# HKUDS/LLMRec

Hardware: AMD Instinct MI355X
Metric: bpr_train_edges_per_sec (higher is better)
Workload: dtype f32

## Files before the change

include/llmrec_hip.h:

```cpp
#ifndef LLMREC_HIP_H
#define LLMREC_HIP_H

#include <stdint.h>

#ifdef __cplusplus
extern "C" {
#endif

#define LLMREC_ABI_VERSION 8

enum {
    LLMREC_OK = 0,
    LLMREC_EINVAL = -1,
    LLMREC_EHIP = -2,
    LLMREC_EWORKSPACE = -3,
    LLMREC_EUNSUPPORTED = -4
};

typedef void* llmrec_stream_t;

int llmrec_abi_version(void);
const char* llmrec_status_string(int status);
const char* llmrec_last_error(void);

// ... 70 lines not shown
    const float* row_scale; const float* col_scale;
    const float* X; int64_t ldx; float* Y; int64_t ldy; int32_t d; int32_t slice_width;
    const llmrec_spmm_plan_t* plan; float* partials;
    const llmrec_spmm_epilogue_t* epilogue;
} llmrec_spmm_problem_t;
int llmrec_spmm_multi_f32(int32_t n, const llmrec_spmm_problem_t* problems, llmrec_stream_t stream);

int llmrec_linear_fwd_f32(int64_t M, int32_t N, int32_t K, const float* X, int64_t ldx,
                          const float* W, int64_t ldw, const float* bias,
                          float* Y, int64_t ldy, llmrec_stream_t stream);
#define LLMREC_LINEAR_MAX_PROBLEMS 8
typedef struct {
    const float* X; int64_t ldx; int64_t M; int32_t K;
    const float* W; int64_t ldw; const float* bias;
    float* Y; int64_t ldy;
    const float* bias_scale;
} llmrec_linear_problem_t;
int llmrec_linear_fwd_grouped_f32(int32_t n_problems, const llmrec_linear_problem_t* problems_host, int32_t N,
                                  llmrec_stream_t stream);
typedef struct { const float* dY; int64_t lddy; const float* X; int64_t ldx; int64_t M;
                 const float* db_row_weight;
                 const int32_t* row_list; const int32_t* n_rows; int64_t rows_expected;
} llmrec_wgrad_problem_t;
int llmrec_linear_wgrad_grouped_f32(int32_t n_problems, const llmrec_wgrad_problem_t* problems_host, int32_t N, int32_t K,
                                    float* dW, int64_t lddw, float* db, int32_t accumulate,
                                    void* workspace, int64_t workspace_bytes, llmrec_stream_t stream);
int llmrec_linear_wgrad_grouped_bf16x3(int32_t n_problems, const llmrec_wgrad_problem_t* problems_host, int32_t N, int32_t K,
                                       float* dW, int64_t lddw, float* db, int32_t accumulate,
                                       void* workspace, int64_t workspace_bytes, llmrec_stream_t stream);
#define LLMREC_WGRAD_MAX_TARGETS 4
typedef struct { int32_t n_problems; const llmrec_wgrad_problem_t* problems; int32_t K; float* dW; int64_t lddw; float* db; int32_t accumulate;
                 int32_t block_budget;
} llmrec_wgrad_target_t;
int64_t llmrec_linear_wgrad_multi_workspace_bytes(int32_t n_targets, const llmrec_wgrad_target_t* targets_host, int32_t N);
int llmrec_linear_wgrad_multi_bf16x3(int32_t n_targets, const llmrec_wgrad_target_t* targets_host, int32_t N,
                                     void* workspace, int64_t workspace_bytes, llmrec_stream_t stream);
typedef struct { float* W; float* m_W; float* v_W; float* b; float* m_b; float* v_b; float g_scale; } llmrec_wgrad_update_t;
int llmrec_linear_wgrad_multi_adamw_bf16x3(int32_t n_targets, const llmrec_wgrad_target_t* targets_host, int32_t N,
                                           void* workspace, int64_t workspace_bytes, const llmrec_wgrad_update_t* updates_host,
                                           const float* state3, float lr, float beta1, float beta2, float eps, float weight_decay,
                                           llmrec_stream_t stream);
int llmrec_linear_fwd_grouped_bf16x3(int32_t n_problems, const llmrec_linear_problem_t* problems_host, int32_t N,
                                     llmrec_stream_t stream);
int64_t llmrec_linear_wgrad_workspace_bytes(int64_t M, int32_t N, int32_t K);
int llmrec_linear_wgrad_f32(int64_t M, int32_t N, int32_t K, const float* dY, int64_t lddy,
                            const float* X, int64_t ldx, float* dW, int64_t lddw, float* db,
                            int32_t accumulate, void* workspace, int64_t workspace_bytes,
                            llmrec_stream_t stream);

int llmrec_softmax_rows_fwd_f32(int64_t rows, int32_t d, const float* Z, int64_t ldz,
                                float* Y, int64_t ldy, llmrec_stream_t stream);
int llmrec_softmax_rows_bwd_f32(int64_t rows, int32_t d, const float* Y, int64_t ldy,
                                const float* dY, int64_t lddy, float* dZ, int64_t lddz,
                                llmrec_stream_t stream);
int llmrec_softmax_rows_bwd_scaled_f32(int64_t rows, int32_t d, float alpha, const float* Y, int64_t ldy, const float* dY, int64_t lddy,
                                       float* dZ, int64_t lddz, llmrec_stream_t stream);
int llmrec_softmax_rows_bwd_listed_f32(int64_t n, const int64_t* ids, int32_t d, float alpha, const float* Y, int64_t ldy,
                                       const float* dY, int64_t lddy, const float* post_scale, float* dZ, int64_t lddz,
                                       llmrec_stream_t stream);

#define LLMREC_MAX_TERMS 12
int llmrec_fuse_fwd_f32(int64_t rows, int32_t d, float mean_scale,
                        int32_t n_mean, const float* const* mean_terms_host, const int64_t* mean_ld_host,
                        int32_t n_norm, const float* const* norm_terms_host, const int64_t* norm_ld_host,
                        const float* rates_host, float* out, int64_t ldo, llmrec_stream_t stream);
int llmrec_fuse_bwd_f32(int64_t rows, int32_t d, const float* dOut, int64_t lddo,
                        int32_t n_norm, const float* const* norm_terms_host, const int64_t* norm_ld_host,
                        const float* rates_host, float* const* d_terms_host, const int64_t* d_ld_host,
                        int32_t accumulate, int32_t n_reg_terms, float reg_two_coef, llmrec_stream_t stream);
int llmrec_fuse_bwd_src_f32(int64_t rows, int32_t d, const float* dOut, int64_t lddo,
                            int32_t n_norm, const float* const* norm_terms_host, const int64_t* norm_ld_host,
                            const float* rates_host, float* const* d_terms_host, const int64_t* d_ld_host,
                            const float* const* src_terms_host, const int64_t* src_ld_host,
                            int32_t n_reg_terms, float reg_two_coef, llmrec_stream_t stream);
typedef struct {
    int64_t rows; float mean_scale;
    int32_t n_mean; const float* const* mean_terms; const int64_t* mean_ld;
    int32_t n_norm; const float* const* norm_terms; const int64_t* norm_ld; const float* rates;
    float* out; int64_t ldo;
} llmrec_fuse_fwd_problem_t;
int llmrec_fuse_fwd_multi_f32(int32_t n_problems, const llmrec_fuse_fwd_problem_t* problems_host, int32_t d, llmrec_stream_t stream);
int llmrec_fuse_fwd_multi_sumsq_f32(int32_t n_problems, const llmrec_fuse_fwd_problem_t* problems_host, int32_t d, int32_t n_sumsq_terms,
                                    float* sumsq_partial, int32_t partial_capacity, int32_t* n_partial_host, llmrec_stream_t stream);
typedef struct {
    int64_t rows; const float* dOut; int64_t lddo;
    int32_t n_norm; const float* const* norm_terms; const int64_t* norm_ld; const float* rates;
    float* const* d_terms; const int64_t* d_ld;
    const float* const* src_terms; const int64_t* src_ld;
    int32_t n_reg_terms; float reg_two_coef;
    const uint8_t* row_flags;
    const int32_t* row_stamp;
} llmrec_fuse_bwd_problem_t;
int llmrec_fuse_bwd_src_multi_f32(int32_t n_problems, const llmrec_fuse_bwd_problem_t* problems_host, int32_t d, llmrec_stream_t stream);


#define LLMREC_BPR_MAX_B 4096
#define LLMREC_BPR_MAX_PROBLEMS 8
#define LLMREC_BPR_SAVED_FLOATS(B) (6 * (B) + 8)
int llmrec_bpr_prune_fwd_f32(const float* Eu, int64_t ldu, const float* Ei, int64_t ldi, int32_t d,
                             const int64_t* users, const int64_t* pos, const int64_t* neg,
                             int32_t B_max, const int32_t* n_valid_dev,
                             double remember_rate, float decay, float batch_size_flag,
                             float* out2, float* saved, llmrec_stream_t stream);
int llmrec_bpr_prune_fwd_sharded_f32(const float* Eu, int64_t ldu, const float* Ei, int64_t ldi, int32_t d,
                                     const int64_t* users, const int64_t* pos, const int64_t* neg,
                                     int32_t B_local, double remember_rate, float decay, float batch_size_flag,
                                     const float* global_m, int32_t global_B, int32_t my_offset, int32_t scores_only,
                                     float* out2, float* saved, llmrec_stream_t stream);
typedef struct {
    const float* Eu; int64_t ldu; const float* Ei; int64_t ldi;
    float* dEu; int64_t lddu; float* dEi; int64_t lddi;
    float g_mf, g_emb;
} llmrec_bpr_problem_t;
int llmrec_bpr_multi_fwd_f32(int32_t n_problems, const llmrec_bpr_problem_t* problems_host, int32_t d,
                             const int64_t* users, const int64_t* pos, const int64_t* neg,
                             int32_t B_max, const int32_t* n_valid_dev, double remember_rate, float decay,
                             float batch_size_flag, float* out, float* saved, llmrec_stream_t stream);
#define LLMREC_BPR_GATHER_FLOATS(P, B) ((P) * (B) + 4 * (P) + 1)
int llmrec_bpr_multi_fwd_sharded_f32(int32_t n_problems, const llmrec_bpr_problem_t* problems_host, int32_t d,
                                     const int64_t* users, const int64_t* pos, const int64_t* neg,
                                     int32_t B_max, const int32_t* n_valid_dev, double remember_rate, float decay,
                                     float batch_size_flag, int32_t phase, float* gather_block,
                                     const float* gathered, int32_t n_ranks, int64_t rank_stride, int32_t my_rank,
                                     float* out, float* saved, llmrec_stream_t stream);
#define LLMREC_BPR_PLAN_WORDS(B) (5 * (B))
int llmrec_bpr_scatter_plan(const int64_t* users, const int64_t* pos, const int64_t* neg, int32_t B_max, const int32_t* n_valid_dev,
                            uint64_t* plan, llmrec_stream_t stream);
int llmrec_bpr_multi_bwd_f32(int32_t n_problems, const llmrec_bpr_problem_t* problems_host, int32_t d,
                             const int64_t* users, const int64_t* pos, const int64_t* neg,
                             int32_t B_max, const int32_t* n_valid_dev, float decay, float batch_size_flag,
                             const float* saved, const uint64_t* plan, llmrec_stream_t stream);
#define LLMREC_ROW_STAMP(counter) ((uint8_t)((uint32_t)(counter) % 255u + 1u))
int llmrec_bpr_multi_scores_f32(int32_t n_problems, const llmrec_bpr_problem_t* problems_host, int32_t d,
                                const int64_t* users, const int64_t* pos, const int64_t* neg,
                                int32_t B_max, const int32_t* n_valid_dev, float* saved,
                                int32_t* row_stamp , llmrec_stream_t stream);
int llmrec_bpr_multi_select_bwd_f32(int32_t n_problems, const llmrec_bpr_problem_t* problems_host, int32_t d,
                                    const int64_t* users, const int64_t* pos, const int64_t* neg,
                                    int32_t B_max, const int32_t* n_valid_dev, double remember_rate, float decay,
                                    float batch_size_flag, float* saved,
                                    uint8_t* user_row_flags, uint8_t* item_row_flags,
                                    const int32_t* row_stamp,
                                    const uint64_t* plan,
                                    llmrec_stream_t stream);
int llmrec_bpr_multi_losses_f32(int32_t n_problems, int32_t B_max, const int32_t* n_valid_dev, double remember_rate, float decay,
                                float batch_size_flag, float* out, float* saved, llmrec_stream_t stream);
int llmrec_bpr_multi_scores_step_f32(int32_t n_problems, const llmrec_bpr_problem_t* problems_host, int32_t d,
                                     const int64_t* users, const int64_t* pos, const int64_t* neg,
                                     int32_t B_max, const int32_t* n_valid_dev, float* saved, int32_t* row_stamp,
                                     float* adamw_state3, float lr, float beta1, float beta2, llmrec_stream_t stream);
int llmrec_bpr_multi_losses_assemble_f32(int32_t n_problems, int32_t B_max, const int32_t* n_valid_dev, double remember_rate, float decay,
                                         float batch_size_flag, float* out, float* saved, const float* w_mf_host,
                                         const float* sumsq_partial, int32_t n_partial, float feat_reg_coef,
                                         float* scal4, double* running_sums3, llmrec_stream_t stream);
int llmrec_bpr_multi_zero_rows_f32(int32_t n_problems, const llmrec_bpr_problem_t* problems_host, int32_t d,
                                   const int64_t* users, const int64_t* pos, const int64_t* neg,
                                   int32_t B_max, const int32_t* n_valid_dev, llmrec_stream_t stream);
int llmrec_bpr_prune_bwd_f32(const float* Eu, int64_t ldu, const float* Ei, int64_t ldi, int32_t d,
                             const int64_t* users, const int64_t* pos, const int64_t* neg,
                             int32_t B_max, const int32_t* n_valid_dev,
                             float decay, float batch_size_flag,
                             const float* saved, const float* grads2,
                             float* dEu, int64_t lddu, float* dEi, int64_t lddi, const uint64_t* plan, llmrec_stream_t stream);

int llmrec_bpr_prune_bwd_rows_f32(const float* Eu, int64_t ldu, const float* Ei, int64_t ldi, int32_t d,
                                  const int64_t* users, const int64_t* pos, const int64_t* neg,
                                  int32_t B_max, const int32_t* n_valid_dev,
                                  float decay, float batch_size_flag,
                                  const float* saved, const float* grads2, float* rows3, llmrec_stream_t stream);

int64_t llmrec_scatter_rows_workspace_bytes(int64_t n);
int llmrec_scatter_rows_f32(int64_t n, const int64_t* ids, const float* rows, int64_t ldr, int32_t d, float alpha,
                            float* dst, int64_t ldd, void* workspace, int64_t workspace_bytes, llmrec_stream_t stream);

int64_t llmrec_sumsq_workspace_bytes(int64_t rows, int32_t d);
int llmrec_sumsq_f32(int64_t rows, int32_t d, const float* X, int64_t ldx, float coef, int32_t accumulate,
                     float* out, void* workspace, int64_t workspace_bytes, llmrec_stream_t stream);
int llmrec_axpy_f32(int64_t rows, int32_t d, float alpha, const float* alpha_dev, const float* X, int64_t ldx,
                    float* Y, int64_t ldy, int32_t accumulate, llmrec_stream_t stream);

#define LLMREC_COLSUM_MAX_GROUPS 8
int64_t llmrec_weighted_colsum_workspace_bytes(int32_t n_columns);
int llmrec_weighted_colsum_f32(int64_t rows, int32_t n_groups, int32_t group_width, const float* X, int64_t ldx, const float* w,
                               float* const* group_out_host, int32_t accumulate,
                               void* workspace, int64_t workspace_bytes, llmrec_stream_t stream);

#define LLMREC_ZERO_MAX_TENSORS 8
typedef struct { float* p; int64_t n; } llmrec_zero_tensor_t;
int llmrec_zero_multi_f32(int32_t n_tensors, const llmrec_zero_tensor_t* tensors_host, llmrec_stream_t stream);
int llmrec_zero_rows_f32(int64_t n, const int64_t* ids, int32_t d, float* dst, int64_t ldd, llmrec_stream_t stream);

int llmrec_loss_assemble_f32(int32_t mode, int32_t n_problems, const float* bpr_out, const float* w_mf_host,
                             float* scal4, float* tail, float inv_world, double* running_sums3, llmrec_stream_t stream);

int llmrec_gather_mean_f32(int64_t n, const int64_t* idx, int32_t d, float scale, int32_t n_terms,
                           const float* const* terms, const int64_t* term_ld, float* out, int64_t ldo, llmrec_stream_t stream);
int llmrec_scale_rows_f32(int64_t rows, int32_t d, const float* s, const float* X, int64_t ldx, float* Y, int64_t ldy,
                          llmrec_stream_t stream);

int llmrec_adamw_advance(float* state3, float lr, float beta1, float beta2, llmrec_stream_t stream);
int llmrec_adamw_f32(int64_t n, float* p, const float* g, float* m, float* v, const float* state3,
                     float lr, float beta1, float beta2, float eps, float weight_decay, llmrec_stream_t stream);

#define LLMREC_ADAMW_MAX_TENSORS 16
#define LLMREC_ADAMW_CHUNK 1024
typedef struct { float* p; const float* g; float* m; float* v; int64_t n;
                 float g_scale;
                 float* g_out;
} llmrec_adamw_tensor_t;
int llmrec_adamw_multi_f32(int32_t n_tensors, const llmrec_adamw_tensor_t* tensors_host, const float* state3,
                           float lr, float beta1, float beta2, float eps, float weight_decay, llmrec_stream_t stream);
#define LLMREC_ZERO_ROWS_MAX_JOBS 24
typedef struct { const int64_t* ids; float* dst; int64_t ldd; int32_t d; } llmrec_zero_rows_job_t;
int llmrec_adamw_multi_zero_rows_f32(int32_t n_tensors, const llmrec_adamw_tensor_t* tensors_host, const float* state3,
                                     float lr, float beta1, float beta2, float eps, float weight_decay,
                                     int32_t n_jobs, const llmrec_zero_rows_job_t* jobs_host, int32_t B_cap, const int32_t* n_valid_dev,
                                     llmrec_stream_t stream);

int llmrec_step_rows_group_f32(int32_t n_fuse_problems, const llmrec_fuse_bwd_problem_t* fuse_host, int32_t d,
                               int32_t n_tensors, const llmrec_adamw_tensor_t* tensors_host, const float* state3,
                               float lr, float beta1, float beta2, float eps, float weight_decay,
                               int64_t sm_rows, int32_t sm_d, float sm_alpha, const float* sm_Y, int64_t sm_ldy, const float* sm_dY, int64_t sm_lddy,
                               float* sm_dZ, int64_t sm_lddz, llmrec_stream_t stream);

#define LLMREC_TOPK_MAX 64
int llmrec_score_topk_f32(int32_t n_query, const int64_t* query_users,
                          const float* Eu, int64_t ldu, const float* Ei, int64_t ldi,
                          int64_t n_items, int32_t d,
                          const int32_t* train_rowptr, const int32_t* train_colidx,
                          int32_t K, int32_t* out_idx , float* out_score ,
                          llmrec_stream_t stream);
int llmrec_topk_set_part_items(int32_t items);
int64_t llmrec_score_topk_workspace_bytes(int32_t n_query, int64_t n_items, int32_t d);
int llmrec_score_topk_ws_f32(int32_t n_query, const int64_t* query_users,
                             const float* Eu, int64_t ldu, const float* Ei, int64_t ldi,
                             int64_t n_items, int32_t d,
                             const int32_t* train_rowptr, const int32_t* train_colidx,
                             int32_t K, int32_t* out_idx , float* out_score ,
                             void* workspace, int64_t workspace_bytes, llmrec_stream_t stream);
#define LLMREC_TOPK_PREFILTER_MAX_K 56
#define LLMREC_TOPK_MODE_EXACT_SWEEP 0
#define LLMREC_TOPK_MODE_PREFILTER 1
int llmrec_score_topk_mode_f32(int32_t n_query, const int64_t* query_users,
                               const float* Eu, int64_t ldu, const float* Ei, int64_t ldi,
                               int64_t n_items, int32_t d,
                               const int32_t* train_rowptr, const int32_t* train_colidx,
                               int32_t K, int32_t* out_idx, float* out_score,
                               void* workspace, int64_t workspace_bytes, int32_t mode, llmrec_stream_t stream);
int64_t llmrec_score_topk_stats_offset(int32_t n_query, int64_t n_items);
#define LLMREC_TOPK_WIDE_MAX 1024
int64_t llmrec_score_topk_wide_workspace_bytes(int32_t n_query, int64_t n_items, int32_t d, int32_t K, int64_t train_nnz);
int llmrec_score_topk_wide_f32(int32_t n_query, const int64_t* query_users,
                               const float* Eu, int64_t ldu, const float* Ei, int64_t ldi,
                               int64_t n_items, int32_t d,
                               const int32_t* train_rowptr, const int32_t* train_colidx,
                               int32_t K, int32_t* out_idx, float* out_score,
                               void* workspace, int64_t workspace_bytes, int32_t mode, int64_t train_nnz, llmrec_stream_t stream);
int llmrec_scores_f32(int32_t n_query, const int64_t* query_users,
                      const float* Eu, int64_t ldu, const float* Ei, int64_t ldi,
                      int64_t n_items, int32_t d, float* S, int64_t lds, llmrec_stream_t stream);
int llmrec_topk_hits(int32_t n_query, const int64_t* query_users, int32_t K, const int32_t* topk_idx,
                     const int32_t* test_rowptr, const int32_t* test_colidx, uint8_t* hits,
                     llmrec_stream_t stream);
int llmrec_topk_metrics(int32_t n_query, const int64_t* query_users, int32_t K, const uint8_t* hits, const int32_t* topk_idx,
                        const int32_t* test_rowptr, int32_t n_ks, const int32_t* ks_host, double* out, llmrec_stream_t stream);
int64_t llmrec_topk_eval_sums_workspace_bytes(int32_t n_query, int32_t n_ks);
int llmrec_topk_eval_sums(int32_t n_query, const int64_t* query_users, int32_t K, const int32_t* topk_idx, const int32_t* test_rowptr,
                          const int32_t* test_colidx, int32_t n_ks, const int32_t* ks_host, void* workspace, int64_t workspace_bytes,
                          double* out, llmrec_stream_t stream);
int64_t llmrec_score_auc_workspace_bytes(int32_t n_query, int64_t n_items, int32_t d);
int llmrec_score_auc_f32(int32_t n_query, const int64_t* query_users,
                         const float* Eu, int64_t ldu, const float* Ei, int64_t ldi,
                         int64_t n_items, int32_t d,
                         const int32_t* train_rowptr, const int32_t* train_colidx,
                         const int32_t* held_rowptr, const int32_t* held_colidx,
                         double* auc_out, int64_t* counts_out, double* sum_out,
                         void* workspace, int64_t workspace_bytes, llmrec_stream_t stream);

int llmrec_sample_bpr(uint64_t seed, uint64_t step, int64_t n_exist_users, const int64_t* exist_users,
                      int64_t n_items, const int32_t* train_rowptr, const int32_t* train_colidx,
                      int32_t B, int64_t* users, int64_t* pos, int64_t* neg, llmrec_stream_t stream);
int llmrec_sample_batch(uint64_t seed, uint64_t* step_dev, int64_t n_exist_users, const int64_t* exist_users,
                        int64_t n_items, const int32_t* train_rowptr, const int32_t* train_colidx,
                        int32_t B_global, int32_t slice_begin, int32_t B, int32_t n_aug,
                        const int64_t* aug_pos, const int64_t* aug_neg,
                        int64_t* users, int64_t* pos, int64_t* neg, int32_t* n_valid_dev, llmrec_stream_t stream);

int llmrec_timestamp(uint64_t* slot, llmrec_stream_t stream);
int64_t llmrec_timestamp_rate_hz(void);

#ifdef __cplusplus
}
#endif
#endif
```

llmrec_amd/csrc/bpr.hip:

```cpp
#include "common.h"

namespace llmrec {

constexpr int BPR_THREADS = 1024;

__device__ __forceinline__ float logsigmoid_f(float x) {
    return fminf(x, 0.f) - log1pf(expf(-fabsf(x)));
}

struct BprTables {
    const float* Eu[LLMREC_BPR_MAX_PROBLEMS];
    const float* Ei[LLMREC_BPR_MAX_PROBLEMS];
    int64_t ldu[LLMREC_BPR_MAX_PROBLEMS];
    int64_t ldi[LLMREC_BPR_MAX_PROBLEMS];
    float* dEu[LLMREC_BPR_MAX_PROBLEMS];
    float* dEi[LLMREC_BPR_MAX_PROBLEMS];
    int64_t lddu[LLMREC_BPR_MAX_PROBLEMS];
    int64_t lddi[LLMREC_BPR_MAX_PROBLEMS];
    float g_mf[LLMREC_BPR_MAX_PROBLEMS];
    float g_emb[LLMREC_BPR_MAX_PROBLEMS];
};

__device__ __forceinline__ int bpr_batch(const int32_t* n_valid_dev, int B_max) {
    int B = n_valid_dev ? n_valid_dev[0] : B_max;
    return B > B_max ? B_max : (B < 0 ? 0 : B);
}

struct StepBegin {
    int32_t* row_stamp;
    float* adamw_state;
    float lr, b1, b2;
};

__global__ __launch_bounds__(256) void bpr_scores_kernel(BprTables t, int d, const int64_t* __restrict__ users,
                                                         const int64_t* __restrict__ pos, const int64_t* __restrict__ neg,
                                                         int B_max, const int32_t* __restrict__ n_valid_dev,
                                                         float* __restrict__ saved_all, int saved_stride, StepBegin sb) {
    const int B = bpr_batch(n_valid_dev, B_max);
    const int prob = blockIdx.y;
    const int gl = threadIdx.x & 15;
    const int b = blockIdx.x * 16 + (threadIdx.x >> 4);
    if (blockIdx.x == 0 && blockIdx.y == 0 && threadIdx.x == 0) {
        if (sb.row_stamp) sb.row_stamp[0] = (int32_t)((uint32_t)sb.row_stamp[0] + 1u);
        if (sb.adamw_state) {
            const int tt = __float_as_int(sb.adamw_state[0]) + 1;
            sb.adamw_state[0] = __int_as_float(tt);
            const double bc1 = 1.0 - pow((double)sb.b1, (double)tt);
            const double bc2 = 1.0 - pow((double)sb.b2, (double)tt);
            sb.adamw_state[1] = (float)((double)sb.lr / bc1);
            sb.adamw_state[2] = (float)sqrt(bc2);
        }
    }
    if (b >= B) return;
    float* sc = saved_all + (int64_t)prob * saved_stride + B_max + 4;
    const float* u = t.Eu[prob] + users[b] * t.ldu[prob];
    const float* p = t.Ei[prob] + pos[b] * t.ldi[prob];
    const float* q = t.Ei[prob] + neg[b] * t.ldi[prob];
    float dp = 0.f, dn = 0.f, nu = 0.f, np_ = 0.f, nq = 0.f;
    for (int c = gl; c < d; c += 16) {
        const float uu = u[c], pp = p[c], qq = q[c];
        dp = fmaf(uu, pp, dp); dn = fmaf(uu, qq, dn);
        nu = fmaf(uu, uu, nu); np_ = fmaf(pp, pp, np_); nq = fmaf(qq, qq, nq);
    }
    dp = group_sum<16>(dp); dn = group_sum<16>(dn);
    nu = group_sum<16>(nu); np_ = group_sum<16>(np_); nq = group_sum<16>(nq);
    if (gl == 0) {
        const float x = (dp - dn) + 1e-8f;
        sc[b] = logsigmoid_f(x);
        sc[B_max + b] = 1.0f / (1.0f + expf(x));
        sc[2 * B_max + b] = nu; sc[3 * B_max + b] = np_; sc[4 * B_max + b] = nq;
    }
}

__device__ __forceinline__ float block_tree_sum(float v, float* red) {
    red[threadIdx.x] = v;
    __syncthreads();
    for (int off = BPR_THREADS / 2; off > 0; off >>= 1) {
        if ((int)threadIdx.x < off) red[threadIdx.x] += red[threadIdx.x + off];
        __syncthreads();
    }
    const float r = red[0];
    __syncthreads();
    return r;
// ... 26 lines not shown
    extern __shared__ __attribute__((aligned(16))) char smem[];
    float* m_s = reinterpret_cast<float*>(smem);
    const int B = bpr_batch(n_valid_dev, B_max);
    const int prob = blockIdx.y;
    float* saved = saved_all + (int64_t)prob * saved_stride;
    float* sc = saved + B_max + 4;
    int Bg, slots;
    if (ga.g) {
        slots = ga.n_ranks * ga.cap;
        Bg = gather_batch(ga);
        for (int r = 0; r < ga.n_ranks; ++r) {
            const int nv = gather_valid(ga, r);
            const float* src = ga.g + r * ga.stride + (int64_t)prob * ga.cap;
            for (int j = threadIdx.x; j < ga.cap; j += 256) m_s[r * ga.cap + j] = j < nv ? src[j] : __builtin_inff();
        }
    } else {
        slots = Bg = B;
        for (int j = threadIdx.x; j < B; j += 256) m_s[j] = sc[j];
    }
    __syncthreads();
    const int k = (int)(remember_rate * (double)Bg);
    const int gl = threadIdx.x & 15;
    const int b = blockIdx.x * 16 + (threadIdx.x >> 4);
    if (b >= B_max) return;
    if (b >= B) { if (gl == 0) { saved[b] = 0.f; sc[B_max + b] = 0.f; } return; }
    const float mb = sc[b];
    bool keep = true;
    if (k < Bg) {
        int rank = 0;
        const int me = ga.my_offset + b;
        for (int j = gl; j < slots; j += 16) {
            const float mj = m_s[j];
            rank += (mj < mb) || (mj == mb && j < me);
        }
        rank = (int)group_sum<16>((float)rank);
        keep = rank < k;
    }
    if (gl == 0) {
        saved[b] = keep ? (-1.0f / (float)k) * sc[B_max + b] : 0.f;
        sc[B_max + b] = keep ? mb : 0.f;
    }
}

__device__ __forceinline__ void bpr_reduce_problem(int prob, int B_max, const int32_t* __restrict__ n_valid_dev,
                                                   double remember_rate, float decay, float bsz,
                                                   float* __restrict__ out_all, float* __restrict__ saved_all,
                                                   int saved_stride, const BprGather& ga, float* red) {
    const int B = bpr_batch(n_valid_dev, B_max);
    float* saved = saved_all + (int64_t)prob * saved_stride;
    const float* sc = saved + B_max + 4;
    const int Bg = ga.g ? gather_batch(ga) : B;
    const int k = (int)(remember_rate * (double)Bg);
    float part = 0.f, su = 0.f, sp = 0.f, sq = 0.f;
    for (int b = threadIdx.x; b < B; b += BPR_THREADS) {
        part += sc[B_max + b];
        su += sc[2 * B_max + b]; sp += sc[3 * B_max + b]; sq += sc[4 * B_max + b];
    }
    const float kept = block_tree_sum(part, red);
    float Su = block_tree_sum(su, red), Sp = block_tree_sum(sp, red), Sq = block_tree_sum(sq, red);
    if (threadIdx.x == 0) {
        if (ga.g && ga.has_tail) {
            Su = Sp = Sq = 0.f;
            for (int r = 0; r < ga.n_ranks; ++r) {
                const float* nb = ga.g + r * ga.stride + (int64_t)ga.n_prob * ga.cap + 4 * prob;
                Su += nb[0]; Sp += nb[1]; Sq += nb[2];
            }
        }
        out_all[prob * 2 + 0] = -(kept / (float)k);
        const float reg = 1.0f / (2.0f * Su + 1e-8f) + 1.0f / (2.0f * Sp + 1e-8f) + 1.0f / (2.0f * Sq + 1e-8f);
        out_all[prob * 2 + 1] = decay * (reg / bsz);
        saved[B_max + 0] = Su; saved[B_max + 1] = Sp; saved[B_max + 2] = Sq; saved[B_max + 3] = (float)k;
    }
}

__global__ __launch_bounds__(BPR_THREADS) void bpr_reduce_kernel(int B_max, const int32_t* __restrict__ n_valid_dev,
                                                                 double remember_rate, float decay, float bsz,
                                                                 float* __restrict__ out_all, float* __restrict__ saved_all,
                                                                 int saved_stride, BprGather ga) {
    __shared__ float red[BPR_THREADS];
    bpr_reduce_problem(blockIdx.x, B_max, n_valid_dev, remember_rate, decay, bsz, out_all, saved_all, saved_stride, ga, red);
}

struct LossW { float w[LLMREC_BPR_MAX_PROBLEMS]; };
constexpr int LA_GROUP = BPR_THREADS / LLMREC_BPR_MAX_PROBLEMS;
__global__ __launch_bounds__(BPR_THREADS) void bpr_losses_assemble_kernel(int n_prob, int B_max, const int32_t* __restrict__ n_valid_dev,
                                                                          double remember_rate, float decay, float bsz,
                                                                          float* __restrict__ out_all, float* __restrict__ saved_all, int saved_stride,
                                                                          LossW w, const float* __restrict__ partial, int n_partial, float reg_coef,
                                                                          float* __restrict__ scal, double* __restrict__ running) {
    __shared__ float red[LLMREC_BPR_MAX_PROBLEMS][BPR_THREADS];
    __shared__ float outs[LLMREC_BPR_MAX_PROBLEMS][2];
    const int B = bpr_batch(n_valid_dev, B_max);
    const int prob = threadIdx.x / LA_GROUP, t = threadIdx.x % LA_GROUP;
    const bool live = prob < n_prob;
    float* saved = saved_all + (int64_t)(live ? prob : 0) * saved_stride;
    const float* sc = saved + B_max + 4;
    float tot[4] = {0.f, 0.f, 0.f, 0.f};
#pragma unroll
    for (int col = 0; col < 4; ++col) {
        const float* src = sc + (int64_t)(col + 1) * B_max;
        if (live) {
            for (int v = t; v < BPR_THREADS; v += LA_GROUP) {
                float s_ = 0.f;
                for (int b = v; b < B; b += BPR_THREADS) s_ += src[b];
                red[prob][v] = s_;
            }
        }
        __syncthreads();
        for (int off = BPR_THREADS / 2; off > 0; off >>= 1) {
            if (live) for (int i = t; i < off; i += LA_GROUP) red[prob][i] += red[prob][i + off];
            __syncthreads();
        }
        tot[col] = red[live ? prob : 0][0];
        __syncthreads();
    }
    if (live && t == 0) {
        const int k = (int)(remember_rate * (double)B);
        const float mf = -(tot[0] / (float)k);
        const float reg = 1.0f / (2.0f * tot[1] + 1e-8f) + 1.0f / (2.0f * tot[2] + 1e-8f) + 1.0f / (2.0f * tot[3] + 1e-8f);
        const float emb = decay * (reg / bsz);
        out_all[prob * 2 + 0] = mf; out_all[prob * 2 + 1] = emb;
        outs[prob][0] = mf; outs[prob][1] = emb;
        saved[B_max + 0] = tot[1]; saved[B_max + 1] = tot[2]; saved[B_max + 2] = tot[3]; saved[B_max + 3] = (float)k;
    }
    float feat = scal[0];
    if (partial) {
        float s_ = 0.f;
        for (int i = threadIdx.x; i < n_partial; i += BPR_THREADS) s_ += partial[i];
        feat = reg_coef * block_tree_sum(s_, red[0]);
    }
    __syncthreads();
    if (threadIdx.x != 0) return;
    float s = 0.f;
    for (int p = 0; p < n_prob; ++p) s += outs[p][0] * w.w[p];
    scal[0] = feat;
    scal[2] = outs[0][0]; scal[3] = outs[0][1];
    scal[1] = s + outs[0][1] + feat;
    if (running) { running[0] += (double)scal[1]; running[1] += (double)scal[2]; running[2] += (double)scal[3]; }
}

__global__ __launch_bounds__(256) void bpr_pack_kernel(int n_prob, int B_max, const int32_t* __restrict__ n_valid_dev,
                                                       const float* __restrict__ saved_all, int saved_stride, float* __restrict__ block) {
    const int B = bpr_batch(n_valid_dev, B_max);
    const int total = n_prob * B_max + 4 * n_prob + 1;
    for (int i = blockIdx.x * 256 + threadIdx.x; i < total; i += gridDim.x * 256) {
        float v;
        if (i < n_prob * B_max) {
            const int p = i / B_max, b = i - p * B_max;
            v = b < B ? saved_all[(int64_t)p * saved_stride + B_max + 4 + b] : __builtin_inff();
        } else if (i < n_prob * B_max + 4 * n_prob) {
            const int j = i - n_prob * B_max;
            v = saved_all[(int64_t)(j >> 2) * saved_stride + B_max + (j & 3)];
        } else {
            v = (float)B;
        }
        block[i] = v;
    }
}

constexpr uint32_t PLAN_NO_ID = 0xffffffffu;
__global__ __launch_bounds__(256) void bpr_plan_kernel(const int64_t* __restrict__ users, const int64_t* __restrict__ pos,
                                                       const int64_t* __restrict__ neg, int B_max,
                                                       const int32_t* __restrict__ n_valid_dev, uint64_t* __restrict__ plan) {
    extern __shared__ __attribute__((aligned(16))) char smem[];
    uint64_t* k = reinterpret_cast<uint64_t*>(smem);
    const int B = bpr_batch(n_valid_dev, B_max);
    const int nbu = (B_max + 15) / 16;
    const bool items = (int)blockIdx.x >= nbu;
    const int n = items ? 2 * B_max : B_max;
    for (int i = threadIdx.x; i < n; i += 256) {
        const int b = (items && i >= B_max) ? i - B_max : i;
        uint64_t id = PLAN_NO_ID;
        if (b < B) id = (uint64_t)(items ? (i >= B_max ? neg[b] : pos[b]) : users[b]);
        k[i] = (id << 32) | (uint64_t)(uint32_t)i;
    }
    __syncthreads();
    const int gl = threadIdx.x & 15;
    const int i = ((int)blockIdx.x - (items ? nbu : 0)) * 16 + (threadIdx.x >> 4);
    if (i >= n) return;
    const uint64_t me = k[i];
    const uint32_t id = (uint32_t)(me >> 32);
    int below = 0, lower_id = 0, same_id = 0;
    for (int j = gl; j < n; j += 16) {
        const uint64_t kj = k[j];
        const uint32_t idj = (uint32_t)(kj >> 32);
        below += kj < me; lower_id += idj < id; same_id += idj == id;
    }
    below = (int)group_sum<16>((float)below); lower_id = (int)group_sum<16>((float)lower_id); same_id = (int)group_sum<16>((float)same_id);
    if (gl == 0) {
        const int base = items ? B_max : 0;
        plan[base + below] = me;
        int32_t* runlen = reinterpret_cast<int32_t*>(plan + 3 * (int64_t)B_max);
        runlen[base + below] = (below == lower_id && id != PLAN_NO_ID) ? same_id : 0;
    }
}

constexpr int RUN_MAX_SHARE = LLMREC_BPR_MAX_PROBLEMS;
struct RunShare {
    const float* Eu[RUN_MAX_SHARE]; const float* Ei[RUN_MAX_SHARE]; const float* saved[RUN_MAX_SHARE];
    int64_t ldu[RUN_MAX_SHARE], ldi[RUN_MAX_SHARE];
    float g_mf[RUN_MAX_SHARE], cu[RUN_MAX_SHARE], cp[RUN_MAX_SHARE], cq[RUN_MAX_SHARE];
    int n, any_reg;
};
struct RunRec { const float* a; const float* b; const float* self; float ds, cr; };

template <int NV, bool VEC> struct RunAcc;
template <int NV> struct RunAcc<NV, true> {
    float4 v[NV];
    __device__ __forceinline__ void load(const float* row, int c0, int d, int gl) {
#pragma unroll
        for (int i = 0; i < NV; ++i) { const int c = c0 + 4 * (gl + 16 * i); v[i] = c < d ? *reinterpret_cast<const float4*>(row + c) : float4{0.f, 0.f, 0.f, 0.f}; }
    }
    __device__ __forceinline__ void store(float* row, int c0, int d, int gl) const {
#pragma unroll
        for (int i = 0; i < NV; ++i) { const int c = c0 + 4 * (gl + 16 * i); if (c < d) *reinterpret_cast<float4*>(row + c) = v[i]; }
    }
};
template <int NV> struct RunAcc<NV, false> {
    float v[4 * NV];
    __device__ __forceinline__ void load(const float* row, int c0, int d, int gl) {
#pragma unroll
        for (int i = 0; i < 4 * NV; ++i) { const int c = c0 + gl + 16 * i; v[i] = c < d ? row[c] : 0.f; }
    }
    __device__ __forceinline__ void store(float* row, int c0, int d, int gl) const {
#pragma unroll
        for (int i = 0; i < 4 * NV; ++i) { const int c = c0 + gl + 16 * i; if (c < d) row[c] = v[i]; }
    }
};
template <int NV, bool VEC, bool ITEM, bool REG>
__device__ __forceinline__ void run_add(RunAcc<NV, VEC>& acc, const RunAcc<NV, VEC>& a, const RunAcc<NV, VEC>& b, const RunAcc<NV, VEC>& self,
                                        float ds, float cr) {
    if constexpr (VEC) {
#pragma unroll
        for (int i = 0; i < NV; ++i) {
            const float4 x = a.v[i], y = ITEM ? float4{0.f, 0.f, 0.f, 0.f} : b.v[i], z = REG ? self.v[i] : float4{0.f, 0.f, 0.f, 0.f};
            acc.v[i].x += fmaf(ds, ITEM ? x.x : x.x - y.x, cr * z.x); acc.v[i].y += fmaf(ds, ITEM ? x.y : x.y - y.y, cr * z.y);
            acc.v[i].z += fmaf(ds, ITEM ? x.z : x.z - y.z, cr * z.z); acc.v[i].w += fmaf(ds, ITEM ? x.w : x.w - y.w, cr * z.w);
        }
    } else {
#pragma unroll
        for (int i = 0; i < 4 * NV; ++i)
            acc.v[i] += fmaf(ds, ITEM ? a.v[i] : a.v[i] - b.v[i], cr * (REG ? self.v[i] : 0.f));
    }
}

template <int NV, bool VEC, bool ITEM, bool REG>
__device__ __forceinline__ void run_stream(RunAcc<NV, VEC>& acc, const RunRec* __restrict__ recs, int n, int c0, int d, int gl) {
    int i = 0;
    for (; i + 4 <= n; i += 4) {
        RunAcc<NV, VEC> a[4], b[4], z[4];
        float ds[4], cr[4];
#pragma unroll
        for (int u = 0; u < 4; ++u) {
            const RunRec r = recs[i + u];
            ds[u] = r.ds; cr[u] = r.cr;
            a[u].load(r.a, c0, d, gl);
            if (!ITEM) b[u].load(r.b, c0, d, gl);
            if (REG) z[u].load(r.self, c0, d, gl);
        }
#pragma unroll
        for (int u = 0; u < 4; ++u) run_add<NV, VEC, ITEM, REG>(acc, a[u], b[u], z[u], ds[u], cr[u]);
    }
    for (; i < n; ++i) {
        const RunRec r = recs[i];
        RunAcc<NV, VEC> a, b, z;
        a.load(r.a, c0, d, gl);
        if (!ITEM) b.load(r.b, c0, d, gl);
        if (REG) z.load(r.self, c0, d, gl);
        run_add<NV, VEC, ITEM, REG>(acc, a, b, z, r.ds, r.cr);
    }
}

template <bool VEC, int NV>
__global__ __launch_bounds__(256) void bpr_bwd_runs_kernel(BprTables t, int n_prob, int d, const int64_t* __restrict__ users,
                                                           const int64_t* __restrict__ pos, const int64_t* __restrict__ neg,
                                                           int B_max, float decay, float bsz, const float* __restrict__ saved_all,
                                                           int saved_stride, const uint64_t* __restrict__ plan,
// ... 143 lines not shown
    const int B = bpr_batch(n_valid_dev, B_max);
    const int prob = blockIdx.y;
    const int gl = threadIdx.x & 15;
    const int b = blockIdx.x * 16 + (threadIdx.x >> 4);
    if (b >= B) return;
    float* du = t.dEu[prob] + users[b] * t.lddu[prob];
    float* dpp = t.dEi[prob] + pos[b] * t.lddi[prob];
    float* dqq = t.dEi[prob] + neg[b] * t.lddi[prob];
    for (int c = gl; c < d; c += 16) { du[c] = 0.f; dpp[c] = 0.f; dqq[c] = 0.f; }
}

__global__ __launch_bounds__(256) void bpr_bwd_rows_kernel(const float* __restrict__ Eu, int64_t ldu,
                                                           const float* __restrict__ Ei, int64_t ldi, int d,
                                                           const int64_t* __restrict__ users, const int64_t* __restrict__ pos,
                                                           const int64_t* __restrict__ neg, int B_max,
                                                           const int32_t* __restrict__ n_valid_dev, float decay, float bsz,
                                                           const float* __restrict__ saved, const float* __restrict__ grads2,
                                                           float* __restrict__ rows3) {
    int B = n_valid_dev ? n_valid_dev[0] : B_max;
    if (B > B_max) B = B_max;
    const float g_mf = grads2[0], g_emb = grads2[1];
    const float Su = saved[B_max], Sp = saved[B_max + 1], Sq = saved[B_max + 2];
    const float base = -4.0f * decay / bsz * g_emb;
    const float du_ = 2.0f * Su + 1e-8f, dp_ = 2.0f * Sp + 1e-8f, dq_ = 2.0f * Sq + 1e-8f;
    const float cu = base / (du_ * du_), cp = base / (dp_ * dp_), cq = base / (dq_ * dq_);
    const int gl = threadIdx.x & 15;
    const int groups = gridDim.x * (blockDim.x >> 4);
    const int64_t plane = (int64_t)B_max * d;
    for (int b = blockIdx.x * (blockDim.x >> 4) + (threadIdx.x >> 4); b < B_max; b += groups) {
        float* ru = rows3 + (int64_t)b * d;
        if (b >= B) {
            for (int c = gl; c < d; c += 16) { ru[c] = 0.f; ru[plane + c] = 0.f; ru[2 * plane + c] = 0.f; }
            continue;
        }
        const float ds = g_mf * saved[b];
        const float* u = Eu + users[b] * ldu;
        const float* p = Ei + pos[b] * ldi;
        const float* q = Ei + neg[b] * ldi;
        for (int c = gl; c < d; c += 16) {
            const float uu = u[c], pp = p[c], qq = q[c];
            ru[c] = fmaf(ds, pp - qq, cu * uu);
            ru[plane + c] = fmaf(ds, uu, cp * pp);
            ru[2 * plane + c] = fmaf(-ds, uu, cq * qq);
        }
    }
}

struct Philox {
    uint32_t key[2];
    __device__ Philox(uint64_t seed) { key[0] = (uint32_t)seed; key[1] = (uint32_t)(seed >> 32); }
    __device__ void operator()(uint32_t c0, uint32_t c1, uint32_t c2, uint32_t c3, uint32_t out[4]) const {
        uint32_t k0 = key[0], k1 = key[1];
#pragma unroll
        for (int r = 0; r < 10; ++r) {
            const uint64_t p0 = (uint64_t)0xD2511F53u * c0, p1 = (uint64_t)0xCD9E8D57u * c2;
            const uint32_t n0 = (uint32_t)(p1 >> 32) ^ c1 ^ k0, n1 = (uint32_t)p1;
            const uint32_t n2 = (uint32_t)(p0 >> 32) ^ c3 ^ k1, n3 = (uint32_t)p0;
            c0 = n0; c1 = n1; c2 = n2; c3 = n3;
            k0 += 0x9E3779B9u; k1 += 0xBB67AE85u;
        }
        out[0] = c0; out[1] = c1; out[2] = c2; out[3] = c3;
    }
};

__device__ __forceinline__ uint32_t bounded(uint32_t r, uint32_t n) { return (uint32_t)(((uint64_t)r * n) >> 32); }

__device__ uint64_t keyed_perm(uint64_t x, uint64_t n, int half_bits, const Philox& ph, uint32_t step_lo, uint32_t step_hi) {
    const uint64_t mask = (1ull << half_bits) - 1;
    do {
        uint64_t L = x >> half_bits, R = x & mask;
#pragma unroll
        for (int r = 0; r < 4; ++r) {
            uint32_t o[4];
            ph((uint32_t)R, (uint32_t)(R >> 32) ^ (0xA5A50000u + r), step_lo, step_hi, o);
            const uint64_t f = (((uint64_t)o[1] << 32) | o[0]) & mask;
            const uint64_t nL = R, nR = L ^ f;
            L = nL; R = nR;
        }
        x = (L << half_bits) | R;
    } while (x >= n);
    return x;
}

__device__ __forceinline__ void sample_one(const Philox& ph, uint32_t slo, uint32_t shi, int b, int B, int half_bits,
                                           int64_t n_exist, const int64_t* __restrict__ exist_users, int64_t n_items,
                                           const int32_t* __restrict__ rowptr, const int32_t* __restrict__ colidx,
                                           int64_t& u_out, int64_t& p_out, int64_t& q_out) {
    uint64_t slot;
    if ((int64_t)B <= n_exist) {
        slot = keyed_perm((uint64_t)b, (uint64_t)n_exist, half_bits, ph, slo, shi);
    } else {
        uint32_t o[4];
        ph((uint32_t)b, 0x55AA0001u, slo, shi, o);
        slot = ((((uint64_t)o[1] << 32) | o[0]) % (uint64_t)n_exist);
    }
    const int64_t u = exist_users[slot];
    const int32_t s = rowptr[u], e = rowptr[u + 1];
    uint32_t o[4];
    ph((uint32_t)b, 0x55AA0002u, slo, shi, o);
    const int64_t p = colidx[s + (int32_t)bounded(o[0], (uint32_t)(e - s))];
    int64_t q = 0;
    uint32_t ctr = 0;
    int have = 4;
    for (int tries = 0; tries < 4096; ++tries) {
        if (have == 4) { ph((uint32_t)b, 0x55AA0003u + ctr, slo, shi, o); ++ctr; have = 0; }
        const uint32_t r = o[have++];
        q = n_items <= 0xffffffffll ? (int64_t)bounded(r, (uint32_t)n_items) : (int64_t)(r % (uint64_t)n_items);
        int32_t lo = s, hi = e;
        while (lo < hi) {
            const int32_t mid = (lo + hi) >> 1;
            if (colidx[mid] < q) lo = mid + 1; else hi = mid;
        }
        if (!(lo < e && colidx[lo] == q)) break;
    }
    u_out = u; p_out = p; q_out = q;
}

__global__ void sample_bpr_kernel(uint64_t seed, uint64_t step, int64_t n_exist, const int64_t* __restrict__ exist_users,
                                  int64_t n_items, const int32_t* __restrict__ rowptr, const int32_t* __restrict__ colidx,
                                  int B, int half_bits, int64_t* __restrict__ users, int64_t* __restrict__ pos,
                                  int64_t* __restrict__ neg) {
    const int b = blockIdx.x * blockDim.x + threadIdx.x;
    if (b >= B) return;
    const Philox ph(seed);
    sample_one(ph, (uint32_t)step, (uint32_t)(step >> 32), b, B, half_bits, n_exist, exist_users, n_items, rowptr, colidx,
               users[b], pos[b], neg[b]);
}

constexpr int SAMPLE_THREADS = 1024;
__global__ __launch_bounds__(SAMPLE_THREADS) void sample_batch_kernel(
    uint64_t seed, unsigned long long* __restrict__ step_dev, int64_t n_exist, const int64_t* __restrict__ exist_users,
    int64_t n_items, const int32_t* __restrict__ rowptr, const int32_t* __restrict__ colidx,
    int B_global, int half_bits_users, int slice_begin, int B, int n_aug, int half_bits_batch,
    const int64_t* __restrict__ aug_pos, const int64_t* __restrict__ aug_neg,
    int64_t* __restrict__ users, int64_t* __restrict__ pos, int64_t* __restrict__ neg, int32_t* __restrict__ n_valid_dev) {
    __shared__ int wave_tot[SAMPLE_THREADS / 64];
    __shared__ int base_s;
    const unsigned long long step = *step_dev;
    const uint32_t slo = (uint32_t)step, shi = (uint32_t)(step >> 32);
    const Philox ph(seed);
    for (int b = threadIdx.x; b < B; b += SAMPLE_THREADS)
        sample_one(ph, slo, shi, slice_begin + b, B_global, half_bits_users, n_exist, exist_users, n_items, rowptr, colidx,
                   users[b], pos[b], neg[b]);
    if (threadIdx.x == 0) base_s = 0;
    __syncthreads();
    const Philox pa(seed ^ 0x9E3779B97F4A7C15ull);
    const int lane = threadIdx.x & 63, wv = threadIdx.x >> 6;
    for (int a0 = 0; a0 < n_aug; a0 += SAMPLE_THREADS) {
        const int a = a0 + threadIdx.x;
        int64_t u = 0, ap = 0, an = 0;
        bool ok = false;
        if (a < n_aug) {
            const uint64_t slot = keyed_perm((uint64_t)a, (uint64_t)B, half_bits_batch, pa, slo, shi);
            u = users[slot];
            ap = aug_pos[u]; an = aug_neg[u];
            ok = ap >= 0 && an >= 0 && ap < n_items && an < n_items;
        }
        const unsigned long long bal = __ballot(ok);
        const int before = __popcll(bal & ((1ull << lane) - 1ull));
        if (lane == 0) wave_tot[wv] = __popcll(bal);
        __syncthreads();
        int wave_base = 0, chunk_tot = 0;
        for (int k = 0; k < SAMPLE_THREADS / 64; ++k) { const int t = wave_tot[k]; if (k < wv) wave_base += t; chunk_tot += t; }
        const int base = base_s;
        if (a < n_aug && ok) {
            const int o = B + base + wave_base + before;
            users[o] = u; pos[o] = ap; neg[o] = an;
        }
        __syncthreads();
        if (threadIdx.x == 0) base_s = base + chunk_tot;
        __syncthreads();
    }
    const int kept = base_s;
    for (int o = B + kept + threadIdx.x; o < B + n_aug; o += SAMPLE_THREADS) { users[o] = 0; pos[o] = 0; neg[o] = 0; }
    if (threadIdx.x == 0) { n_valid_dev[0] = B + kept; *step_dev = step + 1ull; }
}

}

using namespace llmrec;

extern "C" {

static int launch_bpr_fwd(const BprTables& t, int n_prob, int d, const int64_t* users, const int64_t* pos, const int64_t* neg,
                          int B_max, const int32_t* n_valid_dev, double remember_rate, float decay, float bsz,
                          float* out, float* saved, const BprGather& ga, bool do_scores, bool do_select, float* pack_out,
                          hipStream_t stream, StepBegin step_begin = StepBegin{}) {
    const int stride = LLMREC_BPR_SAVED_FLOATS(B_max);
    const BprGather none = {};
    if (do_scores && B_max > 0) {
        dim3 grid((unsigned)ceil_div(B_max, 16), (unsigned)n_prob);
        bpr_scores_kernel<<<grid, 256, 0, stream>>>(t, d, users, pos, neg, B_max, n_valid_dev, saved, stride, step_begin);
        LLMREC_LAUNCH_CHECK();
    }
    if (pack_out) {
        bpr_reduce_kernel<<<n_prob, BPR_THREADS, 0, stream>>>(B_max, n_valid_dev, remember_rate, decay, bsz, out, saved, stride, none);
        LLMREC_LAUNCH_CHECK();
        bpr_pack_kernel<<<ceil_div(n_prob * B_max + 4 * n_prob + 1, 256), 256, 0, stream>>>(n_prob, B_max, n_valid_dev, saved, stride, pack_out);
        LLMREC_LAUNCH_CHECK();
    }
    if (do_select) {
        const size_t shmem = sizeof(float) * (size_t)(ga.g ? ga.n_ranks * ga.cap : (B_max > 0 ? B_max : 1));
        dim3 grid((unsigned)ceil_div(B_max > 0 ? B_max : 1, 16), (unsigned)n_prob);
        bpr_rank_kernel<<<grid, 256, shmem, stream>>>(B_max, n_valid_dev, remember_rate, saved, stride, ga);
        LLMREC_LAUNCH_CHECK();
        bpr_reduce_kernel<<<n_prob, BPR_THREADS, 0, stream>>>(B_max, n_valid_dev, remember_rate, decay, bsz, out, saved, stride, ga);
        LLMREC_LAUNCH_CHECK();
    }
    return LLMREC_OK;
}

int llmrec_bpr_prune_fwd_f32(const float* Eu, int64_t ldu, const float* Ei, int64_t ldi, int32_t d,
                             const int64_t* users, const int64_t* pos, const int64_t* neg,
                             int32_t B_max, const int32_t* n_valid_dev,
                             double remember_rate, float decay, float batch_size_flag,
                             float* out2, float* saved, llmrec_stream_t stream_) {
    LLMREC_CHECK_ARG(B_max >= 0 && d > 0 && out2 && saved, "bpr_fwd: bad argument");
    if (B_max > LLMREC_BPR_MAX_B) { set_error("bpr_fwd: B_max %d > %d", B_max, LLMREC_BPR_MAX_B); return LLMREC_EUNSUPPORTED; }
    LLMREC_CHECK_ARG(B_max == 0 || (Eu && Ei && users && pos && neg && ldu >= d && ldi >= d), "bpr_fwd: null pointer or ld < d");
    BprTables t = {};
    t.Eu[0] = Eu; t.Ei[0] = Ei; t.ldu[0] = ldu; t.ldi[0] = ldi;
    return launch_bpr_fwd(t, 1, d, users, pos, neg, B_max, n_valid_dev, remember_rate, decay, batch_size_flag, out2, saved,
                          BprGather{}, true, true, nullptr, (hipStream_t)stream_);
}

int llmrec_bpr_prune_fwd_sharded_f32(const float* Eu, int64_t ldu, const float* Ei, int64_t ldi, int32_t d,
                                     const int64_t* users, const int64_t* pos, const int64_t* neg,
                                     int32_t B_local, double remember_rate, float decay, float batch_size_flag,
                                     const float* global_m, int32_t global_B, int32_t my_offset, int32_t scores_only,
                                     float* out2, float* saved, llmrec_stream_t stream_) {
    LLMREC_CHECK_ARG(B_local >= 0 && d > 0 && out2 && saved, "bpr_fwd_sharded: bad argument");
    if (B_local > LLMREC_BPR_MAX_B || global_B > 3 * LLMREC_BPR_MAX_B) { set_error("bpr_fwd_sharded: batch too large"); return LLMREC_EUNSUPPORTED; }
    LLMREC_CHECK_ARG(B_local == 0 || (Eu && Ei && users && pos && neg && ldu >= d && ldi >= d), "bpr_fwd_sharded: null pointer or ld < d");
    LLMREC_CHECK_ARG(scores_only || (global_m && global_B >= B_local && my_offset >= 0 && my_offset + B_local <= global_B),
                     "bpr_fwd_sharded: pass 2 needs the gathered scores and a valid offset");
    BprTables t = {};
    t.Eu[0] = Eu; t.Ei[0] = Ei; t.ldu[0] = ldu; t.ldi[0] = ldi;
    BprGather ga = {};
    if (!scores_only) { ga.g = global_m; ga.n_ranks = 1; ga.stride = 0; ga.cap = global_B; ga.n_prob = 1; ga.my_offset = my_offset; ga.has_tail = 0; }
    return launch_bpr_fwd(t, 1, d, users, pos, neg, B_local, nullptr, remember_rate, decay, batch_size_flag, out2, saved,
                          ga, scores_only != 0, scores_only == 0, nullptr, (hipStream_t)stream_);
}

static int fill_tables(BprTables& t, int n, const llmrec_bpr_problem_t* p, int d, bool need_grads) {
    for (int i = 0; i < n; ++i) {
        if (!p[i].Eu || !p[i].Ei || p[i].ldu < d || p[i].ldi < d) return 1;
        if (need_grads && (!p[i].dEu || !p[i].dEi || p[i].lddu < d || p[i].lddi < d)) return 1;
        t.Eu[i] = p[i].Eu; t.Ei[i] = p[i].Ei; t.ldu[i] = p[i].ldu; t.ldi[i] = p[i].ldi;
        t.dEu[i] = p[i].dEu; t.dEi[i] = p[i].dEi; t.lddu[i] = p[i].lddu; t.lddi[i] = p[i].lddi;
        t.g_mf[i] = p[i].g_mf; t.g_emb[i] = p[i].g_emb;
    }
    return 0;
}

int llmrec_bpr_multi_fwd_f32(int32_t n_problems, const llmrec_bpr_problem_t* problems_host, int32_t d,
                             const int64_t* users, const int64_t* pos, const int64_t* neg,
                             int32_t B_max, const int32_t* n_valid_dev, double remember_rate, float decay,
                             float batch_size_flag, float* out, float* saved, llmrec_stream_t stream_) {
    LLMREC_CHECK_ARG(n_problems >= 1 && n_problems <= LLMREC_BPR_MAX_PROBLEMS && problems_host && d > 0 && out && saved,
                     "bpr_multi_fwd: bad argument");
    if (B_max > LLMREC_BPR_MAX_B) { set_error("bpr_multi_fwd: B_max %d > %d", B_max, LLMREC_BPR_MAX_B); return LLMREC_EUNSUPPORTED; }
    LLMREC_CHECK_ARG(B_max == 0 || (users && pos && neg), "bpr_multi_fwd: null index pointer");
    BprTables t = {};
    LLMREC_CHECK_ARG(!fill_tables(t, n_problems, problems_host, d, false), "bpr_multi_fwd: bad problem table");
    return launch_bpr_fwd(t, n_problems, d, users, pos, neg, B_max, n_valid_dev, remember_rate, decay, batch_size_flag, out, saved,
                          BprGather{}, true, true, nullptr, (hipStream_t)stream_);
}

int llmrec_bpr_multi_fwd_sharded_f32(int32_t n_problems, const llmrec_bpr_problem_t* problems_host, int32_t d,
                                     const int64_t* users, const int64_t* pos, const int64_t* neg,
                                     int32_t B_max, const int32_t* n_valid_dev, double remember_rate, float decay,
                                     float batch_size_flag, int32_t phase, float* gather_block,
                                     const float* gathered, int32_t n_ranks, int64_t rank_stride, int32_t my_rank,
                                     float* out, float* saved, llmrec_stream_t stream_) {
    LLMREC_CHECK_ARG(n_problems >= 1 && n_problems <= LLMREC_BPR_MAX_PROBLEMS && problems_host && d > 0 && out && saved,
                     "bpr_multi_fwd_sharded: bad argument");
    LLMREC_CHECK_ARG(phase == 1 || phase == 2, "bpr_multi_fwd_sharded: phase is 1 (scores + gather block) or 2 (selection)");
    if (B_max > LLMREC_BPR_MAX_B) { set_error("bpr_multi_fwd_sharded: B_max %d > %d", B_max, LLMREC_BPR_MAX_B); return LLMREC_EUNSUPPORTED; }
    LLMREC_CHECK_ARG(B_max == 0 || (users && pos && neg), "bpr_multi_fwd_sharded: null index pointer");
    BprTables t = {};
    LLMREC_CHECK_ARG(!fill_tables(t, n_problems, problems_host, d, false), "bpr_multi_fwd_sharded: bad problem table");
    if (phase == 1) {
        LLMREC_CHECK_ARG(gather_block, "bpr_multi_fwd_sharded: phase 1 needs the gather block");
        return launch_bpr_fwd(t, n_problems, d, users, pos, neg, B_max, n_valid_dev, remember_rate, decay, batch_size_flag, out, saved,
                              BprGather{}, true, false, gather_block, (hipStream_t)stream_);
    }
    LLMREC_CHECK_ARG(gathered && n_ranks >= 1 && my_rank >= 0 && my_rank < n_ranks &&
                     rank_stride >= LLMREC_BPR_GATHER_FLOATS(n_problems, B_max), "bpr_multi_fwd_sharded: bad gathered layout");
    if ((int64_t)n_ranks * B_max > 4 * LLMREC_BPR_MAX_B) {
        set_error("bpr_multi_fwd_sharded: global batch capacity %lld > %d", (long long)n_ranks * B_max, 4 * LLMREC_BPR_MAX_B);
        return LLMREC_EUNSUPPORTED;
    }
    BprGather ga = {};
    ga.g = gathered; ga.n_ranks = n_ranks; ga.stride = rank_stride; ga.cap = B_max; ga.n_prob = n_problems;
    ga.my_offset = my_rank * B_max; ga.has_tail = 1;
    return launch_bpr_fwd(t, n_problems, d, users, pos, neg, B_max, n_valid_dev, remember_rate, decay, batch_size_flag, out, saved,
                          ga, false, true, nullptr, (hipStream_t)stream_);
}

int llmrec_bpr_scatter_plan(const int64_t* users, const int64_t* pos, const int64_t* neg, int32_t B_max, const int32_t* n_valid_dev,
                            uint64_t* plan, llmrec_stream_t stream_) {
    LLMREC_CHECK_ARG(B_max >= 0, "bpr_scatter_plan: bad argument");
    if (B_max > LLMREC_BPR_MAX_B) { set_error("bpr_scatter_plan: B_max %d > %d", B_max, LLMREC_BPR_MAX_B); return LLMREC_EUNSUPPORTED; }
    if (B_max == 0) return LLMREC_OK;
    LLMREC_CHECK_ARG(users && pos && neg && plan, "bpr_scatter_plan: null pointer");
    const unsigned blocks = (unsigned)(ceil_div(B_max, 16) + ceil_div(2 * (int64_t)B_max, 16));
    bpr_plan_kernel<<<blocks, 256, sizeof(uint64_t) * 2 * (size_t)B_max, (hipStream_t)stream_>>>(users, pos, neg, B_max, n_valid_dev, plan);
    LLMREC_LAUNCH_CHECK();
    return LLMREC_OK;
}

static int launch_bwd_runs(const BprTables& t, int n_prob, int d, const int64_t* users, const int64_t* pos, const int64_t* neg, int B_max,
                           float decay, float bsz, const float* saved, const uint64_t* plan, const float* grads2_dev, hipStream_t stream) {
    dim3 grid((unsigned)(ceil_div(B_max, 16) + ceil_div(2 * (int64_t)B_max, 16)), (unsigned)n_prob);
    bool vec = d % 4 == 0;
    for (int i = 0; i < n_prob && vec; ++i)
        vec = t.ldu[i] % 4 == 0 && t.ldi[i] % 4 == 0 && t.lddu[i] % 4 == 0 && t.lddi[i] % 4 == 0 &&
              ((uintptr_t)t.Eu[i] | (uintptr_t)t.Ei[i] | (uintptr_t)t.dEu[i] | (uintptr_t)t.dEi[i]) % 16 == 0;
    const int stride = LLMREC_BPR_SAVED_FLOATS(B_max);
#define RUNS_LAUNCH(V, N) bpr_bwd_runs_kernel<V, N><<<grid, 256, 0, stream>>>(t, n_prob, d, users, pos, neg, B_max, decay, bsz, saved, stride, plan, grads2_dev)
    if (vec) { if (d <= 64) RUNS_LAUNCH(true, 1); else RUNS_LAUNCH(true, 2); }
    else { if (d <= 64) RUNS_LAUNCH(false, 1); else RUNS_LAUNCH(false, 2); }
#undef RUNS_LAUNCH
    LLMREC_LAUNCH_CHECK();
    return LLMREC_OK;
}

int llmrec_bpr_multi_bwd_f32(int32_t n_problems, const llmrec_bpr_problem_t* problems_host, int32_t d,
                             const int64_t* users, const int64_t* pos, const int64_t* neg,
                             int32_t B_max, const int32_t* n_valid_dev, float decay, float batch_size_flag,
                             const float* saved, const uint64_t* plan, llmrec_stream_t stream_) {
    (void)n_valid_dev;
    LLMREC_CHECK_ARG(n_problems >= 1 && n_problems <= LLMREC_BPR_MAX_PROBLEMS && problems_host && d > 0 && saved,
                     "bpr_multi_bwd: bad argument");
    if (B_max == 0) return LLMREC_OK;
    LLMREC_CHECK_ARG(users && pos && neg && plan, "bpr_multi_bwd: null index pointer or no scatter plan (llmrec_bpr_scatter_plan)");
    BprTables t = {};
    LLMREC_CHECK_ARG(!fill_tables(t, n_problems, problems_host, d, true), "bpr_multi_bwd: bad problem table");
    return launch_bwd_runs(t, n_problems, d, users, pos, neg, B_max, decay, batch_size_flag, saved, plan, nullptr, (hipStream_t)stream_);
}

int llmrec_bpr_multi_scores_f32(int32_t n_problems, const llmrec_bpr_problem_t* problems_host, int32_t d,
                                const int64_t* users, const int64_t* pos, const int64_t* neg,
                                int32_t B_max, const int32_t* n_valid_dev, float* saved, int32_t* row_stamp, llmrec_stream_t stream_) {
    LLMREC_CHECK_ARG(n_problems >= 1 && n_problems <= LLMREC_BPR_MAX_PROBLEMS && problems_host && d > 0 && saved, "bpr_multi_scores: bad argument");
    if (B_max > LLMREC_BPR_MAX_B) { set_error("bpr_multi_scores: B_max %d > %d", B_max, LLMREC_BPR_MAX_B); return LLMREC_EUNSUPPORTED; }
    LLMREC_CHECK_ARG(B_max == 0 || (users && pos && neg), "bpr_multi_scores: null index pointer");
    BprTables t = {};
    LLMREC_CHECK_ARG(!fill_tables(t, n_problems, problems_host, d, false), "bpr_multi_scores: bad problem table");
    StepBegin sb = {};
    sb.row_stamp = row_stamp;
    return launch_bpr_fwd(t, n_problems, d, users, pos, neg, B_max, n_valid_dev, 0.0, 0.f, 1.f, nullptr, saved, BprGather{}, true, false,
                          nullptr, (hipStream_t)stream_, sb);
}

int llmrec_bpr_multi_scores_step_f32(int32_t n_problems, const llmrec_bpr_problem_t* problems_host, int32_t d,
                                     const int64_t* users, const int64_t* pos, const int64_t* neg,
                                     int32_t B_max, const int32_t* n_valid_dev, float* saved, int32_t* row_stamp,
                                     float* adamw_state3, float lr, float beta1, float beta2, llmrec_stream_t stream_) {
    LLMREC_CHECK_ARG(n_problems >= 1 && n_problems <= LLMREC_BPR_MAX_PROBLEMS && problems_host && d > 0 && saved, "bpr_multi_scores_step: bad argument");
    if (B_max > LLMREC_BPR_MAX_B) { set_error("bpr_multi_scores_step: B_max %d > %d", B_max, LLMREC_BPR_MAX_B); return LLMREC_EUNSUPPORTED; }
    LLMREC_CHECK_ARG(B_max > 0 && users && pos && neg, "bpr_multi_scores_step: empty batch capacity or null index pointer (the launch carries the step's counters)");
    BprTables t = {};
    LLMREC_CHECK_ARG(!fill_tables(t, n_problems, problems_host, d, false), "bpr_multi_scores_step: bad problem table");
    StepBegin sb = {};
    sb.row_stamp = row_stamp; sb.adamw_state = adamw_state3; sb.lr = lr; sb.b1 = beta1; sb.b2 = beta2;
    return launch_bpr_fwd(t, n_problems, d, users, pos, neg, B_max, n_valid_dev, 0.0, 0.f, 1.f, nullptr, saved, BprGather{}, true, false,
                          nullptr, (hipStream_t)stream_, sb);
}

int llmrec_bpr_multi_select_bwd_f32(int32_t n_problems, const llmrec_bpr_problem_t* problems_host, int32_t d,
                                    const int64_t* users, const int64_t* pos, const int64_t* neg,
                                    int32_t B_max, const int32_t* n_valid_dev, double remember_rate, float decay,
                                    float batch_size_flag, float* saved, uint8_t* user_row_flags, uint8_t* item_row_flags,
                                    const int32_t* row_stamp, const uint64_t* plan, llmrec_stream_t stream_) {
    LLMREC_CHECK_ARG(n_problems >= 1 && n_problems <= LLMREC_BPR_MAX_PROBLEMS && problems_host && d > 0 && saved, "bpr_multi_select_bwd: bad argument");
    if (B_max > LLMREC_BPR_MAX_B) { set_error("bpr_multi_select_bwd: B_max %d > %d", B_max, LLMREC_BPR_MAX_B); return LLMREC_EUNSUPPORTED; }
    if (B_max == 0) return LLMREC_OK;
    LLMREC_CHECK_ARG(users && pos && neg && plan, "bpr_multi_select_bwd: null index pointer or no scatter plan (llmrec_bpr_scatter_plan)");
    BprTables t = {};
    LLMREC_CHECK_ARG(!fill_tables(t, n_problems, problems_host, d, true), "bpr_multi_select_bwd: bad problem table");
    dim3 grid((unsigned)ceil_div(B_max, 16) + 1u, (unsigned)n_problems);
    const size_t shmem = sizeof(float) * (size_t)(B_max > 3 * BPR_THREADS ? B_max : 3 * BPR_THREADS);
    bpr_select_kernel<<<grid, 256, shmem, (hipStream_t)stream_>>>(users, pos, neg, B_max, n_valid_dev, remember_rate, saved,
                                                                 LLMREC_BPR_SAVED_FLOATS(B_max), user_row_flags, item_row_flags, row_stamp);
    LLMREC_LAUNCH_CHECK();
    return launch_bwd_runs(t, n_problems, d, users, pos, neg, B_max, decay, batch_size_flag, saved, plan, nullptr, (hipStream_t)stream_);
}

int llmrec_bpr_multi_losses_f32(int32_t n_problems, int32_t B_max, const int32_t* n_valid_dev, double remember_rate, float decay,
// ... 24 lines not shown
}

int llmrec_bpr_multi_zero_rows_f32(int32_t n_problems, const llmrec_bpr_problem_t* problems_host, int32_t d,
                                   const int64_t* users, const int64_t* pos, const int64_t* neg,
                                   int32_t B_max, const int32_t* n_valid_dev, llmrec_stream_t stream_) {
    LLMREC_CHECK_ARG(n_problems >= 1 && n_problems <= LLMREC_BPR_MAX_PROBLEMS && problems_host && d > 0, "bpr_multi_zero_rows: bad argument");
    if (B_max == 0) return LLMREC_OK;
    LLMREC_CHECK_ARG(users && pos && neg, "bpr_multi_zero_rows: null index pointer");
    BprTables t = {};
    LLMREC_CHECK_ARG(!fill_tables(t, n_problems, problems_host, d, true), "bpr_multi_zero_rows: bad problem table");
    dim3 grid((unsigned)ceil_div(B_max, 16), (unsigned)n_problems);
    bpr_zero_rows_kernel<<<grid, 256, 0, (hipStream_t)stream_>>>(t, d, users, pos, neg, B_max, n_valid_dev);
    LLMREC_LAUNCH_CHECK();
    return LLMREC_OK;
}

int llmrec_bpr_prune_bwd_f32(const float* Eu, int64_t ldu, const float* Ei, int64_t ldi, int32_t d,
                             const int64_t* users, const int64_t* pos, const int64_t* neg,
                             int32_t B_max, const int32_t* n_valid_dev, float decay, float batch_size_flag,
                             const float* saved, const float* grads2,
                             float* dEu, int64_t lddu, float* dEi, int64_t lddi, const uint64_t* plan, llmrec_stream_t stream_) {
    (void)n_valid_dev;
    LLMREC_CHECK_ARG(B_max >= 0 && d > 0 && saved && grads2, "bpr_bwd: bad argument");
    if (B_max == 0) return LLMREC_OK;
    LLMREC_CHECK_ARG(Eu && Ei && users && pos && neg && dEu && dEi && ldu >= d && ldi >= d && lddu >= d && lddi >= d,
                     "bpr_bwd: null pointer or ld < d");
    LLMREC_CHECK_ARG(plan, "bpr_bwd: no scatter plan (llmrec_bpr_scatter_plan)");
    LLMREC_CHECK_ARG(dEu != dEi, "bpr_bwd: dEu and dEi must be distinct buffers");
    BprTables t = {};
    t.Eu[0] = Eu; t.Ei[0] = Ei; t.ldu[0] = ldu; t.ldi[0] = ldi;
    t.dEu[0] = dEu; t.dEi[0] = dEi; t.lddu[0] = lddu; t.lddi[0] = lddi;
    return launch_bwd_runs(t, 1, d, users, pos, neg, B_max, decay, batch_size_flag, saved, plan, grads2, (hipStream_t)stream_);
}

int llmrec_bpr_prune_bwd_rows_f32(const float* Eu, int64_t ldu, const float* Ei, int64_t ldi, int32_t d,
                                  const int64_t* users, const int64_t* pos, const int64_t* neg,
                                  int32_t B_max, const int32_t* n_valid_dev, float decay, float batch_size_flag,
                                  const float* saved, const float* grads2, float* rows3, llmrec_stream_t stream_) {
    hipStream_t stream = (hipStream_t)stream_;
    LLMREC_CHECK_ARG(B_max >= 0 && d > 0 && saved && grads2, "bpr_bwd_rows: bad argument");
    if (B_max == 0) return LLMREC_OK;
    LLMREC_CHECK_ARG(Eu && Ei && users && pos && neg && rows3 && ldu >= d && ldi >= d, "bpr_bwd_rows: null pointer or ld < d");
    bpr_bwd_rows_kernel<<<grid_for(B_max, 16), 256, 0, stream>>>(Eu, ldu, Ei, ldi, d, users, pos, neg, B_max, n_valid_dev, decay,
                                                                 batch_size_flag, saved, grads2, rows3);
    LLMREC_LAUNCH_CHECK();
    return LLMREC_OK;
}

int llmrec_sample_bpr(uint64_t seed, uint64_t step, int64_t n_exist_users, const int64_t* exist_users,
                      int64_t n_items, const int32_t* train_rowptr, const int32_t* train_colidx,
                      int32_t B, int64_t* users, int64_t* pos, int64_t* neg, llmrec_stream_t stream_) {
    LLMREC_CHECK_ARG(B >= 0 && n_exist_users > 0 && n_items > 0, "sample_bpr: bad sizes");
    if (B == 0) return LLMREC_OK;
    LLMREC_CHECK_ARG(exist_users && train_rowptr && train_colidx && users && pos && neg, "sample_bpr: null pointer");
    int half_bits = 1;
    while ((1ull << (2 * half_bits)) < (uint64_t)n_exist_users) ++half_bits;
    sample_bpr_kernel<<<(B + 255) / 256, 256, 0, (hipStream_t)stream_>>>(seed, step, n_exist_users, exist_users, n_items,
                                                                          train_rowptr, train_colidx, B, half_bits, users, pos, neg);
    LLMREC_LAUNCH_CHECK();
    return LLMREC_OK;
}

int llmrec_sample_batch(uint64_t seed, uint64_t* step_dev, int64_t n_exist_users, const int64_t* exist_users,
                        int64_t n_items, const int32_t* train_rowptr, const int32_t* train_colidx,
                        int32_t B_global, int32_t slice_begin, int32_t B, int32_t n_aug,
                        const int64_t* aug_pos, const int64_t* aug_neg,
                        int64_t* users, int64_t* pos, int64_t* neg, int32_t* n_valid_dev, llmrec_stream_t stream_) {
    LLMREC_CHECK_ARG(B >= 1 && B_global >= B && slice_begin >= 0 && slice_begin + B <= B_global && n_aug >= 0 && n_aug <= B &&
                     n_exist_users > 0 && n_items > 0, "sample_batch: bad sizes");
    LLMREC_CHECK_ARG(step_dev && exist_users && train_rowptr && train_colidx && users && pos && neg && n_valid_dev,
                     "sample_batch: null pointer");
    LLMREC_CHECK_ARG(n_aug == 0 || (aug_pos && aug_neg), "sample_batch: augmented pairs missing");
    int hb_users = 1, hb_batch = 1;
    while ((1ull << (2 * hb_users)) < (uint64_t)n_exist_users) ++hb_users;
    while ((1ull << (2 * hb_batch)) < (uint64_t)B) ++hb_batch;
    sample_batch_kernel<<<1, SAMPLE_THREADS, 0, (hipStream_t)stream_>>>(seed, (unsigned long long*)step_dev, n_exist_users, exist_users,
                                                                       n_items, train_rowptr, train_colidx, B_global, hb_users,
                                                                       slice_begin, B, n_aug, hb_batch, aug_pos, aug_neg,
                                                                       users, pos, neg, n_valid_dev);
    LLMREC_LAUNCH_CHECK();
    return LLMREC_OK;
}

}
```

llmrec_amd/csrc/rowops.hip:

```cpp
#include "common.h"
#include <type_traits>

namespace llmrec {

constexpr int RL = 16;
constexpr int ROWS_PER_BLOCK = 256 / RL;

template <int VEC, int NCHUNK>
struct RowReg {
    float x[NCHUNK][VEC];
    __device__ __forceinline__ void load(const float* row, int gl, int d) {
#pragma unroll
        for (int k = 0; k < NCHUNK; ++k) {
            const int c = (k * RL + gl) * VEC;
            if (VEC == 4) {
                float4 v = (c < d) ? *reinterpret_cast<const float4*>(row + c) : make_float4(0.f, 0.f, 0.f, 0.f);
                x[k][0] = v.x; x[k][1 % VEC] = v.y; x[k][2 % VEC] = v.z; x[k][3 % VEC] = v.w;
            } else {
                x[k][0] = (c < d) ? row[c] : 0.f;
            }
        }
    }
    __device__ __forceinline__ void store(float* row, int gl, int d) const {
#pragma unroll
        for (int k = 0; k < NCHUNK; ++k) {
            const int c = (k * RL + gl) * VEC;
            if (c < d) {
                if (VEC == 4) *reinterpret_cast<float4*>(row + c) = make_float4(x[k][0], x[k][1 % VEC], x[k][2 % VEC], x[k][3 % VEC]);
                else row[c] = x[k][0];
            }
        }
    }
    __device__ __forceinline__ void fill(float v) {
#pragma unroll
        for (int k = 0; k < NCHUNK; ++k)
#pragma unroll
            for (int q = 0; q < VEC; ++q) x[k][q] = v;
    }
    __device__ __forceinline__ float dot(const RowReg& o) const {
        float s = 0.f;
#pragma unroll
        for (int k = 0; k < NCHUNK; ++k)
#pragma unroll
            for (int q = 0; q < VEC; ++q) s = fmaf(x[k][q], o.x[k][q], s);
        return group_sum<RL>(s);
    }
};

#define ROW_LOOP_HEADER(vb, nvb)                                                                  \
    const int gl = threadIdx.x & (RL - 1);                                                        \
    const int64_t row_stride = (int64_t)(nvb) * ROWS_PER_BLOCK;                                   \
    for (int64_t row = (int64_t)(vb) * ROWS_PER_BLOCK + threadIdx.x / RL; row < rows; row += row_stride)

template <int VEC, int NCHUNK>
__global__ __launch_bounds__(256) void softmax_fwd_kernel(int64_t rows, int d, const float* __restrict__ Z, int64_t ldz,
                                                          float* __restrict__ Y, int64_t ldy) {
    ROW_LOOP_HEADER(blockIdx.x, gridDim.x) {
        RowReg<VEC, NCHUNK> z;
        z.load(Z + row * ldz, gl, d);
        float mx = -INFINITY;
#pragma unroll
        for (int k = 0; k < NCHUNK; ++k)
#pragma unroll
            for (int q = 0; q < VEC; ++q)
                if ((k * RL + gl) * VEC + q < d) mx = fmaxf(mx, z.x[k][q]);
        mx = group_max<RL>(mx);
        float s = 0.f;
#pragma unroll
        for (int k = 0; k < NCHUNK; ++k)
#pragma unroll
            for (int q = 0; q < VEC; ++q) {
                const bool in = (k * RL + gl) * VEC + q < d;
                z.x[k][q] = in ? expf(z.x[k][q] - mx) : 0.f;
                s += z.x[k][q];
            }
        s = group_sum<RL>(s);
        const float inv = 1.0f / s;
#pragma unroll
        for (int k = 0; k < NCHUNK; ++k)
#pragma unroll
            for (int q = 0; q < VEC; ++q) z.x[k][q] *= inv;
        z.store(Y + row * ldy, gl, d);
    }
// ... 53 lines not shown
            for (int k = 0; k < NCHUNK; ++k)
#pragma unroll
                for (int q = 0; q < VEC; ++q) acc.x[k][q] += t.x[k][q];
        }
#pragma unroll
        for (int k = 0; k < NCHUNK; ++k)
#pragma unroll
            for (int q = 0; q < VEC; ++q) acc.x[k][q] *= a.mean_scale;
        for (int i = 0; i < a.n_norm; ++i) {
            t.load(a.norm_terms[i] + row * a.norm_ld[i], gl, d);
            const float nrm = fmaxf(sqrtf(t.dot(t)), 1e-12f);
            const float w = a.rates[i] / nrm;
#pragma unroll
            for (int k = 0; k < NCHUNK; ++k)
#pragma unroll
                for (int q = 0; q < VEC; ++q) acc.x[k][q] = fmaf(w, t.x[k][q], acc.x[k][q]);
        }
        acc.store(out + row * ldo, gl, d);
    }
}

template <int VEC, int NCHUNK>
__global__ __launch_bounds__(256) void fuse_bwd_kernel(int64_t rows, int d, FuseArgs a, const float* __restrict__ dOut,
                                                       int64_t lddo, int accumulate) {
    ROW_LOOP_HEADER(blockIdx.x, gridDim.x) {
        RowReg<VEC, NCHUNK> g, t, o;
        g.load(dOut + row * lddo, gl, d);
        for (int i = 0; i < a.n_norm; ++i) {
            t.load(a.norm_terms[i] + row * a.norm_ld[i], gl, d);
            const float nn = sqrtf(t.dot(t));
            float* dst = a.d_terms[i] + row * a.d_ld[i];
            if (accumulate == 1) o.load(dst, gl, d);
            else if (accumulate == 2 && a.s_terms[i]) o.load(a.s_terms[i] + row * a.s_ld[i], gl, d);
            else o.fill(0.f);
            if (nn >= 1e-12f) {
                const float inv = 1.0f / nn;
                const float proj = t.dot(g) * inv * inv;
                const float w = a.rates[i] * inv;
#pragma unroll
                for (int k = 0; k < NCHUNK; ++k)
#pragma unroll
                    for (int q = 0; q < VEC; ++q) o.x[k][q] += w * (g.x[k][q] - t.x[k][q] * proj);
            } else {
                const float w = a.rates[i] * 1e12f;
#pragma unroll
                for (int k = 0; k < NCHUNK; ++k)
#pragma unroll
                    for (int q = 0; q < VEC; ++q) o.x[k][q] += w * g.x[k][q];
            }
            if (i < a.n_reg) {
#pragma unroll
                for (int k = 0; k < NCHUNK; ++k)
#pragma unroll
                    for (int q = 0; q < VEC; ++q) o.x[k][q] = fmaf(a.reg2, t.x[k][q], o.x[k][q]);
            }
            o.store(dst, gl, d);
        }
    }
}

constexpr int FUSE_MAX_PROBLEMS = 2;
struct FuseMulti {
    FuseArgs a[FUSE_MAX_PROBLEMS];
    int64_t rows[FUSE_MAX_PROBLEMS];
    float* out[FUSE_MAX_PROBLEMS]; int64_t ldo[FUSE_MAX_PROBLEMS];
    const float* dOut[FUSE_MAX_PROBLEMS]; int64_t lddo[FUSE_MAX_PROBLEMS];
    const uint8_t* row_flags[FUSE_MAX_PROBLEMS];
    const int32_t* row_stamp[FUSE_MAX_PROBLEMS];
    int block_begin;
    int n_sumsq;
    float* sumsq_partial;
};
#define ROW_LOOP_MULTI(m, vb, nvb)                                                                 \
    const int prob = (vb) >= (m).block_begin ? 1 : 0;                                              \
    const FuseArgs& a = (m).a[prob];                                                               \
    const int64_t rows = (m).rows[prob];                                                           \
    const int gl = threadIdx.x & (RL - 1);                                                         \
    const int blk = (vb) - (prob ? (m).block_begin : 0);                                           \
    const int nblk = prob ? (nvb) - (m).block_begin : (m).block_begin;                             \
    const int64_t row_stride = (int64_t)nblk * ROWS_PER_BLOCK;                                     \
    for (int64_t row = (int64_t)blk * ROWS_PER_BLOCK + threadIdx.x / RL; row < rows; row += row_stride)

template <int VEC, int NCHUNK>
__global__ __launch_bounds__(256) void fuse_fwd_multi_kernel(int d, FuseMulti m) {
    __shared__ float ss_red[256];
    float ss = 0.f;
    ROW_LOOP_MULTI(m, (int)blockIdx.x, (int)gridDim.x) {
        RowReg<VEC, NCHUNK> acc, t;
        acc.fill(0.f);
        for (int i = 0; i < a.n_mean; ++i) {
            t.load(a.mean_terms[i] + row * a.mean_ld[i], gl, d);
#pragma unroll
            for (int k = 0; k < NCHUNK; ++k)
#pragma unroll
                for (int q = 0; q < VEC; ++q) acc.x[k][q] += t.x[k][q];
        }
#pragma unroll
        for (int k = 0; k < NCHUNK; ++k)
#pragma unroll
            for (int q = 0; q < VEC; ++q) acc.x[k][q] *= a.mean_scale;
        for (int i = 0; i < a.n_norm; ++i) {
            t.load(a.norm_terms[i] + row * a.norm_ld[i], gl, d);
            const float sq = t.dot(t);
            if (i < m.n_sumsq && gl == 0) ss += sq;
            const float nrm = fmaxf(sqrtf(sq), 1e-12f);
            const float w = a.rates[i] / nrm;
#pragma unroll
            for (int k = 0; k < NCHUNK; ++k)
#pragma unroll
                for (int q = 0; q < VEC; ++q) acc.x[k][q] = fmaf(w, t.x[k][q], acc.x[k][q]);
        }
        acc.store(m.out[prob] + row * m.ldo[prob], gl, d);
    }
    if (m.n_sumsq > 0) {
        ss_red[threadIdx.x] = ss;
        __syncthreads();
        for (int off = 128; off > 0; off >>= 1) {
            if ((int)threadIdx.x < off) ss_red[threadIdx.x] += ss_red[threadIdx.x + off];
            __syncthreads();
        }
        if (threadIdx.x == 0) m.sumsq_partial[blockIdx.x] = ss_red[0];
    }
}

template <int VEC, int NCHUNK>
__device__ __forceinline__ void fuse_bwd_src_multi_rows(int vb, int nvb, int d, const FuseMulti& m) {
    ROW_LOOP_MULTI(m, vb, nvb) {
        RowReg<VEC, NCHUNK> g, t, o;
        if (m.row_flags[prob] && !(m.row_stamp[prob] ? m.row_flags[prob][row] == LLMREC_ROW_STAMP(m.row_stamp[prob][0]) : m.row_flags[prob][row] != 0)) {
            for (int i = 0; i < a.n_norm; ++i) {
                o.fill(0.f);
                if (i < a.n_reg) {
                    t.load(a.norm_terms[i] + row * a.norm_ld[i], gl, d);
#pragma unroll
                    for (int k = 0; k < NCHUNK; ++k)
#pragma unroll
                        for (int q = 0; q < VEC; ++q) o.x[k][q] = fmaf(a.reg2, t.x[k][q], o.x[k][q]);
                }
                o.store(a.d_terms[i] + row * a.d_ld[i], gl, d);
            }
            continue;
        }
        g.load(m.dOut[prob] + row * m.lddo[prob], gl, d);
        for (int i = 0; i < a.n_norm; ++i) {
            t.load(a.norm_terms[i] + row * a.norm_ld[i], gl, d);
            const float nn = sqrtf(t.dot(t));
            float* dst = a.d_terms[i] + row * a.d_ld[i];
            if (a.s_terms[i]) o.load(a.s_terms[i] + row * a.s_ld[i], gl, d);
            else o.fill(0.f);
            if (nn >= 1e-12f) {
                const float inv = 1.0f / nn;
                const float proj = t.dot(g) * inv * inv;
                const float w = a.rates[i] * inv;
#pragma unroll
                for (int k = 0; k < NCHUNK; ++k)
#pragma unroll
                    for (int q = 0; q < VEC; ++q) o.x[k][q] += w * (g.x[k][q] - t.x[k][q] * proj);
            } else {
                const float w = a.rates[i] * 1e12f;
#pragma unroll
                for (int k = 0; k < NCHUNK; ++k)
#pragma unroll
                    for (int q = 0; q < VEC; ++q) o.x[k][q] += w * g.x[k][q];
            }
            if (i < a.n_reg) {
#pragma unroll
                for (int k = 0; k < NCHUNK; ++k)
#pragma unroll
                    for (int q = 0; q < VEC; ++q) o.x[k][q] = fmaf(a.reg2, t.x[k][q], o.x[k][q]);
            }
            o.store(dst, gl, d);
        }
    }
}

template <int VEC, int NCHUNK>
__global__ __launch_bounds__(256) void fuse_bwd_src_multi_kernel(int d, FuseMulti m) {
    fuse_bwd_src_multi_rows<VEC, NCHUNK>((int)blockIdx.x, (int)gridDim.x, d, m);
}

constexpr int SUMSQ_BLOCKS = 1024;

__global__ __launch_bounds__(256) void sumsq_partial_kernel(int64_t rows, int d, const float* __restrict__ X, int64_t ldx,
                                                            float* __restrict__ partial) {
    __shared__ float red[256];
    float s = 0.f;
    const int64_t n = rows * d;
    for (int64_t e = (int64_t)blockIdx.x * 256 + threadIdx.x; e < n; e += (int64_t)gridDim.x * 256) {
        const float v = X[(e / d) * ldx + (e % d)];
        s = fmaf(v, v, s);
    }
    red[threadIdx.x] = s;
    __syncthreads();
    for (int off = 128; off > 0; off >>= 1) {
        if ((int)threadIdx.x < off) red[threadIdx.x] += red[threadIdx.x + off];
        __syncthreads();
    }
    if (threadIdx.x == 0) partial[blockIdx.x] = red[0];
}

__global__ __launch_bounds__(256) void sumsq_final_kernel(int n_partial, const float* __restrict__ partial, float coef,
                                                          int accumulate, float* __restrict__ out) {
    __shared__ float red[256];
    float s = 0.f;
    for (int i = threadIdx.x; i < n_partial; i += 256) s += partial[i];
// ... 215 lines not shown
    if (mode == 0) {
        float s = 0.f;
        for (int p = 0; p < n_prob; ++p) s += out[2 * p] * w.w[p];
        scal[2] = out[0]; scal[3] = out[1];
        scal[1] = s + out[1] + scal[0];
    } else if (mode == 1) {
        for (int p = 0; p < n_prob; ++p) tail[p] = out[2 * p];
        tail[n_prob] = (out[1] + scal[0]) * inv_world;
    } else {
        float s = 0.f;
        for (int p = 0; p < n_prob; ++p) s += tail[p] * w.w[p];
        scal[2] = tail[0]; scal[3] = out[1];
        scal[1] = s + tail[n_prob];
    }
    if (running && mode != 1) { running[0] += (double)scal[1]; running[1] += (double)scal[2]; running[2] += (double)scal[3]; }
}

__global__ __launch_bounds__(256) void scale_rows_kernel(int64_t rows, int d, const float* __restrict__ s, const float* __restrict__ X, int64_t ldx,
                                                         float* __restrict__ Y, int64_t ldy) {
    const int64_t n = rows * d;
    for (int64_t e = (int64_t)blockIdx.x * blockDim.x + threadIdx.x; e < n; e += (int64_t)gridDim.x * blockDim.x) {
        const int64_t r = e / d; const int c = (int)(e - r * d);
        Y[r * ldy + c] = s[r] * X[r * ldx + c];
    }
}

__global__ __launch_bounds__(256) void zero_rows_kernel(int64_t n, const int64_t* __restrict__ ids, int d, float* __restrict__ dst, int64_t ldd) {
    const int gl = threadIdx.x & 15;
    const int64_t j = (int64_t)blockIdx.x * 16 + (threadIdx.x >> 4);
    if (j >= n) return;
    const int64_t row = ids[j];
    if (row < 0) return;
    float* p = dst + row * ldd;
    for (int c = gl; c < d; c += 16) p[c] = 0.f;
}

__global__ __launch_bounds__(256) void scatter_set_rows_kernel(int capacity, const int32_t* __restrict__ list, const int32_t* __restrict__ n_dev, int d,
                                                               const float* __restrict__ src, int64_t lds_, float* __restrict__ dst, int64_t ldd) {
    const int gl = threadIdx.x & 15;
    const int j = blockIdx.x * 16 + (threadIdx.x >> 4);
    if (j >= capacity || j >= n_dev[0]) return;
    const float* s_ = src + (int64_t)j * lds_;
    float* o = dst + (int64_t)list[j] * ldd;
    for (int c = gl; c < d; c += 16) o[c] = s_[c];
}

__global__ __launch_bounds__(256) void mark_rows_kernel(int64_t n, const int64_t* __restrict__ ids, uint8_t value, uint8_t* __restrict__ flags) {
    const int64_t j = (int64_t)blockIdx.x * 256 + threadIdx.x;
    if (j >= n) return;
    const int64_t row = ids[j];
    if (row >= 0) flags[row] = value;
}

__global__ __launch_bounds__(256) void softmax_bwd_listed_kernel(int64_t n, const int64_t* __restrict__ ids, int d, float alpha,
                                                                 const float* __restrict__ Y, int64_t ldy, const float* __restrict__ dY, int64_t lddy,
                                                                 const float* __restrict__ post_scale, float* __restrict__ dZ, int64_t lddz) {
    const int gl = threadIdx.x & 15;
    const int64_t j = (int64_t)blockIdx.x * 16 + (threadIdx.x >> 4);
    if (j >= n) return;
    const int64_t row = ids[j];
    if (row < 0) return;
    const float* y = Y + row * ldy; const float* g = dY + row * lddy;
    float dot = 0.f;
    for (int c = gl; c < d; c += 16) dot = fmaf(y[c], alpha * g[c], dot);
    dot = group_sum<16>(dot);
    const float ps = post_scale ? post_scale[row] : 1.0f;
    float* o = dZ + row * lddz;
    for (int c = gl; c < d; c += 16) o[c] = ps * (y[c] * (alpha * g[c] - dot));
}

constexpr int MARK_SPLIT = 32;
__global__ __launch_bounds__(256) void mark_neighbours_kernel(int64_t n, const int64_t* __restrict__ ids, const int32_t* __restrict__ rowptr,
                                                              const int32_t* __restrict__ colidx, uint8_t value, uint8_t* __restrict__ flags) {
    const int64_t w = (int64_t)blockIdx.x * 4 + (threadIdx.x >> 6);
    const int64_t j = w / MARK_SPLIT;
    const int part = (int)(w - j * MARK_SPLIT);
    if (j >= n) return;
    const int64_t row = ids[j];
    if (row < 0) return;
    const int32_t s = rowptr[row], e = rowptr[row + 1];
    for (int64_t k = (int64_t)s + part * 64 + (threadIdx.x & 63); k < e; k += 64 * MARK_SPLIT) flags[colidx[k]] = value;
}

constexpr int REACH_SPLIT = 8;
__global__ __launch_bounds__(256) void batch_reach_mark_kernel(int B_cap, const int32_t* __restrict__ n_valid, const int64_t* __restrict__ users,
                                                               const int64_t* __restrict__ pos, const int64_t* __restrict__ neg, int64_t n_users,
                                                               int64_t n_items, const int32_t* __restrict__ rowptr, const int32_t* __restrict__ colidx,
                                                               uint8_t* __restrict__ flags) {
    const int w = blockIdx.x * 4 + (threadIdx.x >> 6), lane = threadIdx.x & 63;
    int nv = n_valid ? *n_valid : B_cap;
    nv = nv < B_cap ? nv : B_cap;
    const int part = w % REACH_SPLIT, job = w / REACH_SPLIT;
    const int b = job / 3, role = job - 3 * b;
    if (b >= nv) return;
    if (role == 0) {
        const int64_t u = users[b];
        if (part == 0 && lane == 0 && u >= 0 && u < n_users) flags[u] = 1;
        return;
    }
    const int64_t it = role == 1 ? pos[b] : neg[b];
    if (it < 0 || it >= n_items) return;
    const int32_t s = rowptr[it], e = rowptr[it + 1];
    for (int32_t k = s + part * 64 + lane; k < e; k += 64 * REACH_SPLIT) flags[colidx[k]] = 1;
}

__global__ __launch_bounds__(1024) void flags_compact_kernel(int64_t n, uint8_t* __restrict__ flags, int32_t* __restrict__ list, int32_t* __restrict__ n_out) {
    __shared__ int32_t wave_total[16];
    const int tid = threadIdx.x, lane = tid & 63, wave = tid >> 6;
    const int64_t per = ((n + 1023) / 1024 + 15) / 16 * 16;
    const int64_t r0 = tid * per, r1 = r0 + per < n ? r0 + per : n;
    int32_t c = 0;
    for (int64_t r = r0; r < r1; r += 16) {
        const uint4 v = *reinterpret_cast<const uint4*>(flags + r);
        const uint32_t wd[4] = {v.x, v.y, v.z, v.w};
#pragma unroll
        for (int q = 0; q < 4; ++q)
#pragma unroll
            for (int bb = 0; bb < 4; ++bb)
                c += (r + 4 * q + bb < r1) && ((wd[q] >> (8 * bb)) & 0xffu);
    }
    int32_t incl = c;
#pragma unroll
    for (int off = 1; off < 64; off <<= 1) {
        const int32_t v = __shfl_up(incl, off, 64);
        if (lane >= off) incl += v;
    }
    if (lane == 63) wave_total[wave] = incl;
    __syncthreads();
    int32_t base = 0, total = 0;
#pragma unroll
    for (int w2 = 0; w2 < 16; ++w2) { const int32_t t = wave_total[w2]; if (w2 < wave) base += t; total += t; }
    int32_t o = base + incl - c;
    if (c) {
        for (int64_t r = r0; r < r1; ++r)
            if (flags[r]) { list[o++] = (int32_t)r; flags[r] = 0; }
    }
    const int32_t pad_end = (total + 15) / 16 * 16 + 16;
    for (int32_t k = total + tid; k < pad_end; k += 1024) list[k] = 0;
    if (tid == 0) *n_out = total;
}

constexpr int COLSUM_BLOCKS = 128;
constexpr int COLSUM_MAX_D = 64 * LLMREC_COLSUM_MAX_GROUPS;
__global__ __launch_bounds__(256) void colsum_partial_kernel(int64_t rows, int d, const float* __restrict__ X, int64_t ldx,
                                                             const float* __restrict__ w, float* __restrict__ partial) {
    float acc[COLSUM_MAX_D / 256] = {};
    for (int64_t r = blockIdx.x; r < rows; r += gridDim.x) {
        const float wr = w ? w[r] : 1.f;
        const float* row = X + r * ldx;
#pragma unroll
        for (int k = 0; k < COLSUM_MAX_D / 256; ++k) {
            const int c = k * 256 + threadIdx.x;
            if (c < d) acc[k] = fmaf(wr, row[c], acc[k]);
        }
    }
#pragma unroll
    for (int k = 0; k < COLSUM_MAX_D / 256; ++k) {
        const int c = k * 256 + threadIdx.x;
        if (c < d) partial[(int64_t)blockIdx.x * d + c] = acc[k];
    }
}
struct ColsumGroups { float* out[LLMREC_COLSUM_MAX_GROUPS]; int n_groups; };
__global__ __launch_bounds__(COLSUM_MAX_D) void colsum_final_kernel(int n_partial, int d, int gw, const float* __restrict__ partial, ColsumGroups g, int accumulate) {
    __shared__ float col[COLSUM_MAX_D];
    const int c = threadIdx.x;
    if (c < d) {
        const float* p = partial + c;
        float s0 = 0.f, s1 = 0.f, s2 = 0.f, s3 = 0.f;
        int b = 0;
        for (; b + 4 <= n_partial; b += 4) {
            s0 += p[(int64_t)b * d]; s1 += p[(int64_t)(b + 1) * d]; s2 += p[(int64_t)(b + 2) * d]; s3 += p[(int64_t)(b + 3) * d];
        }
        for (; b < n_partial; ++b) s0 += p[(int64_t)b * d];
        col[c] = (s0 + s1) + (s2 + s3);
    }
    __syncthreads();
    if (c >= gw) return;
    for (int q = 0; q < g.n_groups; ++q) {
        bool first = true;
        for (int e = 0; e < q; ++e) first = first && g.out[e] != g.out[q];
        float* o = g.out[q] + c;
        *o = (first && !accumulate) ? col[gw * q + c] : *o + col[gw * q + c];
    }
}

struct GatherTerms { const float* t[LLMREC_MAX_TERMS]; int64_t ld[LLMREC_MAX_TERMS]; int n; };

__global__ __launch_bounds__(256) void gather_mean_kernel(int64_t n, const int64_t* __restrict__ idx, int d, float scale, GatherTerms g,
                                                          float* __restrict__ out, int64_t ldo) {
    const int gl = threadIdx.x & 15;
    const int64_t b = (int64_t)blockIdx.x * 16 + (threadIdx.x >> 4);
    if (b >= n) return;
    const int64_t row = idx[b];
    for (int c = gl; c < d; c += 16) {
        float s = 0.f;
        for (int t = 0; t < g.n; ++t) s += g.t[t][row * g.ld[t] + c];
        out[b * ldo + c] = scale * s;
    }
}

extern "C" {

int llmrec_softmax_rows_fwd_f32(int64_t rows, int32_t d, const float* Z, int64_t ldz, float* Y, int64_t ldy,
                                llmrec_stream_t stream_) {
    hipStream_t stream = (hipStream_t)stream_;
    LLMREC_CHECK_ARG(rows >= 0 && d > 0, "softmax_fwd: bad sizes");
    if (rows == 0) return LLMREC_OK;
    LLMREC_CHECK_ARG(Z && Y && ldz >= d && ldy >= d, "softmax_fwd: null pointer or ld < d");
    const bool vec4 = d % 4 == 0 && ldz % 4 == 0 && ldy % 4 == 0 && aligned16(Z) && aligned16(Y);
    const int grid = grid_for(rows, ROWS_PER_BLOCK);
    int rc = dispatch_rows(d, vec4,
        [&](auto nc) { softmax_fwd_kernel<4, decltype(nc)::value><<<grid, 256, 0, stream>>>(rows, d, Z, ldz, Y, ldy); return 0; },
        [&](auto nc) { softmax_fwd_kernel<1, decltype(nc)::value><<<grid, 256, 0, stream>>>(rows, d, Z, ldz, Y, ldy); return 0; });
    if (rc) return rc;
    LLMREC_LAUNCH_CHECK();
    return LLMREC_OK;
}

int llmrec_softmax_rows_bwd_scaled_f32(int64_t rows, int32_t d, float alpha, const float* Y, int64_t ldy, const float* dY, int64_t lddy,
                                       float* dZ, int64_t lddz, llmrec_stream_t stream_) {
    hipStream_t stream = (hipStream_t)stream_;
    LLMREC_CHECK_ARG(rows >= 0 && d > 0, "softmax_bwd: bad sizes");
// ... 24 lines not shown
    if (rows == 0) return LLMREC_OK;
    LLMREC_CHECK_ARG(out && ldo >= d, "fuse_fwd: null out or ld < d");
    FuseArgs a = {};
    bool vec4 = d % 4 == 0 && ldo % 4 == 0 && aligned16(out);
    a.n_mean = n_mean; a.n_norm = n_norm; a.mean_scale = mean_scale;
    for (int i = 0; i < n_mean; ++i) {
        LLMREC_CHECK_ARG(mean_terms[i] && mean_ld[i] >= d, "fuse_fwd: bad mean term %d", i);
        a.mean_terms[i] = mean_terms[i]; a.mean_ld[i] = mean_ld[i];
        vec4 = vec4 && mean_ld[i] % 4 == 0 && aligned16(mean_terms[i]);
    }
    for (int i = 0; i < n_norm; ++i) {
        LLMREC_CHECK_ARG(norm_terms[i] && norm_ld[i] >= d, "fuse_fwd: bad norm term %d", i);
        a.norm_terms[i] = norm_terms[i]; a.norm_ld[i] = norm_ld[i]; a.rates[i] = rates[i];
        vec4 = vec4 && norm_ld[i] % 4 == 0 && aligned16(norm_terms[i]);
    }
    const int grid = grid_for(rows, ROWS_PER_BLOCK);
    int rc = dispatch_rows(d, vec4,
        [&](auto nc) { fuse_fwd_kernel<4, decltype(nc)::value><<<grid, 256, 0, stream>>>(rows, d, a, out, ldo); return 0; },
        [&](auto nc) { fuse_fwd_kernel<1, decltype(nc)::value><<<grid, 256, 0, stream>>>(rows, d, a, out, ldo); return 0; });
    if (rc) return rc;
    LLMREC_LAUNCH_CHECK();
    return LLMREC_OK;
}

static int fuse_bwd_impl(int64_t rows, int32_t d, const float* dOut, int64_t lddo,
                         int32_t n_norm, const float* const* norm_terms, const int64_t* norm_ld,
                         const float* rates, float* const* d_terms, const int64_t* d_ld,
                         const float* const* src_terms, const int64_t* src_ld,
                         int32_t accumulate, int32_t n_reg_terms, float reg_two_coef, llmrec_stream_t stream_);

int llmrec_fuse_bwd_f32(int64_t rows, int32_t d, const float* dOut, int64_t lddo,
                        int32_t n_norm, const float* const* norm_terms, const int64_t* norm_ld,
                        const float* rates, float* const* d_terms, const int64_t* d_ld,
                        int32_t accumulate, int32_t n_reg_terms, float reg_two_coef, llmrec_stream_t stream_) {
    return fuse_bwd_impl(rows, d, dOut, lddo, n_norm, norm_terms, norm_ld, rates, d_terms, d_ld, nullptr, nullptr, accumulate ? 1 : 0,
                         n_reg_terms, reg_two_coef, stream_);
}

int llmrec_fuse_bwd_src_f32(int64_t rows, int32_t d, const float* dOut, int64_t lddo,
                            int32_t n_norm, const float* const* norm_terms, const int64_t* norm_ld,
                            const float* rates, float* const* d_terms, const int64_t* d_ld,
                            const float* const* src_terms, const int64_t* src_ld,
                            int32_t n_reg_terms, float reg_two_coef, llmrec_stream_t stream_) {
    LLMREC_CHECK_ARG(src_terms && src_ld, "fuse_bwd_src: null source tables");
    return fuse_bwd_impl(rows, d, dOut, lddo, n_norm, norm_terms, norm_ld, rates, d_terms, d_ld, src_terms, src_ld, 2,
                         n_reg_terms, reg_two_coef, stream_);
}

static int fuse_bwd_impl(int64_t rows, int32_t d, const float* dOut, int64_t lddo,
                         int32_t n_norm, const float* const* norm_terms, const int64_t* norm_ld,
                         const float* rates, float* const* d_terms, const int64_t* d_ld,
                         const float* const* src_terms, const int64_t* src_ld,
                         int32_t accumulate, int32_t n_reg_terms, float reg_two_coef, llmrec_stream_t stream_) {
    hipStream_t stream = (hipStream_t)stream_;
    LLMREC_CHECK_ARG(rows >= 0 && d > 0 && n_norm >= 0 && n_norm <= LLMREC_MAX_TERMS && n_reg_terms >= 0 && n_reg_terms <= n_norm,
                     "fuse_bwd: bad sizes");
    if (rows == 0 || n_norm == 0) return LLMREC_OK;
    LLMREC_CHECK_ARG(dOut && lddo >= d, "fuse_bwd: null dOut or ld < d");
    FuseArgs a = {};
    bool vec4 = d % 4 == 0 && lddo % 4 == 0 && aligned16(dOut);
    a.n_norm = n_norm; a.n_reg = n_reg_terms; a.reg2 = reg_two_coef;
    for (int i = 0; i < n_norm; ++i) {
        LLMREC_CHECK_ARG(norm_terms[i] && d_terms[i] && norm_ld[i] >= d && d_ld[i] >= d, "fuse_bwd: bad term %d", i);
        a.norm_terms[i] = norm_terms[i]; a.norm_ld[i] = norm_ld[i]; a.rates[i] = rates[i];
        a.d_terms[i] = d_terms[i]; a.d_ld[i] = d_ld[i];
        a.s_terms[i] = src_terms ? src_terms[i] : nullptr; a.s_ld[i] = src_terms ? src_ld[i] : 0;
        LLMREC_CHECK_ARG(!a.s_terms[i] || a.s_ld[i] >= d, "fuse_bwd: source term %d has ld < d", i);
        vec4 = vec4 && norm_ld[i] % 4 == 0 && d_ld[i] % 4 == 0 && aligned16(norm_terms[i]) && aligned16(d_terms[i]) &&
               (!a.s_terms[i] || (a.s_ld[i] % 4 == 0 && aligned16(a.s_terms[i])));
    }
    const int grid = grid_for(rows, ROWS_PER_BLOCK);
    int rc = dispatch_rows(d, vec4,
        [&](auto nc) { fuse_bwd_kernel<4, decltype(nc)::value><<<grid, 256, 0, stream>>>(rows, d, a, dOut, lddo, accumulate); return 0; },
        [&](auto nc) { fuse_bwd_kernel<1, decltype(nc)::value><<<grid, 256, 0, stream>>>(rows, d, a, dOut, lddo, accumulate); return 0; });
    if (rc) return rc;
    LLMREC_LAUNCH_CHECK();
    return LLMREC_OK;
}

int llmrec_fuse_fwd_multi_f32(int32_t n_problems, const llmrec_fuse_fwd_problem_t* p, int32_t d, llmrec_stream_t stream_) {
    return llmrec_fuse_fwd_multi_sumsq_f32(n_problems, p, d, 0, nullptr, 0, nullptr, stream_);
}

int llmrec_fuse_fwd_multi_sumsq_f32(int32_t n_problems, const llmrec_fuse_fwd_problem_t* p, int32_t d, int32_t n_sumsq_terms,
                                    float* sumsq_partial, int32_t partial_capacity, int32_t* n_partial_host, llmrec_stream_t stream_) {
    hipStream_t stream = (hipStream_t)stream_;
    LLMREC_CHECK_ARG(n_problems >= 1 && n_problems <= FUSE_MAX_PROBLEMS && p && d > 0, "fuse_fwd_multi: 1..%d problems", FUSE_MAX_PROBLEMS);
    LLMREC_CHECK_ARG(n_sumsq_terms >= 0 && (n_sumsq_terms == 0 || (sumsq_partial && n_partial_host)), "fuse_fwd_multi: sum of squares without a partial buffer");
    FuseMulti m = {};
    bool vec4 = d % 4 == 0;
    int blocks[FUSE_MAX_PROBLEMS] = {0, 0};
    for (int k = 0; k < n_problems; ++k) {
        const llmrec_fuse_fwd_problem_t& q = p[k];
        LLMREC_CHECK_ARG(q.rows >= 0 && q.n_mean >= 0 && q.n_norm >= 0 && q.n_mean <= LLMREC_MAX_TERMS && q.n_norm <= LLMREC_MAX_TERMS,
                         "fuse_fwd_multi: problem %d has bad sizes", k);
        LLMREC_CHECK_ARG(q.rows == 0 || (q.out && q.ldo >= d), "fuse_fwd_multi: problem %d: null out or ld < d", k);
        FuseArgs& a = m.a[k];
        a.n_mean = q.n_mean; a.n_norm = q.n_norm; a.mean_scale = q.mean_scale;
        vec4 = vec4 && q.ldo % 4 == 0 && aligned16(q.out);
        for (int i = 0; i < q.n_mean; ++i) {
            LLMREC_CHECK_ARG(q.mean_terms[i] && q.mean_ld[i] >= d, "fuse_fwd_multi: problem %d: bad mean term %d", k, i);
            a.mean_terms[i] = q.mean_terms[i]; a.mean_ld[i] = q.mean_ld[i];
            vec4 = vec4 && q.mean_ld[i] % 4 == 0 && aligned16(q.mean_terms[i]);
        }
        for (int i = 0; i < q.n_norm; ++i) {
            LLMREC_CHECK_ARG(q.norm_terms[i] && q.norm_ld[i] >= d, "fuse_fwd_multi: problem %d: bad norm term %d", k, i);
            a.norm_terms[i] = q.norm_terms[i]; a.norm_ld[i] = q.norm_ld[i]; a.rates[i] = q.rates[i];
            vec4 = vec4 && q.norm_ld[i] % 4 == 0 && aligned16(q.norm_terms[i]);
        }
        m.rows[k] = q.rows; m.out[k] = q.out; m.ldo[k] = q.ldo;
        blocks[k] = q.rows > 0 ? grid_for(q.rows, ROWS_PER_BLOCK) : 0;
    }
    m.block_begin = blocks[0];
    const int grid = blocks[0] + blocks[1];
    if (n_sumsq_terms > 0) {
        for (int k = 0; k < n_problems; ++k) LLMREC_CHECK_ARG(n_sumsq_terms <= p[k].n_norm, "fuse_fwd_multi: problem %d has fewer than %d norm terms", k, n_sumsq_terms);
        if (grid > partial_capacity) { set_error("fuse_fwd_multi: %d partial sums > capacity %d", grid, partial_capacity); return LLMREC_EWORKSPACE; }
        *n_partial_host = grid;
        m.n_sumsq = n_sumsq_terms; m.sumsq_partial = sumsq_partial;
    }
    if (grid == 0) return LLMREC_OK;
    int rc = dispatch_rows(d, vec4,
        [&](auto nc) { fuse_fwd_multi_kernel<4, decltype(nc)::value><<<grid, 256, 0, stream>>>(d, m); return 0; },
        [&](auto nc) { fuse_fwd_multi_kernel<1, decltype(nc)::value><<<grid, 256, 0, stream>>>(d, m); return 0; });
    if (rc) return rc;
    LLMREC_LAUNCH_CHECK();
    return LLMREC_OK;
}

static int fill_fuse_bwd_multi(int32_t n_problems, const llmrec_fuse_bwd_problem_t* p, int32_t d, FuseMulti& m, bool& vec4, int& grid) {
    LLMREC_CHECK_ARG(n_problems >= 1 && n_problems <= FUSE_MAX_PROBLEMS && p && d > 0, "fuse_bwd_src_multi: 1..%d problems", FUSE_MAX_PROBLEMS);
    vec4 = d % 4 == 0;
    int blocks[FUSE_MAX_PROBLEMS] = {0, 0};
    for (int k = 0; k < n_problems; ++k) {
        const llmrec_fuse_bwd_problem_t& q = p[k];
        LLMREC_CHECK_ARG(q.rows >= 0 && q.n_norm >= 0 && q.n_norm <= LLMREC_MAX_TERMS && q.n_reg_terms >= 0 && q.n_reg_terms <= q.n_norm,
                         "fuse_bwd_src_multi: problem %d has bad sizes", k);
        if (q.rows == 0 || q.n_norm == 0) continue;
        LLMREC_CHECK_ARG(q.dOut && q.lddo >= d && q.src_terms && q.src_ld, "fuse_bwd_src_multi: problem %d: null pointer or ld < d", k);
        FuseArgs& a = m.a[k];
        a.n_norm = q.n_norm; a.n_reg = q.n_reg_terms; a.reg2 = q.reg_two_coef;
        vec4 = vec4 && q.lddo % 4 == 0 && aligned16(q.dOut);
        for (int i = 0; i < q.n_norm; ++i) {
            LLMREC_CHECK_ARG(q.norm_terms[i] && q.d_terms[i] && q.norm_ld[i] >= d && q.d_ld[i] >= d, "fuse_bwd_src_multi: problem %d: bad term %d", k, i);
            a.norm_terms[i] = q.norm_terms[i]; a.norm_ld[i] = q.norm_ld[i]; a.rates[i] = q.rates[i];
            a.d_terms[i] = q.d_terms[i]; a.d_ld[i] = q.d_ld[i];
            a.s_terms[i] = q.src_terms[i]; a.s_ld[i] = q.src_terms[i] ? q.src_ld[i] : 0;
            LLMREC_CHECK_ARG(!a.s_terms[i] || a.s_ld[i] >= d, "fuse_bwd_src_multi: problem %d: source term %d has ld < d", k, i);
            vec4 = vec4 && q.norm_ld[i] % 4 == 0 && q.d_ld[i] % 4 == 0 && aligned16(q.norm_terms[i]) && aligned16(q.d_terms[i]) &&
                   (!a.s_terms[i] || (a.s_ld[i] % 4 == 0 && aligned16(a.s_terms[i])));
        }
        m.rows[k] = q.rows; m.dOut[k] = q.dOut; m.lddo[k] = q.lddo; m.row_flags[k] = q.row_flags; m.row_stamp[k] = q.row_stamp;
        blocks[k] = grid_for(q.rows, ROWS_PER_BLOCK);
    }
    m.block_begin = blocks[0];
    grid = blocks[0] + blocks[1];
    return LLMREC_OK;
}

int llmrec_fuse_bwd_src_multi_f32(int32_t n_problems, const llmrec_fuse_bwd_problem_t* p, int32_t d, llmrec_stream_t stream_) {
    hipStream_t stream = (hipStream_t)stream_;
    FuseMulti m = {};
    bool vec4 = false;
    int grid = 0;
    if (int rc = fill_fuse_bwd_multi(n_problems, p, d, m, vec4, grid)) return rc;
    if (grid == 0) return LLMREC_OK;
    int rc = dispatch_rows(d, vec4,
        [&](auto nc) { fuse_bwd_src_multi_kernel<4, decltype(nc)::value><<<grid, 256, 0, stream>>>(d, m); return 0; },
        [&](auto nc) { fuse_bwd_src_multi_kernel<1, decltype(nc)::value><<<grid, 256, 0, stream>>>(d, m); return 0; });
    if (rc) return rc;
    LLMREC_LAUNCH_CHECK();
    return LLMREC_OK;
}

int64_t llmrec_sumsq_workspace_bytes(int64_t rows, int32_t d) {
    (void)rows; (void)d;
    return 4 * SUMSQ_BLOCKS;
}

int llmrec_sumsq_f32(int64_t rows, int32_t d, const float* X, int64_t ldx, float coef, int32_t accumulate,
                     float* out, void* workspace, int64_t workspace_bytes, llmrec_stream_t stream_) {
    hipStream_t stream = (hipStream_t)stream_;
    LLMREC_CHECK_ARG(rows >= 0 && d >= 0 && out, "sumsq: bad argument");
    LLMREC_CHECK_ARG(rows * d == 0 || (X && ldx >= d), "sumsq: null X or ld < d");
    if (workspace_bytes < 4 * SUMSQ_BLOCKS || !workspace) { set_error("sumsq: workspace too small"); return LLMREC_EWORKSPACE; }
    const int nb = rows * d == 0 ? 1 : grid_for(rows * d, 256 * 8, SUMSQ_BLOCKS);
    sumsq_partial_kernel<<<nb, 256, 0, stream>>>(rows, d > 0 ? d : 1, X, ldx, (float*)workspace);
    LLMREC_LAUNCH_CHECK();
    sumsq_final_kernel<<<1, 256, 0, stream>>>(nb, (const float*)workspace, coef, accumulate, out);
    LLMREC_LAUNCH_CHECK();
    return LLMREC_OK;
}

int llmrec_axpy_f32(int64_t rows, int32_t d, float alpha, const float* alpha_dev, const float* X, int64_t ldx,
                    float* Y, int64_t ldy, int32_t accumulate, llmrec_stream_t stream_) {
    hipStream_t stream = (hipStream_t)stream_;
    LLMREC_CHECK_ARG(rows >= 0 && d >= 0, "axpy: bad sizes");
    if (rows * d == 0) return LLMREC_OK;
    LLMREC_CHECK_ARG(X && Y && ldx >= d && ldy >= d, "axpy: null pointer or ld < d");
    axpy_kernel<<<grid_for(rows * d, 256 * 4), 256, 0, stream>>>(rows, d, alpha, alpha_dev, X, ldx, Y, ldy, accumulate);
    LLMREC_LAUNCH_CHECK();
    return LLMREC_OK;
}

int llmrec_adamw_advance(float* state3, float lr, float beta1, float beta2, llmrec_stream_t stream_) {
    LLMREC_CHECK_ARG(state3, "adamw_advance: null state");
    adamw_advance_kernel<<<1, 1, 0, (hipStream_t)stream_>>>(state3, lr, beta1, beta2);
    LLMREC_LAUNCH_CHECK();
    return LLMREC_OK;
}
// ... 81 lines not shown
    SoftmaxBwdArgs s = {};
    int sm_blocks = 0;
    bool sm_vec4 = true;
    if (sm_rows > 0) {
        LLMREC_CHECK_ARG(sm_d > 0 && sm_Y && sm_dY && sm_dZ && sm_ldy >= sm_d && sm_lddy >= sm_d && sm_lddz >= sm_d,
                         "step_rows_group: softmax backward: null pointer or ld < d");
        sm_vec4 = sm_d % 4 == 0 && sm_ldy % 4 == 0 && sm_lddy % 4 == 0 && sm_lddz % 4 == 0 && aligned16(sm_Y) && aligned16(sm_dY) && aligned16(sm_dZ);
        s.rows = sm_rows; s.d = sm_d; s.alpha = sm_alpha;
        s.Y = sm_Y; s.ldy = sm_ldy; s.dY = sm_dY; s.lddy = sm_lddy; s.dZ = sm_dZ; s.lddz = sm_lddz;
        sm_blocks = grid_for(sm_rows, ROWS_PER_BLOCK);
    }
    if ((fuse_blocks > 0 && !(fuse_vec4 && d <= 64)) || (sm_blocks > 0 && !(sm_vec4 && sm_d <= 64))) {
        set_error("step_rows_group: only the 16-byte, d <= 64 row kernels are grouped (fusion d = %d, softmax d = %d)", d, sm_d);
        return LLMREC_EUNSUPPORTED;
    }
    const int total = fuse_blocks + adamw_blocks + sm_blocks;
    if (total == 0) return LLMREC_OK;
    const float decay_mul = (float)(1.0 - (double)lr * (double)weight_decay);
    step_rows_group_kernel<<<total, 256, 0, (hipStream_t)stream_>>>(d, m, t, state3, decay_mul, beta1, beta2, eps, s, fuse_blocks,
                                                                    fuse_blocks + adamw_blocks);
    LLMREC_LAUNCH_CHECK();
    return LLMREC_OK;
}

int llmrec_zero_multi_f32(int32_t n_tensors, const llmrec_zero_tensor_t* tensors_host, llmrec_stream_t stream_) {
    LLMREC_CHECK_ARG(n_tensors >= 0 && n_tensors <= LLMREC_ZERO_MAX_TENSORS && (n_tensors == 0 || tensors_host),
                     "zero_multi: bad argument (at most %d tensors)", LLMREC_ZERO_MAX_TENSORS);
    ZeroTensors t = {};
    t.n_tensors = n_tensors;
    int64_t blocks = 0;
    for (int i = 0; i < n_tensors; ++i) {
        LLMREC_CHECK_ARG(tensors_host[i].n >= 0 && (tensors_host[i].n == 0 || tensors_host[i].p), "zero_multi: tensor %d has a null pointer", i);
        t.p[i] = tensors_host[i].p; t.n[i] = tensors_host[i].n;
        t.block_begin[i] = (int32_t)blocks;
        blocks += ceil_div(tensors_host[i].n, ZERO_PER_BLOCK);
        LLMREC_CHECK_ARG(blocks < 0x7fffffffll, "zero_multi: too many elements for one launch");
    }
    for (int i = n_tensors; i <= LLMREC_ZERO_MAX_TENSORS; ++i) t.block_begin[i] = (int32_t)blocks;
    if (blocks == 0) return LLMREC_OK;
    zero_multi_kernel<<<(unsigned)blocks, 256, 0, (hipStream_t)stream_>>>(t);
    LLMREC_LAUNCH_CHECK();
    return LLMREC_OK;
}

int llmrec_loss_assemble_f32(int32_t mode, int32_t n_problems, const float* bpr_out, const float* w_mf_host,
                             float* scal4, float* tail, float inv_world, double* running_sums3, llmrec_stream_t stream_) {
    LLMREC_CHECK_ARG(mode >= 0 && mode <= 2 && n_problems >= 1 && n_problems <= LLMREC_BPR_MAX_PROBLEMS, "loss_assemble: bad mode / problem count");
    LLMREC_CHECK_ARG(bpr_out && scal4 && (mode == 1 || w_mf_host) && (mode == 0 || tail), "loss_assemble: null pointer");
    LossWeights w = {};
    if (w_mf_host) for (int i = 0; i < n_problems; ++i) w.w[i] = w_mf_host[i];
    loss_assemble_kernel<<<1, 64, 0, (hipStream_t)stream_>>>(mode, n_problems, bpr_out, w, scal4, tail, inv_world, running_sums3);
    LLMREC_LAUNCH_CHECK();
    return LLMREC_OK;
}

int llmrec_scatter_set_rows_f32(int32_t capacity, const int32_t* row_list, const int32_t* n_list_dev, int32_t d, const float* src, int64_t lds_,
                                float* dst, int64_t ldd, llmrec_stream_t stream_) {
    LLMREC_CHECK_ARG(capacity >= 0 && d > 0, "scatter_set_rows: bad sizes");
    if (capacity == 0) return LLMREC_OK;
    LLMREC_CHECK_ARG(row_list && n_list_dev && src && dst && lds_ >= d && ldd >= d, "scatter_set_rows: null pointer or ld < d");
    scatter_set_rows_kernel<<<(unsigned)ceil_div(capacity, 16), 256, 0, (hipStream_t)stream_>>>(capacity, row_list, n_list_dev, d, src, lds_, dst, ldd);
    LLMREC_LAUNCH_CHECK();
    return LLMREC_OK;
}

int llmrec_mark_rows_u8(int64_t n, const int64_t* ids, int32_t value, uint8_t* flags, llmrec_stream_t stream_) {
    LLMREC_CHECK_ARG(n >= 0 && value >= 0 && value <= 255, "mark_rows: bad argument");
    if (n == 0) return LLMREC_OK;
    LLMREC_CHECK_ARG(ids && flags, "mark_rows: null pointer");
    LLMREC_CHECK_ARG(n / 256 < 0x7fffffffll, "mark_rows: too many rows for one launch");
    mark_rows_kernel<<<(unsigned)ceil_div(n, 256), 256, 0, (hipStream_t)stream_>>>(n, ids, (uint8_t)value, flags);
    LLMREC_LAUNCH_CHECK();
    return LLMREC_OK;
}

int llmrec_batch_reach_rows(int64_t n_users, int64_t n_items, const int64_t* users, const int64_t* pos, const int64_t* neg, int32_t B_cap,
                            const int32_t* n_valid, const int32_t* item_rowptr, const int32_t* item_colidx, uint8_t* flags,
                            int32_t* row_list, int32_t* n_rows, llmrec_stream_t stream_) {
    LLMREC_CHECK_ARG(n_users > 0 && n_users < 0x7fffffffll && n_items > 0 && B_cap >= 0, "batch_reach_rows: bad sizes");
    LLMREC_CHECK_ARG(users && pos && neg && item_rowptr && item_colidx && flags && row_list && n_rows, "batch_reach_rows: null pointer");
    LLMREC_CHECK_ARG((uintptr_t)flags % 16 == 0, "batch_reach_rows: flags must be 16-byte aligned (and readable up to n_users rounded up to 16 bytes)");
    hipStream_t stream = (hipStream_t)stream_;
    if (B_cap > 0) {
        batch_reach_mark_kernel<<<(unsigned)ceil_div(3 * (int64_t)B_cap * REACH_SPLIT, 4), 256, 0, stream>>>(B_cap, n_valid, users, pos, neg, n_users, n_items,
                                                                                                item_rowptr, item_colidx, flags);
        LLMREC_LAUNCH_CHECK();
    }
    flags_compact_kernel<<<1, 1024, 0, stream>>>(n_users, flags, row_list, n_rows);
    LLMREC_LAUNCH_CHECK();
    return LLMREC_OK;
}

int llmrec_softmax_rows_bwd_listed_f32(int64_t n, const int64_t* ids, int32_t d, float alpha, const float* Y, int64_t ldy,
                                       const float* dY, int64_t lddy, const float* post_scale, float* dZ, int64_t lddz,
                                       llmrec_stream_t stream_) {
    LLMREC_CHECK_ARG(n >= 0 && d > 0, "softmax_bwd_listed: bad sizes");
    if (n == 0) return LLMREC_OK;
    LLMREC_CHECK_ARG(ids && Y && dY && dZ && ldy >= d && lddy >= d && lddz >= d, "softmax_bwd_listed: null pointer or ld < d");
    softmax_bwd_listed_kernel<<<(unsigned)ceil_div(n, 16), 256, 0, (hipStream_t)stream_>>>(n, ids, d, alpha, Y, ldy, dY, lddy, post_scale, dZ, lddz);
    LLMREC_LAUNCH_CHECK();
    return LLMREC_OK;
}

int llmrec_mark_neighbours_u8(int64_t n, const int64_t* ids, const int32_t* rowptr, const int32_t* colidx, int32_t value, uint8_t* flags,
                              llmrec_stream_t stream_) {
    LLMREC_CHECK_ARG(n >= 0 && value >= 0 && value <= 255, "mark_neighbours: bad argument");
    if (n == 0) return LLMREC_OK;
    LLMREC_CHECK_ARG(ids && rowptr && colidx && flags, "mark_neighbours: null pointer");
    LLMREC_CHECK_ARG(n * MARK_SPLIT / 4 < 0x7fffffffll, "mark_neighbours: too many rows for one launch");
    mark_neighbours_kernel<<<(unsigned)ceil_div(n * MARK_SPLIT, 4), 256, 0, (hipStream_t)stream_>>>(n, ids, rowptr, colidx, (uint8_t)value, flags);
    LLMREC_LAUNCH_CHECK();
    return LLMREC_OK;
}

int llmrec_scale_rows_f32(int64_t rows, int32_t d, const float* s, const float* X, int64_t ldx, float* Y, int64_t ldy,
                          llmrec_stream_t stream_) {
    LLMREC_CHECK_ARG(rows >= 0 && d >= 0, "scale_rows: bad sizes");
    if (rows * d == 0) return LLMREC_OK;
    LLMREC_CHECK_ARG(s && X && Y && ldx >= d && ldy >= d, "scale_rows: null pointer or ld < d");
    scale_rows_kernel<<<grid_for(rows * d, 256 * 4), 256, 0, (hipStream_t)stream_>>>(rows, d, s, X, ldx, Y, ldy);
    LLMREC_LAUNCH_CHECK();
    return LLMREC_OK;
}

int llmrec_gather_mean_f32(int64_t n, const int64_t* idx, int32_t d, float scale, int32_t n_terms,
                           const float* const* terms, const int64_t* term_ld, float* out, int64_t ldo, llmrec_stream_t stream_) {
    LLMREC_CHECK_ARG(n >= 0 && d > 0 && n_terms >= 1 && n_terms <= LLMREC_MAX_TERMS, "gather_mean: bad sizes");
    if (n == 0) return LLMREC_OK;
    LLMREC_CHECK_ARG(idx && terms && term_ld && out && ldo >= d, "gather_mean: null pointer or ld < d");
    GatherTerms g = {};
    g.n = n_terms;
    for (int t = 0; t < n_terms; ++t) {
        LLMREC_CHECK_ARG(terms[t] && term_ld[t] >= d, "gather_mean: bad term %d", t);
        g.t[t] = terms[t]; g.ld[t] = term_ld[t];
    }
    gather_mean_kernel<<<(unsigned)ceil_div(n, 16), 256, 0, (hipStream_t)stream_>>>(n, idx, d, scale, g, out, ldo);
    LLMREC_LAUNCH_CHECK();
    return LLMREC_OK;
}

int llmrec_zero_rows_f32(int64_t n, const int64_t* ids, int32_t d, float* dst, int64_t ldd, llmrec_stream_t stream_) {
    LLMREC_CHECK_ARG(n >= 0 && d > 0, "zero_rows: bad sizes");
    if (n == 0) return LLMREC_OK;
    LLMREC_CHECK_ARG(ids && dst && ldd >= d, "zero_rows: null pointer or ld < d");
    zero_rows_kernel<<<(unsigned)ceil_div(n, 16), 256, 0, (hipStream_t)stream_>>>(n, ids, d, dst, ldd);
    LLMREC_LAUNCH_CHECK();
    return LLMREC_OK;
}

int64_t llmrec_weighted_colsum_workspace_bytes(int32_t d) {
    if (d <= 0 || d > COLSUM_MAX_D) return -1;
    return (int64_t)sizeof(float) * COLSUM_BLOCKS * d;
}

int llmrec_weighted_colsum_f32(int64_t rows, int32_t n_groups, int32_t group_width, const float* X, int64_t ldx, const float* w,
                               float* const* group_out_host, int32_t accumulate,
                               void* workspace, int64_t workspace_bytes, llmrec_stream_t stream_) {
    LLMREC_CHECK_ARG(rows >= 0 && n_groups >= 1 && n_groups <= LLMREC_COLSUM_MAX_GROUPS && group_width >= 1 && group_width <= 64,
                     "weighted_colsum: 1..%d groups of 1..64 columns", LLMREC_COLSUM_MAX_GROUPS);
    const int32_t d = n_groups * group_width;
    LLMREC_CHECK_ARG(group_out_host && (rows == 0 || (X && ldx >= d)), "weighted_colsum: null pointer or ld < d");
    if (!workspace || workspace_bytes < llmrec_weighted_colsum_workspace_bytes(d)) {
        set_error("weighted_colsum: workspace %lld < %lld", (long long)workspace_bytes, (long long)llmrec_weighted_colsum_workspace_bytes(d));
        return LLMREC_EWORKSPACE;
    }
    ColsumGroups g = {};
    g.n_groups = n_groups;
// ... 30 lines not shown
```

llmrec_amd/engine.py:

```python
from __future__ import annotations

from dataclasses import dataclass
from typing import Optional

import torch

from . import ops


@dataclass
class Hyper:
    batch_size: int = 1024
    decay: float = 1e-5
    feat_reg_decay: float = 1e-5
    aug_mf_rate: float = 0.012
    mm_mf_rate: float = 0.0001
    prune_loss_drop_rate: float = 0.71
    aug_sample_rate: float = 0.1

    @staticmethod
    def from_args(args) -> "Hyper":
        return Hyper(batch_size=args.batch_size, decay=eval(args.regs)[0], feat_reg_decay=args.feat_reg_decay,
                     aug_mf_rate=args.aug_mf_rate, mm_mf_rate=args.mm_mf_rate,
                     prune_loss_drop_rate=args.prune_loss_drop_rate, aug_sample_rate=args.aug_sample_rate)


def bpr(hp: Hyper, user_table, item_table, users, pos, neg, n_valid=None):
    out = ops.bpr_prune(user_table, item_table, users, pos, neg, hp.prune_loss_drop_rate, hp.decay, hp.batch_size, n_valid)
    return out[0], out[1]


def step_loss(hp: Hyper, fw, users, pos, neg, n_items: int, n_valid=None, on_bpr=None):
    (e_u, e_i, img_i, txt_i, img_u, txt_u, _p_usr, _att_i_dup, prof_u, _prof_i, _att_u, att_i, _im, _um) = fw
    record = on_bpr or (lambda *a: None)
    mf, emb = bpr(hp, e_u, e_i, users, pos, neg, n_valid)
    record(mf, emb)
    img_mf, e1 = bpr(hp, img_u, img_i, users, pos, neg, n_valid)
    record(img_mf, e1)
    txt_mf, e2 = bpr(hp, txt_u, txt_i, users, pos, neg, n_valid)
    record(txt_mf, e2)
    aug_mf = 0
    for key in att_i:
        a_mf, e = bpr(hp, prof_u, att_i[key], users, pos, neg, n_valid)
        record(a_mf, e)
        aug_mf = aug_mf + a_mf
    feat_reg = ops.sumsq(hp.feat_reg_decay * 0.5 / n_items, [img_i, txt_i, img_u, txt_u])[0]
    loss = mf + emb + feat_reg + hp.aug_mf_rate * aug_mf + hp.mm_mf_rate * (img_mf + txt_mf)
    return loss, mf, emb


def train_step(model, optimizer, ui, iu, users, pos, neg, hp: Hyper, n_valid=None, on_bpr=None, extra_loss=None):
    model.train()
    fw = model(ui, iu, ui, iu, ui, iu)
    loss, mf, emb = step_loss(hp, fw, users, pos, neg, model.n_items, n_valid, on_bpr)
    if extra_loss is not None:
        loss = loss + extra_loss(fw)
    optimizer.zero_grad()
    loss.backward()
    optimizer.step()
    return loss.detach(), mf.detach(), emb.detach()


class DeviceBatcher:

    def __init__(self, train: ops.Csr, exist_users: torch.Tensor, n_items: int, batch_size: int,
                 aug_pos: Optional[torch.Tensor], aug_neg: Optional[torch.Tensor], aug_rate: float, seed: int,
                 rank: int = 0, world: int = 1):
        self.train, self.exist_users, self.n_items, self.B = train, exist_users, n_items, batch_size
        self.rank, self.world = rank, world
        self.aug_pos, self.aug_neg = aug_pos, aug_neg
        self.n_aug = int(batch_size * aug_rate) if aug_pos is not None else 0
        self.seed = seed
        self.capacity = self.B + self.n_aug
        self.step_dev = torch.zeros(1, dtype=torch.int64, device=exist_users.device)

    def fill(self, users, pos, neg, n_valid):
        ops.sample_batch(self.seed, self.step_dev, self.exist_users, self.n_items, self.train, self.B * self.world,
                         self.rank * self.B, self.B, self.n_aug, self.aug_pos, self.aug_neg, users, pos, neg, n_valid)

    def next(self, step: Optional[int] = None):
        dev = self.exist_users.device
        if step is not None:
            self.step_dev.fill_(int(step))
        u, p, n = (torch.empty(self.capacity, dtype=torch.int64, device=dev) for _ in range(3))
        nv = torch.empty(1, dtype=torch.int32, device=dev)
        self.fill(u, p, n, nv)
        return u, p, n, nv


@torch.no_grad()
def evaluate_topk(model, ui, iu, query_users: torch.Tensor, train: ops.Csr, k: int):
    model.eval()
    fw = model(ui, iu, ui, iu, ui, iu)
    return ops.score_topk(fw[0], fw[1], query_users, train, k)
```

llmrec_amd/fused.py:

```python
from __future__ import annotations

import ctypes
import os
from typing import List, Optional

import torch

from . import _lib, ops
from .engine import Hyper

_p, _ld, _c = ops._p, ops._ld, ctypes


def _call(name, *a):
    _lib.call(name, *a, ops._stream())


class _capture_without_gc:

    def __init__(self, graph, multi_branch: bool):
        from . import require_graph_replay
        require_graph_replay("llmrec_amd: stream capture", multi_branch)
        self.ctx = torch.cuda.graph(graph, capture_error_mode="thread_local")

# ... 23 lines not shown

    def __init__(self, model, graph, hp: Hyper, rates, optimizer: ops.FusedAdamW, b_max: int):
        self.m, self.hp, self.opt = model, hp, optimizer
        self.ui, self.iu = graph.ui, graph.iu
        self.U, self.I = model.n_users, model.n_items
        self.d = d = model.embedding_dim
        self.L = model.n_ui_layers
        self.keys = list(model.item_feats.keys())
        self.S = S = 2 + len(self.keys)
        self.c_m, self.c_u, self.c_a = rates
        self.b_max = b_max
        dev = model.item_id_embedding.weight.device
        f = lambda *s: torch.empty(*s, dtype=torch.float32, device=dev)
        U, I = self.U, self.I
        self.U_cat, self.I_cat = f(U, S * d), f(I, S * d)
        self.P_usr, self.prof_i, self.prof_u = f(U, d), f(I, d), f(U, d)
        self.Ul = [f(U, d) for _ in range(self.L)]
        self.Il = [f(I, d) for _ in range(self.L)]
        self.E_u, self.E_i = f(U, d), f(I, d)
        self.check_zero = os.environ.get("LLMREC_CHECK_ZERO", "0") == "1"
        z = lambda *s: torch.zeros(*s, dtype=torch.float32, device=dev)
        self.dE_u, self.dE_i = z(U, d), z(I, d)
        self.sc_U, self.sc_I, self.sc_prof = z(U, 2 * d), z(I, S * d), z(U, d)
        self.flag_u = torch.zeros(U, dtype=torch.uint8, device=dev)
        self.flag_i = torch.zeros(I, dtype=torch.uint8, device=dev)
        self.row_stamp = torch.zeros(1, dtype=torch.int32, device=dev)
        self.bpr_plan = torch.zeros(max(ops.bpr_plan_words(b_max), 1), dtype=torch.int64, device=dev)
        self.epoch_sums = torch.zeros(3, dtype=torch.float64, device=dev)
        self.dU_cat, self.dI_cat = f(U, S * d), f(I, S * d)
        self.dprof_u, self.dprof_i, self.dP_usr = f(U, d), f(I, d), f(U, d)
        self.bufU, self.bufI, self.tmpU, self.tmpI = f(U, d), f(I, d), f(U, d), f(I, d)
        self.out = f(8, 2)
        self.saved = f(8 * ops.bpr_saved_floats(b_max))
        self.scal = f(4)
        self.ws_sumsq = torch.empty(_lib.query("llmrec_sumsq_workspace_bytes", 0, 0), dtype=torch.uint8, device=dev)
        feats = [model.image_feats, model.text_feats, model.user_feats] + [model.item_feats[k] for k in self.keys]
        ws = max(_lib.query("llmrec_linear_wgrad_workspace_bytes", x.shape[0] * (len(self.keys) if i >= 3 else 1), d, x.shape[1])
                 for i, x in enumerate(feats))
        self.ws_wgrad = torch.empty(ws, dtype=torch.uint8, device=dev)
        wsq = lambda x: torch.empty(_lib.query("llmrec_linear_wgrad_workspace_bytes", x.shape[0], d, x.shape[1]), dtype=torch.uint8, device=dev)
        self.ws_wgrad_b, self.ws_wgrad_c, self.ws_wgrad_d = wsq(model.user_feats), wsq(model.text_feats), wsq(model.image_feats)
        self.ws_wgrad_multi = None
        self._partials = {}
        self.multi_stream = os.environ.get("LLMREC_STREAMS", "0") == "1"
        self.s1, self.s2, self.s3 = (torch.cuda.Stream(device=dev) for _ in range(3))
        for p in model.parameters():
            if p.requires_grad and p.grad is None and p is not model.batch_norm.weight and p is not model.batch_norm.bias:
                p.grad = torch.zeros_like(p)
        self.w_mf = [1.0, hp.mm_mf_rate, hp.mm_mf_rate] + [hp.aug_mf_rate] * len(self.keys)
        self.w_emb = [1.0] + [0.0] * (S)
        self.n_prob = 1 + S
        if self.n_prob > _lib.CONST["LLMREC_BPR_MAX_PROBLEMS"]:
            raise RuntimeError("FusedStep: %d BPR problems exceed LLMREC_BPR_MAX_PROBLEMS" % self.n_prob)
        self.w_mf_dev = torch.tensor(self.w_mf, dtype=torch.float32, device=dev)
        self.graph_exec = None
        self.static = None
        self._eval_graphs = {}
        self.stamps = None
        self.spmm_edge_units = 0.0
        self.gemm = os.environ.get("LLMREC_GEMM", "bf16x3")
        want = os.environ.get("LLMREC_PREPROPAGATE", "auto")
        self.preprop = d <= 64 and (want == "1" or (want not in ("0", "1") and U <= I))
        if not self.preprop:
            self.P_cat, self.dP_cat = f(I, S * d), f(I, S * d)
        if self.preprop:
            item_feats = [model.image_feats, model.text_feats] + [model.item_feats[k] for k in self.keys]
            self.AX = [self._propagate_constant(self.ui.fwd, x) for x in item_feats]
            self.a_rowsum = ops.spmm_raw(self.ui.fwd, torch.ones(I, 4, dtype=torch.float32, device=dev))[:, 0].contiguous()
            self.ws_colsum = torch.empty(_lib.query("llmrec_weighted_colsum_workspace_bytes", S * d), dtype=torch.uint8, device=dev)
        self.wgrad_rows = (getattr(type(self), "WGRAD_ROWS", True) and os.environ.get("LLMREC_WGRAD_ROWS", "1") == "1" and self.preprop
                           and len(self.keys) > 0 and self.gemm == "bf16x3")
        if self.wgrad_rows:
            self.act_flags = torch.zeros(U + 16, dtype=torch.uint8, device=dev)[:U]
            self.act_rows = torch.zeros(U + 32, dtype=torch.int32, device=dev)
            self.act_n = torch.zeros(1, dtype=torch.int32, device=dev)
            self.act_expected = None
        self.inline_adamw = getattr(type(self), "INLINE_ADAMW", True)
        self.fold = getattr(type(self), "FOLD", True) and os.environ.get("LLMREC_FOLD", "1") == "1" and self.inline_adamw
        if self.fold:
            self.ss_cap = 2 * 2048
            self.ss_partial = torch.zeros(self.ss_cap, dtype=torch.float32, device=dev)
            self.ss_n = 0
        self._ev_plan = self._ev_reach = None
        self._zero_in_forward = False
        self._emb_params = [model.user_id_embedding.weight, model.item_id_embedding.weight]
        self._lin_params = [p for p in optimizer.params if p.grad is not None and all(p is not e for e in self._emb_params)]

    @staticmethod
    def _propagate_constant(a: ops.Csr, X: torch.Tensor) -> torch.Tensor:
        X = X.detach()
        out = torch.empty(a.n_rows, X.shape[1], dtype=torch.float32, device=X.device)
        step = 64 if X.shape[1] % 64 == 0 else X.shape[1]
        for c0 in range(0, X.shape[1], step):
            ops.spmm_raw(a, X[:, c0:c0 + step], out=out[:, c0:c0 + step])
        return out

    def _fork(self, *streams):
        if self.multi_stream:
            cur = torch.cuda.current_stream()
            for st in streams:
                st.wait_stream(cur)

    def _mark(self):
        if not self.multi_stream:
            return None
        ev = torch.cuda.Event()
        ev.record(torch.cuda.current_stream())
        return ev

    def _fork_from(self, ev, *streams):
        if self.multi_stream:
            for st in streams:
                st.wait_event(ev)

    def _join(self, *streams):
        if self.multi_stream:
            cur = torch.cuda.current_stream()
            for st in streams:
                cur.wait_stream(st)

    def _on(self, st):
        return torch.cuda.stream(st) if self.multi_stream else torch.cuda.stream(torch.cuda.current_stream())

    STAMP_SLOTS = 6

    def _stamp(self, slot: int):
        if self.stamps is not None:
            _call("llmrec_timestamp", self.stamps.data_ptr() + 8 * slot)

    def _spmm_args(self, a: ops.Csr, X, Y, accumulate=False, tag=0, epilogue=None):
        d = X.shape[1]
        sw, pl = a.plan_for(d, whole_row=epilogue is not None and epilogue.op != ops.EPI_NONE)
        partials = None
        if pl.n_seg:
            key = (id(pl), d, tag)
            partials = self._partials.get(key)
            if partials is None:
                partials = self._partials[key] = torch.empty(pl.n_seg * d, dtype=torch.float32, device=X.device)
        if accumulate:
            epilogue = ops.spmm_epilogue(ops.EPI_NONE, 1.0, Y)
        return sw, pl, partials, epilogue

    def _spmm(self, a: ops.Csr, X, Y, accumulate=False, tag=0, epilogue=None):
        d = X.shape[1]
        self.spmm_edge_units += a.nnz * (d / 64.0)
        sw, pl, partials, epilogue = self._spmm_args(a, X, Y, accumulate, tag, epilogue)
        rp, ci = pl.csr_of(a)
        _call("llmrec_spmm_f32", a.n_rows, a.n_cols, _p(rp), _p(ci), _p(a.val), _p(a.row_scale), _p(a.col_scale),
              _p(X), _ld(X), _p(Y), _ld(Y), d, sw, _c.byref(pl.c_struct()), _p(partials),
              _c.byref(epilogue) if epilogue is not None else None)

    def _spmm_jobs(self, jobs):
        for a, X, Y, kw in jobs:
            self._spmm(a, X, Y, **kw)

    def _spmm_group(self, jobs):
        jobs = [j for j in jobs if j is not None]
        if len(jobs) == 1 or self.multi_stream or any(a.nnz >= ops.SPMM_LATENCY_NNZ for a, _, _, _ in jobs):
            return self._spmm_jobs(jobs)
        order = sorted(jobs, key=lambda j: -j[0].nnz * j[1].shape[1])
        probs, keep = [], []
        for a, X, Y, kw in order:
            sw, pl, partials, epi = self._spmm_args(a, X, Y, **kw)
            rp, ci = pl.csr_of(a)
            pc = pl.c_struct()
            keep.append(epi)
# ... 23 lines not shown

    def wgrad_targets(self, dY_cat, dP_usr):
        m = self.m
        if self.preprop:
            feats, roww = self.AX, self.a_rowsum
        else:
            feats, roww = [m.image_feats, m.text_feats] + [m.item_feats[key] for key in self.keys], None
        rows = (self.act_rows, self.act_n, self.act_expected) if self.wgrad_rows else None
        item_pairs = [(self._side(dY_cat, 2 + k), feats[2 + k], roww, rows) for k in range(len(self.keys))]
        return [(item_pairs, m.item_trans.weight.grad, m.item_trans.bias.grad, False),
                ([(dP_usr, m.user_feats)], m.user_trans.weight.grad, m.user_trans.bias.grad, False),
                ([(self._side(dY_cat, 1), feats[1], roww)], m.text_trans.weight.grad, m.text_trans.bias.grad, False),
                ([(self._side(dY_cat, 0), feats[0], roww)], m.image_trans.weight.grad, m.image_trans.bias.grad, False)]

    def _project_all(self):
        jobs = self.projection_jobs()
        if self.d > 64 or len(jobs) > _lib.CONST["LLMREC_LINEAR_MAX_PROBLEMS"]:
            if self.preprop:
                raise RuntimeError("FusedStep: the pre-propagated projection needs the grouped launch (d <= 64); set LLMREC_PREPROPAGATE=0")
            for X, lin, out, _ in jobs:
                self._linear(X, lin, out)
            return
        arr = (ops.LinearProblem * len(jobs))()
        for i, (X, lin, out, bscale) in enumerate(jobs):
            arr[i].X, arr[i].ldx, arr[i].M, arr[i].K = X.data_ptr(), _ld(X), X.shape[0], X.shape[1]
            arr[i].W, arr[i].ldw, arr[i].bias = lin.weight.data_ptr(), _ld(lin.weight), lin.bias.data_ptr()
            arr[i].Y, arr[i].ldy = out.data_ptr(), _ld(out)
            arr[i].bias_scale = bscale.data_ptr() if bscale is not None else None
        _call("llmrec_linear_fwd_grouped_bf16x3" if self.gemm == "bf16x3" else "llmrec_linear_fwd_grouped_f32", len(jobs), arr, self.d)

    def _wgrad(self, dY, X, lin, accumulate, ws=None):
        ops.linear_wgrad_grouped([(dY, X)], lin.weight.grad, lin.bias.grad, accumulate, self.ws_wgrad if ws is None else ws,
                                 precision=self.gemm)

    def _softmax(self, Z, Y):
        _call("llmrec_softmax_rows_fwd_f32", Z.shape[0], self.d, _p(Z), _ld(Z), _p(Y), _ld(Y))

    def _softmax_bwd(self, Y, dY, dZ, alpha: float = 1.0):
        _call("llmrec_softmax_rows_bwd_scaled_f32", Y.shape[0], self.d, float(alpha), _p(Y), _ld(Y), _p(dY), _ld(dY), _p(dZ), _ld(dZ))

    def _axpy(self, alpha, X, Y, accumulate, rows=None, cols=None):
        rows = X.shape[0] if rows is None else rows
        cols = X.shape[1] if cols is None else cols
        _call("llmrec_axpy_f32", rows, cols, float(alpha), None, _p(X), _ld(X), _p(Y), _ld(Y), 1 if accumulate else 0)

    @staticmethod
    def _tables(ts):
        return (_c.c_void_p * len(ts))(*[t.data_ptr() for t in ts]), (_c.c_int64 * len(ts))(*[_ld(t) for t in ts])

    def _side(self, cat, s):
        return cat[:, s * self.d:(s + 1) * self.d]

    def _norm_terms(self, cat, prof):
        return [self._side(cat, 0), self._side(cat, 1), prof] + [self._side(cat, 2 + k) for k in range(len(self.keys))]

    def _rates(self):
        r = [self.c_m, self.c_m, self.c_u] + [self.c_a] * len(self.keys)
        return (_c.c_float * len(r))(*r)

    def forward(self, sampler=None, after_chain=None, profile_on_main: bool = False):
        m, d = self.m, self.d
        if self.multi_stream:
            self._forward_streams(sampler, after_chain, profile_on_main)
        else:
            self._forward_one_stream(sampler, after_chain)

        keep = []

        def problem(pr, out, base, layers, cat, prof):
            means, norms = [base] + layers, self._norm_terms(cat, prof)
            mp, ml = self._tables(means)
            npt, nl = self._tables(norms)
            rates = self._rates()
            keep.extend((mp, ml, npt, nl, rates))
            pr.rows, pr.mean_scale, pr.n_mean, pr.n_norm = out.shape[0], 1.0 / len(means), len(means), len(norms)
            pr.mean_terms, pr.mean_ld = _c.cast(mp, _c.c_void_p), _c.cast(ml, _c.c_void_p)
            pr.norm_terms, pr.norm_ld, pr.rates = _c.cast(npt, _c.c_void_p), _c.cast(nl, _c.c_void_p), _c.cast(rates, _c.c_void_p)
            pr.out, pr.ldo = out.data_ptr(), _ld(out)
        arr = (ops.FuseFwdProblem * 2)()
        problem(arr[0], self.E_i, m.item_id_embedding.weight, self.Il, self.I_cat, self.prof_i)
        problem(arr[1], self.E_u, m.user_id_embedding.weight, self.Ul, self.U_cat, self.prof_u)
        if self.fold and self._zero_in_forward:
            n_part = _c.c_int32(0)
            _call("llmrec_fuse_fwd_multi_sumsq_f32", 2, arr, d, 2, _p(self.ss_partial), self.ss_cap, _c.byref(n_part))
            self.ss_n = int(n_part.value)
        else:
            _call("llmrec_fuse_fwd_multi_f32", 2, arr, d)

    def _chain_fwd_jobs(self):
        jobs, i_prev = [], self.m.item_id_embedding.weight
        for l in range(self.L):
            kw = dict(tag=2, epilogue=ops.spmm_epilogue(ops.EPI_SOFTMAX)) if l == self.L - 1 else dict(tag=2)
            jobs.append((self.ui.fwd, i_prev, self.Ul[l], kw))
            jobs.append((self.iu.fwd, self.Ul[l], self.Il[l], dict(kw)))
            i_prev = self.Il[l]
        return jobs

    def _forward_one_stream(self, sampler, after_chain):
        if sampler is not None:
            sampler()
        if self._zero_in_forward and not self.fold:
            self.opt.advance()
        if after_chain is not None:
            after_chain()
        self._stamp(1)
        self._project_all()
        self._stamp(2)
        side = [(self.ui.fwd, self.P_cat, self.U_cat, {})] if not self.preprop else []
        side.append((self.iu.fwd, self.U_cat, self.I_cat, {}))
        prof = [(self.iu.fwd, self.P_usr, self.prof_i, dict(tag=1)), (self.ui.fwd, self.prof_i, self.prof_u, dict(tag=1))]
        chain = self._chain_fwd_jobs()
        for k in range(max(len(chain), len(side), len(prof))):
            self._spmm_group([c[k] if k < len(c) else None for c in (chain, side, prof)])
        if self._zero_in_forward and not self.fold:
            self._feat_reg()

    def _forward_streams(self, sampler, after_chain, profile_on_main):
        self._fork(self.s2)
        with self._on(self.s2):
            if sampler is not None:
                sampler()
            if self._zero_in_forward and not self.fold:
                self.opt.advance()
            self._spmm_jobs(self._chain_fwd_jobs())
            ev_chain = self._mark() if after_chain is not None else None
            if after_chain is not None:
                after_chain()
        self._stamp(1)
        self._project_all()
        self._stamp(2)
        ev1 = self._mark()
        if not self.preprop:
            self._spmm(self.ui.fwd, self.P_cat, self.U_cat)
        self._spmm(self.iu.fwd, self.U_cat, self.I_cat)
        if profile_on_main:
            self._spmm(self.iu.fwd, self.P_usr, self.prof_i, tag=1)
            self._spmm(self.ui.fwd, self.prof_i, self.prof_u, tag=1)
        else:
            self._fork_from(ev1, self.s1)
            with self._on(self.s1):
                self._spmm(self.iu.fwd, self.P_usr, self.prof_i, tag=1)
                self._spmm(self.ui.fwd, self.prof_i, self.prof_u, tag=1)
        if self._zero_in_forward and not self.fold:
            self._fork(self.s3)
            with self._on(self.s3):
                self._feat_reg()
        if ev_chain is not None:
            self._join(self.s1)
            torch.cuda.current_stream().wait_event(ev_chain)
        else:
            self._join(self.s1, self.s2)

    def outputs(self):
        att_i = {k: self._side(self.I_cat, 2 + j) for j, k in enumerate(self.keys)}
        att_u = {k: self._side(self.U_cat, 2 + j) for j, k in enumerate(self.keys)}
        return (self.E_u, self.E_i, self._side(self.I_cat, 0), self._side(self.I_cat, 1), self._side(self.U_cat, 0),
                self._side(self.U_cat, 1), self.P_usr, att_i, self.prof_u, self.prof_i, att_u, att_i, None, None)

    def _problems(self):
        arr = (ops.BprProblem * self.n_prob)()
        tabs = [(self.E_u, self.E_i, self.dE_u, self.dE_i)]
        tU, tI, tP = self.sc_U, self.sc_I, self.sc_prof
        for s in range(2):
            tabs.append((self._side(self.U_cat, s), self._side(self.I_cat, s), self._side(tU, s), self._side(tI, s)))
        for k in range(len(self.keys)):
            tabs.append((self.prof_u, self._side(self.I_cat, 2 + k), tP, self._side(tI, 2 + k)))
        for i, (eu, ei, deu, dei) in enumerate(tabs):
# ... 174 lines not shown
        main_first, loss_s3 = self.fold, self.fold and side_work is not None
        if main_first:
            self._spmm_jobs(side)
            self._fork_from(ev_fuse, self.s1)
        else:
            self._fork(self.s1)
        if loss_s3:
            self._fork_from(ev_rows, self.s3)
            with self._on(self.s3):
                side_work()
            side_work = None
        with self._on(self.s1):
            self._spmm_jobs(prof)
            if self.gemm != "bf16x3":
                self._wgrad(self.dP_usr, self.m.user_feats, self.m.user_trans, False, ws=self.ws_wgrad_b)
        self._fork_from(ev_rows, self.s2)
        with self._on(self.s2):
            self._chain_head(side_work)
            self._spmm_jobs(self._chain_bwd_jobs())
            self._chain_tail(probs, batch, ev_fuse)
        if not main_first:
            self._spmm_jobs(side)

    def _weight_gradients(self):
        m, S, d = self.m, self.S, self.d
        dY_cat = self.dU_cat if self.preprop else self.dP_cat
        targets = self.wgrad_targets(dY_cat, self.dP_usr)
        item_pairs, text_pairs, image_pairs = targets[0][0], targets[2][0], targets[3][0]
        done, updated = False, []
        if self.gemm == "bf16x3":
            self._join(self.s1)
            if self.ws_wgrad_multi is None:
                need = ops.linear_wgrad_multi_workspace(targets, self.wgrad_blocks)
                self.ws_wgrad_multi = torch.empty(max(need, 0), dtype=torch.uint8, device=dY_cat.device) if need >= 0 else False
            if self.ws_wgrad_multi is not False:
                self._stamp(3)
                if self._ev_reach is not None:
                    torch.cuda.current_stream().wait_event(self._ev_reach)
                lins = (m.item_trans, m.user_trans, m.text_trans, m.image_trans)
                if self.inline_adamw:
                    ops.linear_wgrad_multi(targets, self.ws_wgrad_multi, update=(self.opt, [(l.weight, l.bias) for l in lins]), block_budget=self.wgrad_blocks)
                    updated = [p_ for l in lins for p_ in (l.weight, l.bias)]
                else:
                    ops.linear_wgrad_multi(targets, self.ws_wgrad_multi, block_budget=self.wgrad_blocks)
                self._stamp(4)
                done = True
            else:
                self._wgrad(self.dP_usr, m.user_feats, m.user_trans, False, ws=self.ws_wgrad_b)
        if not done:
            strip = lambda pairs: [p_[:2] for p_ in pairs]
            bias = (lambda lin: None) if self.preprop else (lambda lin: lin.bias.grad)
            if self.preprop:
                outs = [m.image_trans.bias.grad, m.text_trans.bias.grad] + [m.item_trans.bias.grad] * len(self.keys)
                gp = (_c.c_void_p * S)(*[t.data_ptr() for t in outs])
                _call("llmrec_weighted_colsum_f32", self.U, S, d, _p(dY_cat), _ld(dY_cat), _p(self.a_rowsum), gp, 0, _p(self.ws_colsum), self.ws_colsum.numel())
            ops.linear_wgrad_grouped(strip(item_pairs), m.item_trans.weight.grad, bias(m.item_trans), False, self.ws_wgrad, precision=self.gemm)
            ops.linear_wgrad_grouped(strip(text_pairs), m.text_trans.weight.grad, bias(m.text_trans), False, self.ws_wgrad_c, precision=self.gemm)
            ops.linear_wgrad_grouped(strip(image_pairs), m.image_trans.weight.grad, bias(m.image_trans), False, self.ws_wgrad_d, precision=self.gemm)
        self._join(self.s1)
        if self.inline_adamw:
            self.opt.step_params([p_ for p_ in self._lin_params if all(p_ is not q for q in updated)])

    def _train_forward(self, sampler=None, after_chain=None):
        self._zero_in_forward = True
        try:
            self.forward(sampler, after_chain)
        finally:
            self._zero_in_forward = False

    def build_scatter_plan(self, users, pos, neg, n_valid=None):
        B = users.numel()
        if B > self.b_max:
            raise RuntimeError("FusedStep: batch of %d exceeds b_max %d" % (B, self.b_max))
        _call("llmrec_bpr_scatter_plan", _p(users), _p(pos), _p(neg), B, _p(n_valid), _p(self.bpr_plan))

    def reset_scatter_targets(self):
        for t in (self.dE_u, self.dE_i, self.sc_U, self.sc_I, self.sc_prof):
            t.zero_()

    def step_eager(self, users, pos, neg, n_valid=None, sampler=None):
        self._ev_plan = self._ev_reach = None

        def batch_lists():
            self.build_scatter_plan(users, pos, neg, n_valid)
            self._ev_plan = self._mark()
            if self.wgrad_rows:
                ops.batch_reach_rows(users, pos, neg, n_valid, self.iu.fwd, self.act_flags, self.act_rows, self.act_n)
                self._ev_reach = self._mark()
        self.spmm_edge_units = 0.0
        calls0 = _lib.n_calls
        try:
            self._stamp(0)
            if self.multi_stream:
                self._train_forward(sampler, batch_lists)
            else:
                if sampler is not None:
                    sampler()
                batch_lists()
                self._train_forward()
            self.loss_backward(users, pos, neg, n_valid)
            if not self.inline_adamw:
                self.opt.step(advanced=True)
            self._stamp(5)
            self.entry_point_calls_per_step = _lib.n_calls - calls0 - (2 if self.stamps is not None else 0) * 3
            if self.wgrad_rows and self.act_expected is None and not torch.cuda.is_current_stream_capturing():
                self._size_wgrad_for_rows()
        except Exception:
            if not torch.cuda.is_current_stream_capturing():
                try:
                    self.reset_scatter_targets()
                except Exception:
                    pass
            raise
        return self.scal[1], self.scal[2], self.scal[3]

    def _size_wgrad_for_rows(self):
        n = int(self.act_n.item())
        self.act_expected = max(64, min(self.U, int(n * 1.10) + 32))
        need = ops.linear_wgrad_multi_workspace(self.wgrad_targets(self.dU_cat if self.preprop else self.dP_cat, self.dP_usr), self.wgrad_blocks)
        self.ws_wgrad_multi = torch.empty(max(need, 0), dtype=torch.uint8, device=self.dP_usr.device) if need >= 0 else False

    def check_wgrad_geometry(self, factor: float = 1.5) -> bool:
        if not self.wgrad_rows or self.act_expected is None or torch.cuda.is_current_stream_capturing():
            return False
        want = max(64, min(self.U, int(int(self.act_n.item()) * 1.10) + 32))
        if self.act_expected / factor <= want <= self.act_expected * factor:
            return False
        self._size_wgrad_for_rows()
        if self.graph_exec is not None and getattr(self, "_capture_args", None) is not None:
            self.capture(warm=False, **self._capture_args)
        return True

    def flush(self):
        """Nothing is deferred in the single-graph step (DataParallelStep defers its AdamW)."""

    def eval_topk(self, query_users: torch.Tensor, train: Optional[ops.Csr], K: int, use_graph: bool = False, held=None, Ks=None,
                  auc: bool = False):
        if auc and (not use_graph or held is None):
            raise RuntimeError("FusedStep.eval_topk: auc=True needs use_graph=True and the held-out rows")
        if not use_graph:
            self.forward()
            return ops.score_topk(self.E_u, self.E_i, query_users, train, K)
        Ks = tuple(int(k) for k in Ks) if held is not None else None
        key = (query_users.data_ptr(), query_users.numel(), K, id(train), None if held is None else (held[0].data_ptr(), Ks), bool(auc))
        ev = self._eval_graphs.get(key)
        if ev is None:
            q = query_users.to(torch.int64).contiguous()
            n = q.numel()
            idx = torch.empty(n, K, dtype=torch.int32, device=q.device)
            sc = torch.empty(n, K, dtype=torch.float32, device=q.device)
            wide = K > _lib.CONST["LLMREC_TOPK_MAX"]
            nnz = ops._wide_train_nnz(train, q) if wide else 0
            ws = ops.topk_workspace(n, self.I, q.device, self.d, K, nnz)
            sums = sums_ws = None
            if held is not None:
                sums = torch.zeros(4, len(Ks), dtype=torch.float64).pin_memory()
                sums_ws = torch.empty(_lib.query("llmrec_topk_eval_sums_workspace_bytes", n, len(Ks)), dtype=torch.uint8, device=q.device)
            auc_sum = auc_ws = None
            if auc:
                auc_sum = torch.zeros(1, dtype=torch.float64).pin_memory()
                auc_ws = ops.auc_workspace(n, self.I, q.device, self.d)

            def run():
                self.forward(profile_on_main=True)
                if wide:
                    _call("llmrec_score_topk_wide_f32", n, _p(q), _p(self.E_u), _ld(self.E_u), _p(self.E_i), _ld(self.E_i), self.I, self.d,
                          _p(train.rowptr) if train is not None else None, _p(train.colidx) if train is not None else None,
                          K, _p(idx), _p(sc), _p(ws), ws.numel(), ops.topk_wide_mode(None, self.I, self.d, K), nnz)
                else:
                    _call("llmrec_score_topk_mode_f32", n, _p(q), _p(self.E_u), _ld(self.E_u), _p(self.E_i), _ld(self.E_i), self.I, self.d,
                          _p(train.rowptr) if train is not None else None, _p(train.colidx) if train is not None else None,
                          K, _p(idx), _p(sc), _p(ws), ws.numel() if ws is not None else 0, ops.topk_mode(None, self.I, self.d, K))
                if held is not None:
                    ops.topk_eval_sums(idx, q, held[0], held[1], Ks, out=sums, ws=sums_ws)
                if auc:
                    _call("llmrec_score_auc_f32", n, _p(q), _p(self.E_u), _ld(self.E_u), _p(self.E_i), _ld(self.E_i), self.I, self.d,
                          _p(train.rowptr) if train is not None else None, _p(train.colidx) if train is not None else None,
                          _p(held[0]), _p(held[1]), None, None, _c.c_void_p(auc_sum.data_ptr()), _p(auc_ws), auc_ws.numel())
            side = torch.cuda.Stream()
            side.wait_stream(torch.cuda.current_stream())
            with torch.cuda.stream(side):
                run()
            torch.cuda.current_stream().wait_stream(side)
            torch.cuda.synchronize()
            g = torch.cuda.CUDAGraph()
            with _capture_without_gc(g, self.multi_stream):
                run()
            ev = self._eval_graphs[key] = (g, idx, sc, q, train, ws, sums, sums_ws, held, auc_sum, auc_ws)
        ev[0].replay()
        self._last_eval = ev
        return ev[1], ev[2]

# ... 102 lines not shown
```

llmrec_amd/ops.py:

```python
from __future__ import annotations

import ctypes
import os
import weakref
from dataclasses import dataclass
from typing import List, Optional, Sequence

import torch

from . import _lib

CONST = _lib.CONST
_c = ctypes


def _stream():
    return _c.c_void_p(torch.cuda.current_stream().cuda_stream)


def _p(t: Optional[torch.Tensor]):
    return None if t is None else _c.c_void_p(t.data_ptr())


def _ptr(t: Optional[torch.Tensor]):
# ... 968 lines not shown


def scores(Eu, Ei, query_users: torch.Tensor):
    _need_gpu(Eu, Ei, query_users)
    Eu, Ei = _rowmajor(Eu.detach()), _rowmajor(Ei.detach())
    q = query_users.to(torch.int64).contiguous()
    S = torch.empty(q.numel(), Ei.shape[0], dtype=torch.float32, device=Eu.device)
    _lib.call("llmrec_scores_f32", q.numel(), _p(q), _p(Eu), _ld(Eu), _p(Ei), _ld(Ei), Ei.shape[0], Eu.shape[1], _p(S), _ld(S), _stream())
    return S


def topk_hits(topk_idx: torch.Tensor, query_users: torch.Tensor, test_rowptr: torch.Tensor, test_colidx: torch.Tensor):
    q = query_users.to(torch.int64).contiguous()
    hits = torch.empty(topk_idx.shape, dtype=torch.uint8, device=topk_idx.device)
    _lib.call("llmrec_topk_hits", q.numel(), _p(q), topk_idx.shape[1], _p(topk_idx), _p(test_rowptr), _p(test_colidx), _p(hits), _stream())
    return hits


def topk_eval_sums(idx: torch.Tensor, query_users: torch.Tensor, test_rowptr: torch.Tensor, test_colidx: torch.Tensor, Ks,
                   out: Optional[torch.Tensor] = None, ws: Optional[torch.Tensor] = None) -> torch.Tensor:
    _need_gpu(idx, query_users, test_rowptr, test_colidx)
    n, K = idx.shape
    Ks = [int(k) for k in Ks]
    if out is None:
        out = torch.empty(4, len(Ks), dtype=torch.float64, device=idx.device)
    need = _lib.query("llmrec_topk_eval_sums_workspace_bytes", n, len(Ks))
    if ws is None or ws.numel() < need:
        ws = torch.empty(need, dtype=torch.uint8, device=idx.device)
    arr = (_c.c_int32 * len(Ks))(*Ks)
    _lib.call("llmrec_topk_eval_sums", n, _p(query_users.to(torch.int64).contiguous()), K, _p(idx.contiguous()), _p(test_rowptr), _p(test_colidx),
              len(Ks), arr, _p(ws), ws.numel(), _c.c_void_p(out.data_ptr()), _stream())
    return out


def _rows(csr):
    return (csr.rowptr, csr.colidx) if hasattr(csr, "rowptr") else (csr[0], csr[1])


def auc_workspace(n_query: int, n_items: int, device, d: int = 64) -> torch.Tensor:
    return torch.empty(_lib.query("llmrec_score_auc_workspace_bytes", n_query, n_items, d), dtype=torch.uint8, device=device)


def score_auc(Eu, Ei, query_users: torch.Tensor, train, held, counts: bool = False, out: Optional[torch.Tensor] = None,
              ws: Optional[torch.Tensor] = None):
    _need_gpu(Eu, Ei, query_users)
    Eu, Ei = _rowmajor(Eu.detach()), _rowmajor(Ei.detach())
    q = query_users.to(torch.int64).contiguous()
    n, I, d = q.numel(), Ei.shape[0], Eu.shape[1]
    hr, hc = _rows(held)
    tr, tc = _rows(train) if train is not None else (None, None)
    _need_gpu(hr, hc, tr, tc)
    if out is not None and (out.dtype != torch.float64 or out.numel() < 1):
        raise RuntimeError("score_auc: out must be a float64 tensor of one element")
    need = _lib.query("llmrec_score_auc_workspace_bytes", n, I, d)
    if ws is None or ws.numel() < need:
        ws = auc_workspace(n, I, Eu.device, d)
    auc = torch.empty(n, dtype=torch.float64, device=Eu.device)
    cnt = torch.empty(n, 3, dtype=torch.int64, device=Eu.device) if counts else None
    _lib.call("llmrec_score_auc_f32", n, _p(q), _p(Eu), _ld(Eu), _p(Ei), _ld(Ei), I, d, _p(tr), _p(tc), _p(hr), _p(hc),
              _p(auc), _p(cnt), _c.c_void_p(out.data_ptr()) if out is not None else None, _p(ws), ws.numel(), _stream())
    return (auc, cnt) if counts else auc


def sample_bpr(seed: int, step: int, exist_users: torch.Tensor, n_items: int, train: Csr, B: int):
    dev = exist_users.device
    u = torch.empty(B, dtype=torch.int64, device=dev)
    p = torch.empty(B, dtype=torch.int64, device=dev)
    n = torch.empty(B, dtype=torch.int64, device=dev)
    _lib.call("llmrec_sample_bpr", seed, step, exist_users.numel(), _p(exist_users), n_items, _p(train.rowptr), _p(train.colidx),
              B, _p(u), _p(p), _p(n), _stream())
    return u, p, n


def sample_batch(seed: int, step_dev: torch.Tensor, exist_users: torch.Tensor, n_items: int, train: Csr, B_global: int,
                 slice_begin: int, B: int, n_aug: int, aug_pos: Optional[torch.Tensor], aug_neg: Optional[torch.Tensor],
                 users: torch.Tensor, pos: torch.Tensor, neg: torch.Tensor, n_valid: torch.Tensor):
    _need_gpu(step_dev, exist_users, users, pos, neg, n_valid)
    if users.numel() < B + n_aug or step_dev.dtype != torch.int64 or n_valid.dtype != torch.int32:
        raise RuntimeError("sample_batch: buffers of B + n_aug int64 entries, int64 step counter, int32 n_valid expected")
    _lib.call("llmrec_sample_batch", seed, _p(step_dev), exist_users.numel(), _p(exist_users), n_items, _p(train.rowptr), _p(train.colidx),
              B_global, slice_begin, B, n_aug, _p(aug_pos), _p(aug_neg), _p(users), _p(pos), _p(neg), _p(n_valid), _stream())


def topk_metrics(idx: torch.Tensor, hits: torch.Tensor, query_users: torch.Tensor, test_rowptr: torch.Tensor, Ks) -> torch.Tensor:
    _need_gpu(idx, hits, query_users, test_rowptr)
    n, K = idx.shape
    Ks = [int(k) for k in Ks]
    out = torch.empty(n, 4, len(Ks), dtype=torch.float64, device=idx.device)
    arr = (_c.c_int32 * len(Ks))(*Ks)
    _lib.call("llmrec_topk_metrics", n, _p(query_users.to(torch.int64).contiguous()), K, _p(hits.contiguous()), _p(idx.contiguous()),
              _p(test_rowptr), len(Ks), arr, _p(out), _stream())
    return out
```

Measured before the change: 1.870 million.

## Fuse plan with reach marking, compact fwd rows, widen sampler, wave-parallel loss assembly

Several changes aimed at cutting launches and serial work per training step. The scatter-plan kernel and the batch-reach-mark kernel are merged into one launch. Row compaction is folded into the fused forward sumsq kernel. A multi-block sampler advances the step counter through an atomic ticket. The loss-assembly kernel now reduces each column with a per-wave register tree instead of block-wide shared-memory passes. These changes add complexity: the step counter now depends on a ticket counter being reset correctly, and the reach marking is deferred to the forward pass.

Result: faster. 1.993 million (median of 6 runs) (+6.6%).

```diff
diff --git a/include/llmrec_hip.h b/include/llmrec_hip.h
--- a/include/llmrec_hip.h
+++ b/include/llmrec_hip.h
@@ -176,6 +176,9 @@
 int llmrec_fuse_fwd_multi_f32(int32_t n_problems, const llmrec_fuse_fwd_problem_t* problems_host, int32_t d, llmrec_stream_t stream);
 int llmrec_fuse_fwd_multi_sumsq_f32(int32_t n_problems, const llmrec_fuse_fwd_problem_t* problems_host, int32_t d, int32_t n_sumsq_terms,
                                     float* sumsq_partial, int32_t partial_capacity, int32_t* n_partial_host, llmrec_stream_t stream);
+int llmrec_fuse_fwd_multi_sumsq_compact_f32(int32_t n_problems, const llmrec_fuse_fwd_problem_t* problems_host, int32_t d, int32_t n_sumsq_terms,
+                                            float* sumsq_partial, int32_t partial_capacity, int32_t* n_partial_host,
+                                            int64_t n_users, uint8_t* flags, int32_t* row_list, int32_t* n_rows, llmrec_stream_t stream);
 typedef struct {
     int64_t rows; const float* dOut; int64_t lddo;
     int32_t n_norm; const float* const* norm_terms; const int64_t* norm_ld; const float* rates;
@@ -220,6 +223,9 @@
 #define LLMREC_BPR_PLAN_WORDS(B) (5 * (B))
 int llmrec_bpr_scatter_plan(const int64_t* users, const int64_t* pos, const int64_t* neg, int32_t B_max, const int32_t* n_valid_dev,
                             uint64_t* plan, llmrec_stream_t stream);
+int llmrec_bpr_scatter_plan_reach_mark(const int64_t* users, const int64_t* pos, const int64_t* neg, int32_t B_max, const int32_t* n_valid_dev,
+                                       uint64_t* plan, int64_t n_users, int64_t n_items, const int32_t* item_rowptr,
+                                       const int32_t* item_colidx, uint8_t* flags, llmrec_stream_t stream);
 int llmrec_bpr_multi_bwd_f32(int32_t n_problems, const llmrec_bpr_problem_t* problems_host, int32_t d,
                              const int64_t* users, const int64_t* pos, const int64_t* neg,
                              int32_t B_max, const int32_t* n_valid_dev, float decay, float batch_size_flag,
@@ -379,6 +385,11 @@
                         int32_t B_global, int32_t slice_begin, int32_t B, int32_t n_aug,
                         const int64_t* aug_pos, const int64_t* aug_neg,
                         int64_t* users, int64_t* pos, int64_t* neg, int32_t* n_valid_dev, llmrec_stream_t stream);
+int llmrec_sample_batch_wide(uint64_t seed, uint64_t* step_dev, int64_t n_exist_users, const int64_t* exist_users,
+                             int64_t n_items, const int32_t* train_rowptr, const int32_t* train_colidx,
+                             int32_t B_global, int32_t slice_begin, int32_t B, int32_t n_aug,
+                             const int64_t* aug_pos, const int64_t* aug_neg,
+                             int64_t* users, int64_t* pos, int64_t* neg, int32_t* n_valid_dev, int32_t* ticket, llmrec_stream_t stream);
 
 int llmrec_timestamp(uint64_t* slot, llmrec_stream_t stream);
 int64_t llmrec_timestamp_rate_hz(void);
diff --git a/llmrec_amd/csrc/bpr.hip b/llmrec_amd/csrc/bpr.hip
--- a/llmrec_amd/csrc/bpr.hip
+++ b/llmrec_amd/csrc/bpr.hip
@@ -1,4 +1,5 @@
 #include "common.h"
+#include "reach.h"
 
 namespace llmrec {
 
@@ -191,57 +192,75 @@
 }
 
 struct LossW { float w[LLMREC_BPR_MAX_PROBLEMS]; };
-constexpr int LA_GROUP = BPR_THREADS / LLMREC_BPR_MAX_PROBLEMS;
+constexpr int LA_WAVES = BPR_THREADS / 64;
+constexpr int LA_TREES = 4 * LLMREC_BPR_MAX_PROBLEMS + 1;
+__device__ __forceinline__ float wave_tree_sum_1024(const float* __restrict__ src, int n, int lane) {
+    float r[16];
+#pragma unroll
+    for (int j = 0; j < 16; ++j) r[j] = 0.f;
+    for (int base = 0; base < n; base += BPR_THREADS) {
+        float x[16];
+#pragma unroll
+        for (int j = 0; j < 16; ++j) { const int b = base + lane + 64 * j; x[j] = b < n ? src[b] : 0.f; }
+#pragma unroll
+        for (int j = 0; j < 16; ++j) { const int b = base + lane + 64 * j; if (b < n) r[j] += x[j]; }
+    }
+#pragma unroll
+    for (int h = 8; h > 0; h >>= 1) {
+#pragma unroll
+        for (int j = 0; j < h; ++j) r[j] += r[j + h];
+    }
+    float x = r[0];
+#pragma unroll
+    for (int off = 32; off > 0; off >>= 1) x += __shfl_down(x, off, 64);
+    return x;
+}
+
 __global__ __launch_bounds__(BPR_THREADS) void bpr_losses_assemble_kernel(int n_prob, int B_max, const int32_t* __restrict__ n_valid_dev,
                                                                           double remember_rate, float decay, float bsz,
                                                                           float* __restrict__ out_all, float* __restrict__ saved_all, int saved_stride,
                                                                           LossW w, const float* __restrict__ partial, int n_partial, float reg_coef,
                                                                           float* __restrict__ scal, double* __restrict__ running) {
-    __shared__ float red[LLMREC_BPR_MAX_PROBLEMS][BPR_THREADS];
-    __shared__ float outs[LLMREC_BPR_MAX_PROBLEMS][2];
+    __shared__ float tot_s[LA_TREES];
     const int B = bpr_batch(n_valid_dev, B_max);
-    const int prob = threadIdx.x / LA_GROUP, t = threadIdx.x % LA_GROUP;
-    const bool live = prob < n_prob;
-    float* saved = saved_all + (int64_t)(live ? prob : 0) * saved_stride;
-    const float* sc = saved + B_max + 4;
-    float tot[4] = {0.f, 0.f, 0.f, 0.f};
-#pragma unroll
-    for (int col = 0; col < 4; ++col) {
-        const float* src = sc + (int64_t)(col + 1) * B_max;
-        if (live) {
-            for (int v = t; v < BPR_THREADS; v += LA_GROUP) {
-                float s_ = 0.f;
-                for (int b = v; b < B; b += BPR_THREADS) s_ += src[b];
-                red[prob][v] = s_;
-            }
-        }
-        __syncthreads();
-        for (int off = BPR_THREADS / 2; off > 0; off >>= 1) {
-            if (live) for (int i = t; i < off; i += LA_GROUP) red[prob][i] += red[prob][i + off];
-            __syncthreads();
-        }
-        tot[col] = red[live ? prob : 0][0];
-        __syncthreads();
-    }
-    if (live && t == 0) {
+    const int lane = threadIdx.x & 63, wv = threadIdx.x >> 6;
+    const int n_trees = 4 * n_prob + (partial ? 1 : 0);
+    for (int tr = wv; tr < n_trees; tr += LA_WAVES) {
+        const int tree = partial ? (tr == 0 ? 4 * n_prob : tr - 1) : tr;
+        float x;
+        if (tree == 4 * n_prob) {
+            x = wave_tree_sum_1024(partial, n_partial, lane);
+        } else {
+            const int prob = tree >> 2, col = tree & 3;
+            x = wave_tree_sum_1024(saved_all + (int64_t)prob * saved_stride + B_max + 4 + (int64_t)(col + 1) * B_max, B, lane);
+        }
+        if (lane == 0) tot_s[tree] = x;
+    }
+    __syncthreads();
+    if (wv != 0) return;
+    float mf = 0.f, emb = 0.f;
+    if (lane < n_prob) {
+        const int prob = lane;
+        float* saved = saved_all + (int64_t)prob * saved_stride;
+        float tot[4];
+#pragma unroll
+        for (int c = 0; c < 4; ++c) tot[c] = tot_s[4 * prob + c];
         const int k = (int)(remember_rate * (double)B);
-        const float mf = -(tot[0] / (float)k);
+        mf = -(tot[0] / (float)k);
         const float reg = 1.0f / (2.0f * tot[1] + 1e-8f) + 1.0f / (2.0f * tot[2] + 1e-8f) + 1.0f / (2.0f * tot[3] + 1e-8f);
-        const float emb = decay * (reg / bsz);
+        emb = decay * (reg / bsz);
         out_all[prob * 2 + 0] = mf; out_all[prob * 2 + 1] = emb;
-        outs[prob][0] = mf; outs[prob][1] = emb;
         saved[B_max + 0] = tot[1]; saved[B_max + 1] = tot[2]; saved[B_max + 2] = tot[3]; saved[B_max + 3] = (float)k;
     }
+    float outs[LLMREC_BPR_MAX_PROBLEMS][2];
+#pragma unroll
+    for (int p = 0; p < LLMREC_BPR_MAX_PROBLEMS; ++p) { outs[p][0] = __shfl(mf, p, 64); outs[p][1] = __shfl(emb, p, 64); }
+    if (lane != 0) return;
     float feat = scal[0];
-    if (partial) {
-        float s_ = 0.f;
-        for (int i = threadIdx.x; i < n_partial; i += BPR_THREADS) s_ += partial[i];
-        feat = reg_coef * block_tree_sum(s_, red[0]);
-    }
-    __syncthreads();
-    if (threadIdx.x != 0) return;
+    if (partial) feat = reg_coef * tot_s[4 * n_prob];
     float s = 0.f;
-    for (int p = 0; p < n_prob; ++p) s += outs[p][0] * w.w[p];
+#pragma unroll
+    for (int p = 0; p < LLMREC_BPR_MAX_PROBLEMS; ++p) if (p < n_prob) s += outs[p][0] * w.w[p];
     scal[0] = feat;
     scal[2] = outs[0][0]; scal[3] = outs[0][1];
     scal[1] = s + outs[0][1] + feat;
@@ -268,14 +287,12 @@
 }
 
 constexpr uint32_t PLAN_NO_ID = 0xffffffffu;
-__global__ __launch_bounds__(256) void bpr_plan_kernel(const int64_t* __restrict__ users, const int64_t* __restrict__ pos,
-                                                       const int64_t* __restrict__ neg, int B_max,
-                                                       const int32_t* __restrict__ n_valid_dev, uint64_t* __restrict__ plan) {
-    extern __shared__ __attribute__((aligned(16))) char smem[];
-    uint64_t* k = reinterpret_cast<uint64_t*>(smem);
+__device__ __forceinline__ void bpr_plan_block(int vb, uint64_t* k, const int64_t* __restrict__ users, const int64_t* __restrict__ pos,
+                                               const int64_t* __restrict__ neg, int B_max,
+                                               const int32_t* __restrict__ n_valid_dev, uint64_t* __restrict__ plan) {
     const int B = bpr_batch(n_valid_dev, B_max);
     const int nbu = (B_max + 15) / 16;
-    const bool items = (int)blockIdx.x >= nbu;
+    const bool items = vb >= nbu;
     const int n = items ? 2 * B_max : B_max;
     for (int i = threadIdx.x; i < n; i += 256) {
         const int b = (items && i >= B_max) ? i - B_max : i;
@@ -285,7 +302,7 @@
     }
     __syncthreads();
     const int gl = threadIdx.x & 15;
-    const int i = ((int)blockIdx.x - (items ? nbu : 0)) * 16 + (threadIdx.x >> 4);
+    const int i = (vb - (items ? nbu : 0)) * 16 + (threadIdx.x >> 4);
     if (i >= n) return;
     const uint64_t me = k[i];
     const uint32_t id = (uint32_t)(me >> 32);
@@ -302,6 +319,26 @@
         int32_t* runlen = reinterpret_cast<int32_t*>(plan + 3 * (int64_t)B_max);
         runlen[base + below] = (below == lower_id && id != PLAN_NO_ID) ? same_id : 0;
     }
+}
+
+__global__ __launch_bounds__(256) void bpr_plan_kernel(const int64_t* __restrict__ users, const int64_t* __restrict__ pos,
+                                                       const int64_t* __restrict__ neg, int B_max,
+                                                       const int32_t* __restrict__ n_valid_dev, uint64_t* __restrict__ plan) {
+    extern __shared__ __attribute__((aligned(16))) char smem[];
+    bpr_plan_block((int)blockIdx.x, reinterpret_cast<uint64_t*>(smem), users, pos, neg, B_max, n_valid_dev, plan);
+}
+
+__global__ __launch_bounds__(256) void bpr_plan_reach_mark_kernel(const int64_t* __restrict__ users, const int64_t* __restrict__ pos,
+                                                                  const int64_t* __restrict__ neg, int B_max,
+                                                                  const int32_t* __restrict__ n_valid_dev, uint64_t* __restrict__ plan,
+                                                                  int plan_blocks, int64_t n_users, int64_t n_items,
+                                                                  const int32_t* __restrict__ item_rowptr, const int32_t* __restrict__ item_colidx,
+                                                                  uint8_t* __restrict__ flags) {
+    extern __shared__ __attribute__((aligned(16))) char smem[];
+    if ((int)blockIdx.x < plan_blocks)
+        bpr_plan_block((int)blockIdx.x, reinterpret_cast<uint64_t*>(smem), users, pos, neg, B_max, n_valid_dev, plan);
+    else
+        batch_reach_mark_block((int)blockIdx.x - plan_blocks, B_max, n_valid_dev, users, pos, neg, n_users, n_items, item_rowptr, item_colidx, flags);
 }
 
 constexpr int RUN_MAX_SHARE = LLMREC_BPR_MAX_PROBLEMS;
@@ -611,10 +648,8 @@
     return x;
 }
 
-__device__ __forceinline__ void sample_one(const Philox& ph, uint32_t slo, uint32_t shi, int b, int B, int half_bits,
-                                           int64_t n_exist, const int64_t* __restrict__ exist_users, int64_t n_items,
-                                           const int32_t* __restrict__ rowptr, const int32_t* __restrict__ colidx,
-                                           int64_t& u_out, int64_t& p_out, int64_t& q_out) {
+__device__ __forceinline__ int64_t sample_user(const Philox& ph, uint32_t slo, uint32_t shi, int b, int B, int half_bits,
+                                               int64_t n_exist, const int64_t* __restrict__ exist_users) {
     uint64_t slot;
     if ((int64_t)B <= n_exist) {
         slot = keyed_perm((uint64_t)b, (uint64_t)n_exist, half_bits, ph, slo, shi);
@@ -623,7 +658,14 @@
         ph((uint32_t)b, 0x55AA0001u, slo, shi, o);
         slot = ((((uint64_t)o[1] << 32) | o[0]) % (uint64_t)n_exist);
     }
-    const int64_t u = exist_users[slot];
+    return exist_users[slot];
+}
+
+__device__ __forceinline__ void sample_one(const Philox& ph, uint32_t slo, uint32_t shi, int b, int B, int half_bits,
+                                           int64_t n_exist, const int64_t* __restrict__ exist_users, int64_t n_items,
+                                           const int32_t* __restrict__ rowptr, const int32_t* __restrict__ colidx,
+                                           int64_t& u_out, int64_t& p_out, int64_t& q_out) {
+    const int64_t u = sample_user(ph, slo, shi, b, B, half_bits, n_exist, exist_users);
     const int32_t s = rowptr[u], e = rowptr[u + 1];
     uint32_t o[4];
     ph((uint32_t)b, 0x55AA0002u, slo, shi, o);
@@ -705,6 +747,68 @@
     if (threadIdx.x == 0) { n_valid_dev[0] = B + kept; *step_dev = step + 1ull; }
 }
 
+constexpr int SAMPLE_WIDE_THREADS = 256;
+__global__ __launch_bounds__(SAMPLE_WIDE_THREADS) void sample_batch_wide_kernel(
+    uint64_t seed, unsigned long long* step_dev, int64_t n_exist, const int64_t* __restrict__ exist_users,
+    int64_t n_items, const int32_t* __restrict__ rowptr, const int32_t* __restrict__ colidx,
+    int B_global, int half_bits_users, int slice_begin, int B, int n_aug, int half_bits_batch,
+    const int64_t* __restrict__ aug_pos, const int64_t* __restrict__ aug_neg,
+    int64_t* __restrict__ users, int64_t* __restrict__ pos, int64_t* __restrict__ neg, int32_t* __restrict__ n_valid_dev,
+    int32_t* ticket, int n_blocks) {
+    __shared__ int wave_tot[SAMPLE_WIDE_THREADS / 64];
+    __shared__ int base_s;
+    const unsigned long long step = *step_dev;
+    const uint32_t slo = (uint32_t)step, shi = (uint32_t)(step >> 32);
+    const Philox ph(seed);
+    if ((int)blockIdx.x + 1 < n_blocks) {
+        const int b = blockIdx.x * SAMPLE_WIDE_THREADS + threadIdx.x;
+        if (b < B)
+            sample_one(ph, slo, shi, slice_begin + b, B_global, half_bits_users, n_exist, exist_users, n_items, rowptr, colidx,
+                       users[b], pos[b], neg[b]);
+    } else {
+        if (threadIdx.x == 0) base_s = 0;
+        __syncthreads();
+        const Philox pa(seed ^ 0x9E3779B97F4A7C15ull);
+        const int lane = threadIdx.x & 63, wv = threadIdx.x >> 6;
+        for (int a0 = 0; a0 < n_aug; a0 += SAMPLE_WIDE_THREADS) {
+            const int a = a0 + threadIdx.x;
+            int64_t u = 0, ap = 0, an = 0;
+            bool ok = false;
+            if (a < n_aug) {
+                const uint64_t slot = keyed_perm((uint64_t)a, (uint64_t)B, half_bits_batch, pa, slo, shi);
+                u = sample_user(ph, slo, shi, slice_begin + (int)slot, B_global, half_bits_users, n_exist, exist_users);
+                ap = aug_pos[u]; an = aug_neg[u];
+                ok = ap >= 0 && an >= 0 && ap < n_items && an < n_items;
+            }
+            const unsigned long long bal = __ballot(ok);
+            const int before = __popcll(bal & ((1ull << lane) - 1ull));
+            if (lane == 0) wave_tot[wv] = __popcll(bal);
+            __syncthreads();
+            int wave_base = 0, chunk_tot = 0;
+            for (int k = 0; k < SAMPLE_WIDE_THREADS / 64; ++k) { const int t = wave_tot[k]; if (k < wv) wave_base += t; chunk_tot += t; }
+            const int base = base_s;
+            if (a < n_aug && ok) {
+                const int o = B + base + wave_base + before;
+                users[o] = u; pos[o] = ap; neg[o] = an;
+            }
+            __syncthreads();
+            if (threadIdx.x == 0) base_s = base + chunk_tot;
+            __syncthreads();
+        }
+        const int kept = base_s;
+        for (int o = B + kept + threadIdx.x; o < B + n_aug; o += SAMPLE_WIDE_THREADS) { users[o] = 0; pos[o] = 0; neg[o] = 0; }
+        if (threadIdx.x == 0) n_valid_dev[0] = B + kept;
+    }
+    __syncthreads();
+    if (threadIdx.x == 0) {
+        __threadfence();
+        if (atomicAdd(ticket, 1) == n_blocks - 1) {
+            *step_dev = step + 1ull;
+            atomicExch(ticket, 0);
+        }
+    }
+}
+
 }
 
 using namespace llmrec;
@@ -835,6 +939,22 @@
     LLMREC_CHECK_ARG(users && pos && neg && plan, "bpr_scatter_plan: null pointer");
     const unsigned blocks = (unsigned)(ceil_div(B_max, 16) + ceil_div(2 * (int64_t)B_max, 16));
     bpr_plan_kernel<<<blocks, 256, sizeof(uint64_t) * 2 * (size_t)B_max, (hipStream_t)stream_>>>(users, pos, neg, B_max, n_valid_dev, plan);
+    LLMREC_LAUNCH_CHECK();
+    return LLMREC_OK;
+}
+
+int llmrec_bpr_scatter_plan_reach_mark(const int64_t* users, const int64_t* pos, const int64_t* neg, int32_t B_max, const int32_t* n_valid_dev,
+                                       uint64_t* plan, int64_t n_users, int64_t n_items, const int32_t* item_rowptr,
+                                       const int32_t* item_colidx, uint8_t* flags, llmrec_stream_t stream_) {
+    LLMREC_CHECK_ARG(B_max >= 0 && n_users > 0 && n_users < 0x7fffffffll && n_items > 0, "bpr_scatter_plan_reach_mark: bad sizes");
+    LLMREC_CHECK_ARG(item_rowptr && item_colidx && flags, "bpr_scatter_plan_reach_mark: null pointer");
+    if (B_max > LLMREC_BPR_MAX_B) { set_error("bpr_scatter_plan_reach_mark: B_max %d > %d", B_max, LLMREC_BPR_MAX_B); return LLMREC_EUNSUPPORTED; }
+    if (B_max == 0) return LLMREC_OK;
+    LLMREC_CHECK_ARG(users && pos && neg && plan, "bpr_scatter_plan_reach_mark: null pointer");
+    const int plan_blocks = (int)(ceil_div(B_max, 16) + ceil_div(2 * (int64_t)B_max, 16));
+    const unsigned blocks = (unsigned)(plan_blocks + reach_mark_blocks(B_max));
+    bpr_plan_reach_mark_kernel<<<blocks, 256, sizeof(uint64_t) * 2 * (size_t)B_max, (hipStream_t)stream_>>>(
+        users, pos, neg, B_max, n_valid_dev, plan, plan_blocks, n_users, n_items, item_rowptr, item_colidx, flags);
     LLMREC_LAUNCH_CHECK();
     return LLMREC_OK;
 }
@@ -1025,4 +1145,25 @@
     return LLMREC_OK;
 }
 
-}
+int llmrec_sample_batch_wide(uint64_t seed, uint64_t* step_dev, int64_t n_exist_users, const int64_t* exist_users,
+                             int64_t n_items, const int32_t* train_rowptr, const int32_t* train_colidx,
+                             int32_t B_global, int32_t slice_begin, int32_t B, int32_t n_aug,
+                             const int64_t* aug_pos, const int64_t* aug_neg,
+                             int64_t* users, int64_t* pos, int64_t* neg, int32_t* n_valid_dev, int32_t* ticket, llmrec_stream_t stream_) {
+    LLMREC_CHECK_ARG(B >= 1 && B_global >= B && slice_begin >= 0 && slice_begin + B <= B_global && n_aug >= 0 && n_aug <= B &&
+                     n_exist_users > 0 && n_items > 0, "sample_batch_wide: bad sizes");
+    LLMREC_CHECK_ARG(step_dev && exist_users && train_rowptr && train_colidx && users && pos && neg && n_valid_dev && ticket,
+                     "sample_batch_wide: null pointer");
+    LLMREC_CHECK_ARG(n_aug == 0 || (aug_pos && aug_neg), "sample_batch_wide: augmented pairs missing");
+    int hb_users = 1, hb_batch = 1;
+    while ((1ull << (2 * hb_users)) < (uint64_t)n_exist_users) ++hb_users;
+    while ((1ull << (2 * hb_batch)) < (uint64_t)B) ++hb_batch;
+    const int n_blocks = (int)ceil_div(B, SAMPLE_WIDE_THREADS) + 1;
+    sample_batch_wide_kernel<<<n_blocks, SAMPLE_WIDE_THREADS, 0, (hipStream_t)stream_>>>(
+        seed, (unsigned long long*)step_dev, n_exist_users, exist_users, n_items, train_rowptr, train_colidx, B_global, hb_users,
+        slice_begin, B, n_aug, hb_batch, aug_pos, aug_neg, users, pos, neg, n_valid_dev, ticket, n_blocks);
+    LLMREC_LAUNCH_CHECK();
+    return LLMREC_OK;
+}
+
+}
diff --git a/llmrec_amd/csrc/reach.h b/llmrec_amd/csrc/reach.h
--- /dev/null
+++ b/llmrec_amd/csrc/reach.h
@@ -0,0 +1,31 @@
+#pragma once
+#include "common.h"
+
+namespace llmrec {
+
+constexpr int REACH_SPLIT = 8;
+
+static inline int64_t reach_mark_blocks(int B_cap) { return ceil_div(3 * (int64_t)B_cap * REACH_SPLIT, 4); }
+
+__device__ __forceinline__ void batch_reach_mark_block(int vb, int B_cap, const int32_t* __restrict__ n_valid, const int64_t* __restrict__ users,
+                                                       const int64_t* __restrict__ pos, const int64_t* __restrict__ neg, int64_t n_users,
+                                                       int64_t n_items, const int32_t* __restrict__ rowptr, const int32_t* __restrict__ colidx,
+                                                       uint8_t* __restrict__ flags) {
+    const int w = vb * 4 + (threadIdx.x >> 6), lane = threadIdx.x & 63;
+    int nv = n_valid ? *n_valid : B_cap;
+    nv = nv < B_cap ? nv : B_cap;
+    const int part = w % REACH_SPLIT, job = w / REACH_SPLIT;
+    const int b = job / 3, role = job - 3 * b;
+    if (b >= nv) return;
+    if (role == 0) {
+        const int64_t u = users[b];
+        if (part == 0 && lane == 0 && u >= 0 && u < n_users) flags[u] = 1;
+        return;
+    }
+    const int64_t it = role == 1 ? pos[b] : neg[b];
+    if (it < 0 || it >= n_items) return;
+    const int32_t s = rowptr[it], e = rowptr[it + 1];
+    for (int32_t k = s + part * 64 + lane; k < e; k += 64 * REACH_SPLIT) flags[colidx[k]] = 1;
+}
+
+}
diff --git a/llmrec_amd/csrc/rowops.hip b/llmrec_amd/csrc/rowops.hip
--- a/llmrec_amd/csrc/rowops.hip
+++ b/llmrec_amd/csrc/rowops.hip
@@ -1,4 +1,5 @@
 #include "common.h"
+#include "reach.h"
 #include <type_traits>
 
 namespace llmrec {
@@ -218,10 +219,9 @@
     for (int64_t row = (int64_t)blk * ROWS_PER_BLOCK + threadIdx.x / RL; row < rows; row += row_stride)
 
 template <int VEC, int NCHUNK>
-__global__ __launch_bounds__(256) void fuse_fwd_multi_kernel(int d, FuseMulti m) {
-    __shared__ float ss_red[256];
+__device__ __forceinline__ void fuse_fwd_multi_block(int vb, int nvb, int d, const FuseMulti& m, float* ss_red) {
     float ss = 0.f;
-    ROW_LOOP_MULTI(m, (int)blockIdx.x, (int)gridDim.x) {
+    ROW_LOOP_MULTI(m, vb, nvb) {
         RowReg<VEC, NCHUNK> acc, t;
         acc.fill(0.f);
         for (int i = 0; i < a.n_mean; ++i) {
@@ -255,8 +255,14 @@
             if ((int)threadIdx.x < off) ss_red[threadIdx.x] += ss_red[threadIdx.x + off];
             __syncthreads();
         }
-        if (threadIdx.x == 0) m.sumsq_partial[blockIdx.x] = ss_red[0];
-    }
+        if (threadIdx.x == 0) m.sumsq_partial[vb] = ss_red[0];
+    }
+}
+
+template <int VEC, int NCHUNK>
+__global__ __launch_bounds__(256) void fuse_fwd_multi_kernel(int d, FuseMulti m) {
+    __shared__ float ss_red[256];
+    fuse_fwd_multi_block<VEC, NCHUNK>((int)blockIdx.x, (int)gridDim.x, d, m, ss_red);
 }
 
 template <int VEC, int NCHUNK>
@@ -638,26 +644,11 @@
     for (int64_t k = (int64_t)s + part * 64 + (threadIdx.x & 63); k < e; k += 64 * MARK_SPLIT) flags[colidx[k]] = value;
 }
 
-constexpr int REACH_SPLIT = 8;
 __global__ __launch_bounds__(256) void batch_reach_mark_kernel(int B_cap, const int32_t* __restrict__ n_valid, const int64_t* __restrict__ users,
                                                                const int64_t* __restrict__ pos, const int64_t* __restrict__ neg, int64_t n_users,
                                                                int64_t n_items, const int32_t* __restrict__ rowptr, const int32_t* __restrict__ colidx,
                                                                uint8_t* __restrict__ flags) {
-    const int w = blockIdx.x * 4 + (threadIdx.x >> 6), lane = threadIdx.x & 63;
-    int nv = n_valid ? *n_valid : B_cap;
-    nv = nv < B_cap ? nv : B_cap;
-    const int part = w % REACH_SPLIT, job = w / REACH_SPLIT;
-    const int b = job / 3, role = job - 3 * b;
-    if (b >= nv) return;
-    if (role == 0) {
-        const int64_t u = users[b];
-        if (part == 0 && lane == 0 && u >= 0 && u < n_users) flags[u] = 1;
-        return;
-    }
-    const int64_t it = role == 1 ? pos[b] : neg[b];
-    if (it < 0 || it >= n_items) return;
-    const int32_t s = rowptr[it], e = rowptr[it + 1];
-    for (int32_t k = s + part * 64 + lane; k < e; k += 64 * REACH_SPLIT) flags[colidx[k]] = 1;
+    batch_reach_mark_block((int)blockIdx.x, B_cap, n_valid, users, pos, neg, n_users, n_items, rowptr, colidx, flags);
 }
 
 __global__ __launch_bounds__(1024) void flags_compact_kernel(int64_t n, uint8_t* __restrict__ flags, int32_t* __restrict__ list, int32_t* __restrict__ n_out) {
@@ -694,6 +685,84 @@
     const int32_t pad_end = (total + 15) / 16 * 16 + 16;
     for (int32_t k = total + tid; k < pad_end; k += 1024) list[k] = 0;
     if (tid == 0) *n_out = total;
+}
+
+constexpr int COMPACT_WPT = 8;
+__device__ __forceinline__ void flags_compact_block256(int64_t n, uint8_t* __restrict__ flags, int32_t* __restrict__ list, int32_t* __restrict__ n_out,
+                                                       int32_t* wave_total ) {
+    const int tid = threadIdx.x, lane = tid & 63, wave = tid >> 6;
+    const int64_t n_words = (n + 15) / 16;
+    int64_t wpt64 = (n_words + 255) / 256;
+    const int wpt = wpt64 > COMPACT_WPT ? COMPACT_WPT : (int)wpt64;
+    int32_t done = 0;
+    for (int64_t w0 = 0; w0 < n_words; w0 += 256 * (int64_t)wpt) {
+        uint4 v[COMPACT_WPT];
+        const int64_t mine = w0 + (int64_t)tid * wpt;
+        int32_t c = 0;
+#pragma unroll
+        for (int j = 0; j < COMPACT_WPT; ++j) {
+            v[j] = uint4{0u, 0u, 0u, 0u};
+            const int64_t wd_i = mine + j;
+            if (j < wpt && wd_i < n_words) {
+                v[j] = *reinterpret_cast<const uint4*>(flags + 16 * wd_i);
+                const int64_t left = n - 16 * wd_i;
+                uint32_t wd[4] = {v[j].x, v[j].y, v[j].z, v[j].w};
+                if (left < 16) {
+#pragma unroll
+                    for (int q = 0; q < 4; ++q)
+#pragma unroll
+                        for (int bb = 0; bb < 4; ++bb)
+                            if (4 * q + bb >= left) wd[q] &= ~(0xffu << (8 * bb));
+                    v[j] = uint4{wd[0], wd[1], wd[2], wd[3]};
+                }
+#pragma unroll
+                for (int q = 0; q < 4; ++q)
+#pragma unroll
+                    for (int bb = 0; bb < 4; ++bb) c += ((wd[q] >> (8 * bb)) & 0xffu) != 0u;
+            }
+        }
+        int32_t incl = c;
+#pragma unroll
+        for (int off = 1; off < 64; off <<= 1) {
+            const int32_t t = __shfl_up(incl, off, 64);
+            if (lane >= off) incl += t;
+        }
+        if (lane == 63) wave_total[wave] = incl;
+        __syncthreads();
+        int32_t base = 0, total = 0;
+#pragma unroll
+        for (int w2 = 0; w2 < 4; ++w2) { const int32_t t = wave_total[w2]; if (w2 < wave) base += t; total += t; }
+        __syncthreads();
+        int32_t o = done + base + incl - c;
+        if (c) {
+#pragma unroll
+            for (int j = 0; j < COMPACT_WPT; ++j) {
+                const uint32_t wd[4] = {v[j].x, v[j].y, v[j].z, v[j].w};
+                if ((wd[0] | wd[1] | wd[2] | wd[3]) == 0u) continue;
+                const int64_t r = 16 * (mine + j);
+#pragma unroll
+                for (int q = 0; q < 4; ++q)
+#pragma unroll
+                    for (int bb = 0; bb < 4; ++bb)
+                        if ((wd[q] >> (8 * bb)) & 0xffu) list[o++] = (int32_t)(r + 4 * q + bb);
+                const int64_t left = n - r;
+                if (left >= 16) *reinterpret_cast<uint4*>(flags + r) = uint4{0u, 0u, 0u, 0u};
+                else for (int64_t bb = 0; bb < left; ++bb) flags[r + bb] = 0;
+            }
+        }
+        done += total;
+    }
+    const int32_t pad_end = (done + 15) / 16 * 16 + 16;
+    for (int32_t k = done + tid; k < pad_end; k += 256) list[k] = 0;
+    if (tid == 0) *n_out = done;
+}
+
+template <int VEC, int NCHUNK>
+__global__ __launch_bounds__(256) void fuse_fwd_multi_compact_kernel(int d, FuseMulti m, int64_t n_flags, uint8_t* __restrict__ flags,
+                                                                     int32_t* __restrict__ list, int32_t* __restrict__ n_out) {
+    __shared__ float ss_red[256];
+    if (blockIdx.x == 0) { flags_compact_block256(n_flags, flags, list, n_out, reinterpret_cast<int32_t*>(ss_red)); return; }
+    fuse_fwd_multi_block<VEC, NCHUNK>((int)blockIdx.x - 1, (int)gridDim.x - 1, d, m, ss_red);
 }
 
 constexpr int COLSUM_BLOCKS = 128;
@@ -884,9 +953,9 @@
     return llmrec_fuse_fwd_multi_sumsq_f32(n_problems, p, d, 0, nullptr, 0, nullptr, stream_);
 }
 
-int llmrec_fuse_fwd_multi_sumsq_f32(int32_t n_problems, const llmrec_fuse_fwd_problem_t* p, int32_t d, int32_t n_sumsq_terms,
-                                    float* sumsq_partial, int32_t partial_capacity, int32_t* n_partial_host, llmrec_stream_t stream_) {
-    hipStream_t stream = (hipStream_t)stream_;
+static int fuse_fwd_multi_launch(int32_t n_problems, const llmrec_fuse_fwd_problem_t* p, int32_t d, int32_t n_sumsq_terms,
+                                 float* sumsq_partial, int32_t partial_capacity, int32_t* n_partial_host,
+                                 int64_t n_flags, uint8_t* flags, int32_t* row_list, int32_t* n_rows, hipStream_t stream) {
     LLMREC_CHECK_ARG(n_problems >= 1 && n_problems <= FUSE_MAX_PROBLEMS && p && d > 0, "fuse_fwd_multi: 1..%d problems", FUSE_MAX_PROBLEMS);
     LLMREC_CHECK_ARG(n_sumsq_terms >= 0 && (n_sumsq_terms == 0 || (sumsq_partial && n_partial_host)), "fuse_fwd_multi: sum of squares without a partial buffer");
     FuseMulti m = {};
@@ -921,6 +990,14 @@
         *n_partial_host = grid;
         m.n_sumsq = n_sumsq_terms; m.sumsq_partial = sumsq_partial;
     }
+    if (flags) {
+        int rc = dispatch_rows(d, vec4,
+            [&](auto nc) { fuse_fwd_multi_compact_kernel<4, decltype(nc)::value><<<grid + 1, 256, 0, stream>>>(d, m, n_flags, flags, row_list, n_rows); return 0; },
+            [&](auto) { set_error("fuse_fwd_multi_sumsq_compact: d = %d with rows that are not 16-byte aligned", d); return (int)LLMREC_EUNSUPPORTED; });
+        if (rc) return rc;
+        LLMREC_LAUNCH_CHECK();
+        return LLMREC_OK;
+    }
     if (grid == 0) return LLMREC_OK;
     int rc = dispatch_rows(d, vec4,
         [&](auto nc) { fuse_fwd_multi_kernel<4, decltype(nc)::value><<<grid, 256, 0, stream>>>(d, m); return 0; },
@@ -928,6 +1005,22 @@
     if (rc) return rc;
     LLMREC_LAUNCH_CHECK();
     return LLMREC_OK;
+}
+
+int llmrec_fuse_fwd_multi_sumsq_f32(int32_t n_problems, const llmrec_fuse_fwd_problem_t* p, int32_t d, int32_t n_sumsq_terms,
+                                    float* sumsq_partial, int32_t partial_capacity, int32_t* n_partial_host, llmrec_stream_t stream_) {
+    return fuse_fwd_multi_launch(n_problems, p, d, n_sumsq_terms, sumsq_partial, partial_capacity, n_partial_host, 0, nullptr, nullptr, nullptr,
+                                 (hipStream_t)stream_);
+}
+
+int llmrec_fuse_fwd_multi_sumsq_compact_f32(int32_t n_problems, const llmrec_fuse_fwd_problem_t* p, int32_t d, int32_t n_sumsq_terms,
+                                            float* sumsq_partial, int32_t partial_capacity, int32_t* n_partial_host,
+                                            int64_t n_users, uint8_t* flags, int32_t* row_list, int32_t* n_rows, llmrec_stream_t stream_) {
+    LLMREC_CHECK_ARG(n_users > 0 && n_users < 0x7fffffffll, "fuse_fwd_multi_sumsq_compact: bad sizes");
+    LLMREC_CHECK_ARG(flags && row_list && n_rows, "fuse_fwd_multi_sumsq_compact: null pointer");
+    LLMREC_CHECK_ARG((uintptr_t)flags % 16 == 0, "fuse_fwd_multi_sumsq_compact: flags must be 16-byte aligned (and readable up to n_users rounded up to 16 bytes)");
+    return fuse_fwd_multi_launch(n_problems, p, d, n_sumsq_terms, sumsq_partial, partial_capacity, n_partial_host, n_users, flags, row_list, n_rows,
+                                 (hipStream_t)stream_);
 }
 
 static int fill_fuse_bwd_multi(int32_t n_problems, const llmrec_fuse_bwd_problem_t* p, int32_t d, FuseMulti& m, bool& vec4, int& grid) {
@@ -1175,7 +1268,7 @@
     LLMREC_CHECK_ARG((uintptr_t)flags % 16 == 0, "batch_reach_rows: flags must be 16-byte aligned (and readable up to n_users rounded up to 16 bytes)");
     hipStream_t stream = (hipStream_t)stream_;
     if (B_cap > 0) {
-        batch_reach_mark_kernel<<<(unsigned)ceil_div(3 * (int64_t)B_cap * REACH_SPLIT, 4), 256, 0, stream>>>(B_cap, n_valid, users, pos, neg, n_users, n_items,
+        batch_reach_mark_kernel<<<(unsigned)reach_mark_blocks(B_cap), 256, 0, stream>>>(B_cap, n_valid, users, pos, neg, n_users, n_items,
                                                                                                 item_rowptr, item_colidx, flags);
         LLMREC_LAUNCH_CHECK();
     }
diff --git a/llmrec_amd/engine.py b/llmrec_amd/engine.py
--- a/llmrec_amd/engine.py
+++ b/llmrec_amd/engine.py
@@ -73,8 +73,13 @@
         self.seed = seed
         self.capacity = self.B + self.n_aug
         self.step_dev = torch.zeros(1, dtype=torch.int64, device=exist_users.device)
+        self.ticket = torch.zeros(1, dtype=torch.int32, device=exist_users.device)
 
     def fill(self, users, pos, neg, n_valid):
+        if self.world == 1:
+            ops.sample_batch_wide(self.seed, self.step_dev, self.exist_users, self.n_items, self.train, self.B, 0, self.B, self.n_aug,
+                                  self.aug_pos, self.aug_neg, users, pos, neg, n_valid, self.ticket)
+            return
         ops.sample_batch(self.seed, self.step_dev, self.exist_users, self.n_items, self.train, self.B * self.world,
                          self.rank * self.B, self.B, self.n_aug, self.aug_pos, self.aug_neg, users, pos, neg, n_valid)
 
diff --git a/llmrec_amd/fused.py b/llmrec_amd/fused.py
--- a/llmrec_amd/fused.py
+++ b/llmrec_amd/fused.py
@@ -129,6 +129,7 @@
             self.ss_partial = torch.zeros(self.ss_cap, dtype=torch.float32, device=dev)
             self.ss_n = 0
         self._ev_plan = self._ev_reach = None
+        self._reach_pending = None
         self._zero_in_forward = False
         self._emb_params = [model.user_id_embedding.weight, model.item_id_embedding.weight]
         self._lin_params = [p for p in optimizer.params if p.grad is not None and all(p is not e for e in self._emb_params)]
@@ -318,7 +319,15 @@
         problem(arr[1], self.E_u, m.user_id_embedding.weight, self.Ul, self.U_cat, self.prof_u)
         if self.fold and self._zero_in_forward:
             n_part = _c.c_int32(0)
-            _call("llmrec_fuse_fwd_multi_sumsq_f32", 2, arr, d, 2, _p(self.ss_partial), self.ss_cap, _c.byref(n_part))
+            pending, self._reach_pending = self._reach_pending, None
+            if pending is not None and _lib.call_unless_unsupported(
+                    "llmrec_fuse_fwd_multi_sumsq_compact_f32", 2, arr, d, 2, _p(self.ss_partial), self.ss_cap, _c.byref(n_part),
+                    self.iu.fwd.n_cols, _p(self.act_flags), _p(self.act_rows), _p(self.act_n), ops._stream()):
+                pending = None
+            else:
+                _call("llmrec_fuse_fwd_multi_sumsq_f32", 2, arr, d, 2, _p(self.ss_partial), self.ss_cap, _c.byref(n_part))
+            if pending is not None:
+                ops.batch_reach_rows(*pending, self.iu.fwd, self.act_flags, self.act_rows, self.act_n)
             self.ss_n = int(n_part.value)
         else:
             _call("llmrec_fuse_fwd_multi_f32", 2, arr, d)
@@ -659,6 +668,14 @@
         self._ev_plan = self._ev_reach = None
 
         def batch_lists():
+            if self.wgrad_rows and sampler is not None and self.fold and not self.multi_stream:
+                if users.numel() > self.b_max:
+                    raise RuntimeError("FusedStep: batch of %d exceeds b_max %d" % (users.numel(), self.b_max))
+                if _lib.call_unless_unsupported("llmrec_bpr_scatter_plan_reach_mark", _p(users), _p(pos), _p(neg), users.numel(), _p(n_valid),
+                                                _p(self.bpr_plan), self.iu.fwd.n_cols, self.iu.fwd.n_rows, _p(self.iu.fwd.rowptr),
+                                                _p(self.iu.fwd.colidx), _p(self.act_flags), ops._stream()):
+                    self._reach_pending = (users, pos, neg, n_valid)
+                    return
             self.build_scatter_plan(users, pos, neg, n_valid)
             self._ev_plan = self._mark()
             if self.wgrad_rows:
@@ -685,6 +702,9 @@
         except Exception:
             if not torch.cuda.is_current_stream_capturing():
                 try:
+                    if self._reach_pending is not None:
+                        self._reach_pending = None
+                        self.act_flags.zero_()
                     self.reset_scatter_targets()
                 except Exception:
                     pass
diff --git a/llmrec_amd/ops.py b/llmrec_amd/ops.py
--- a/llmrec_amd/ops.py
+++ b/llmrec_amd/ops.py
@@ -1074,6 +1074,16 @@
               B_global, slice_begin, B, n_aug, _p(aug_pos), _p(aug_neg), _p(users), _p(pos), _p(neg), _p(n_valid), _stream())
 
 
+def sample_batch_wide(seed: int, step_dev: torch.Tensor, exist_users: torch.Tensor, n_items: int, train: Csr, B_global: int,
+                      slice_begin: int, B: int, n_aug: int, aug_pos: Optional[torch.Tensor], aug_neg: Optional[torch.Tensor],
+                      users: torch.Tensor, pos: torch.Tensor, neg: torch.Tensor, n_valid: torch.Tensor, ticket: torch.Tensor):
+    _need_gpu(step_dev, exist_users, users, pos, neg, n_valid, ticket)
+    if users.numel() < B + n_aug or step_dev.dtype != torch.int64 or n_valid.dtype != torch.int32 or ticket.dtype != torch.int32:
+        raise RuntimeError("sample_batch_wide: buffers of B + n_aug int64 entries, int64 step counter, int32 n_valid and ticket expected")
+    _lib.call("llmrec_sample_batch_wide", seed, _p(step_dev), exist_users.numel(), _p(exist_users), n_items, _p(train.rowptr), _p(train.colidx),
+              B_global, slice_begin, B, n_aug, _p(aug_pos), _p(aug_neg), _p(users), _p(pos), _p(neg), _p(n_valid), _p(ticket), _stream())
+
+
 def topk_metrics(idx: torch.Tensor, hits: torch.Tensor, query_users: torch.Tensor, test_rowptr: torch.Tensor, Ks) -> torch.Tensor:
     _need_gpu(idx, hits, query_users, test_rowptr)
     n, K = idx.shape
```
